# zhang-tao-whu/DVIS_Plus

Hardware: AMD Instinct MI355X
Metric: frames/sec DVIS++ R50 offline, 720p T=30 synthetic (higher is better)
Workload: dtype f32 (storage, accumulation, results; the segmenter's dense layers - R50 convolutions from 128 channels on, pixel-decoder projections and FPN output convolution, the deformable encoder's projections and FFN, the decoder's key / value projections - multiply each fp32 operand as two f16 terms on the f1

## Files before the change

### dvis_plus_amd/csrc/conv1x1_x3.hip

```cpp
#include "dvis_common.h"
#include "x3_common.h"

DVIS_EXPORT int64_t dvis_conv_x3_image_bytes(int64_t N, int C, int H, int W);

namespace {

constexpr unsigned kOOB = 0x80000000u;

struct CxArgs {
  const float *x, *bias, *res;
  const void *wp;
  float *y;
  int N, C, K, relu, npass;
  int stride, W_in, OW, H_in;
  int taps;
  long long HW, HW_in, pixels;
  long long tiles;
  float xscale, inv;
  int *flag;
  int tag;
  const float *x2;
  int C2, stride2, W2_in;
  long long HW2_in;
  void *img;
  int XG;
  float oscale;
  int OH;
  const void *ximg;
  int XG_in;
};

__device__ __forceinline__ bool cx_item(const CxArgs &a, long long w, long long *tile, int *pass) {
  const int xcd = blockIdx.x & 7, i = blockIdx.x >> 3, per = gridDim.x >> 3;
  const long long m = i + (long long)per * w;
  const long long u = m / a.npass;
  *pass = (int)(m - u * a.npass);
  *tile = xcd + 8 * u;
  return *tile < a.tiles;
}

struct CxGeom {
  unsigned base;
  int iy, ix;
  int row0;
};
__device__ __forceinline__ CxGeom cx_geom(const CxArgs &a, long long p) {
  CxGeom gm = {kOOB, 0, 0, 0};
  if (p >= a.pixels) return gm;
  const long long n = p / a.HW;
  const int pix = (int)(p - n * a.HW);
  const int oy = pix / a.OW, ox = pix - oy * a.OW, pad = a.taps == 9 ? 1 : 0;
  gm.base = (unsigned)(n * a.C * a.HW_in * 4);
  gm.iy = oy * a.stride - pad, gm.ix = ox * a.stride - pad;
  gm.row0 = (int)(n * a.H_in);
  return gm;
}
__device__ __forceinline__ unsigned cx_tap_offset(const CxArgs &a, const CxGeom &gm, int tap) {
  const int dy = a.taps == 9 ? tap / 3 : 0, dx = a.taps == 9 ? tap - 3 * dy : 0;
  const int iy = gm.iy + dy, ix = gm.ix + dx;
  const bool ok = gm.base != kOOB && iy >= 0 && iy < a.H_in && ix >= 0 && ix < a.W_in;
  return ok ? gm.base + (unsigned)((iy * a.W_in + ix) * 4) : kOOB;
}

__device__ __forceinline__ unsigned cx_tap_offset_img(const CxArgs &a, const CxGeom &gm, int tap, int g) {
  const int dy = a.taps == 9 ? tap / 3 : 0, dx = a.taps == 9 ? tap - 3 * dy : 0;
  const int iy = gm.iy + dy, ix = gm.ix + dx;
  const bool ok = gm.base != kOOB && iy >= 0 && iy < a.H_in && ix >= 0 && ix < a.W_in;
  return ok ? (unsigned)(((gm.row0 + iy) * a.XG_in + (ix >> 5)) * ((a.C / 64) * 8192) + g * 512 + (ix & 31) * 16) : kOOB;
}

__device__ __forceinline__ unsigned cx_geom2(const CxArgs &a, long long p) {
  if (a.C2 == 0 || p >= a.pixels) return kOOB;
  const long long n = p / a.HW;
  const int pix = (int)(p - n * a.HW);
  const int oy = pix / a.OW, ox = pix - oy * a.OW;
  return (unsigned)(n * a.C2 * a.HW2_in * 4) + (unsigned)((oy * a.stride2 * a.W2_in + ox * a.stride2) * 4);
}

template <int NB, int IK, bool IMGIN = false, bool IMGOUT = false>
__global__ __launch_bounds__(512) void conv1x1_x3_kernel(const CxArgs a) {
  constexpr int NW = 8, kTile = NW * 32, PW = 2 * IK * NB / NW, STAGES = IK == 4 ? 2 : 3, IPC = 4 / IK;
  static_assert(2 * IK * NB % NW == 0, "the item's pieces must divide among the waves");
  extern __shared__ __attribute__((aligned(1024))) char lds[];
  const int wave = threadIdx.x >> 6, lane = threadIdx.x & 63, j = lane & 31, g = lane >> 5;
  const int NCC = a.C / 64, NC1 = a.taps * NCC, NC = NC1 + a.C2 / 64, NI = IPC * NC;
  long long wcount = 0;
  {
    long long t;
    int q;
    while (cx_item(a, wcount, &t, &q)) ++wcount;
  }
  if (wcount == 0) return;
  const __amdgpu_buffer_rsrc_t rx = dvis_make_rsrc_uniform(a.x, (unsigned)((long long)a.N * a.C * a.HW_in * 4));
  const __amdgpu_buffer_rsrc_t ry = dvis_make_rsrc_uniform(a.y, (unsigned)((long long)a.N * a.K * a.HW * 4));
  const __amdgpu_buffer_rsrc_t rr = dvis_make_rsrc_uniform(a.res ? a.res : a.y, (unsigned)((long long)a.N * a.K * a.HW * 4));
  const unsigned chan = (unsigned)(a.HW_in * 4);
  const __amdgpu_buffer_rsrc_t rx2 = dvis_make_rsrc_uniform(a.C2 ? a.x2 : a.x, a.C2 ? (unsigned)((long long)a.N * a.C2 * a.HW2_in * 4) : 0u);
  const unsigned chan2 = (unsigned)(a.HW2_in * 4);

  typedef Ring<PW, IMGIN ? 8 : 32, NW, STAGES> RingT;
  RingT ring;
  long long iw = 0;
  int ic = 0, ipass;
  {
    long long t;
    cx_item(a, 0, &t, &ipass);
  }
  auto next_offset = [&]() -> size_t {
    const size_t o = ((size_t)ipass * NI + ic) * RingT::kItemBytes;
    if (++ic == NI) {
      ic = 0;
      long long t;
      if (!cx_item(a, ++iw, &t, &ipass)) ipass = 0;
    }
    return o;
  };
  ring.init(a.wp, lds, 1, (int)(wcount * NI), wave, lane);
#pragma unroll
  for (int i = 0; i < RingT::kAhead; ++i)
    if (ring.total > i) ring.issue_at(next_offset());

  float raw[32];
  auto load_raw = [&](unsigned pixoff, int cc, bool second = false) {
    const __amdgpu_buffer_rsrc_t r = second ? rx2 : rx;
    const unsigned ch = second ? chan2 : chan;
    const unsigned vo = pixoff + (unsigned)(8 * g) * ch;
    const unsigned so = (unsigned)(64 * cc) * ch;
#pragma unroll
    for (int s = 0; s < 4; ++s)
#pragma unroll
      for (int e = 0; e < 8; ++e)
        raw[8 * s + e] = __builtin_bit_cast(float, __builtin_amdgcn_raw_buffer_load_b32(r, vo, so + (unsigned)(16 * s + e) * ch, 0));
  };
  const __amdgpu_buffer_rsrc_t rxi = dvis_make_rsrc_uniform(IMGIN ? a.ximg : (const void *)a.x,
                                                            IMGIN ? (unsigned)((long long)a.N * a.H_in * a.XG_in * (a.C / 64) * 8192) : 0u);
  h8 nh[4], nl[4];
  auto load_img = [&](unsigned off, int cc) {
#pragma unroll
    for (int s = 0; s < 4; ++s) {
      nh[s] = __builtin_bit_cast(h8, __builtin_amdgcn_raw_buffer_load_b128(rxi, off, (unsigned)(8192 * cc + 2048 * s), 0));
      nl[s] = __builtin_bit_cast(h8, __builtin_amdgcn_raw_buffer_load_b128(rxi, off, (unsigned)(8192 * cc + 2048 * s + 1024), 0));
    }
  };
  long long tile;
  int pass;
  cx_item(a, 0, &tile, &pass);
  CxGeom gm = cx_geom(a, tile * kTile + wave * 32 + j);
  unsigned gm2 = cx_geom2(a, tile * kTile + wave * 32 + j);
  if constexpr (IMGIN)
    load_img(cx_tap_offset_img(a, gm, 0, g), 0);
  else
    load_raw(cx_tap_offset(a, gm, 0), 0);
  for (long long w = 0; w < wcount; ++w) {
    const long long p = tile * kTile + wave * 32 + j;
    long long ntile = tile;
    int npass_ = pass;
    const bool more = cx_item(a, w + 1, &ntile, &npass_);
    const CxGeom ngm = more ? cx_geom(a, ntile * kTile + wave * 32 + j) : CxGeom{kOOB, 0, 0, 0};
    const unsigned ngm2 = more ? cx_geom2(a, ntile * kTile + wave * 32 + j) : kOOB;
    int tap = 0, cc = 0;
    f16v acc[NB];
#pragma unroll
    for (int nb = 0; nb < NB; ++nb)
#pragma unroll
      for (int i = 0; i < 16; ++i) acc[nb][i] = 0.f;
    const long long n = p / a.HW;
    const unsigned obase = p < a.pixels ? (unsigned)((n * a.K * a.HW + (p - n * a.HW)) * 4) : kOOB;
    const unsigned ochan = (unsigned)(a.HW * 4);
    const int co0 = pass * 32 * NB;
    for (int kc = 0; kc < NC; ++kc) {
      h8 xh[4], xl[4];
      if constexpr (IMGIN) {
#pragma unroll
        for (int s = 0; s < 4; ++s) {
          asm volatile("" : "+v"(nh[s]), "+v"(nl[s]));
          xh[s] = nh[s], xl[s] = nl[s];
        }
        if (++cc == NCC) cc = 0, ++tap;
        const bool first = kc + 1 < NC1;
        load_img(first ? cx_tap_offset_img(a, gm, tap, g) : cx_tap_offset_img(a, ngm, 0, g), first ? cc : 0);
      } else {
#pragma unroll
        for (int i = 0; i < 32; ++i) asm volatile("" : "+v"(raw[i]));
#pragma unroll
        for (int s = 0; s < 4; ++s) {
          const f4 lo4 = {raw[8 * s], raw[8 * s + 1], raw[8 * s + 2], raw[8 * s + 3]};
          const f4 hi4 = {raw[8 * s + 4], raw[8 * s + 5], raw[8 * s + 6], raw[8 * s + 7]};
          split8(lo4, hi4, a.xscale, xh[s], xl[s]);
        }
        if (++cc == NCC) cc = 0, ++tap;
        const bool first = kc + 1 < NC1, sec = !first && kc + 1 < NC;
        const unsigned po = first ? cx_tap_offset(a, gm, tap) : (sec ? gm2 : cx_tap_offset(a, ngm, 0));
        load_raw(po, first ? cc : (sec ? kc + 1 - NC1 : 0), sec);
      }
#pragma unroll
      for (int part = 0; part < IPC; ++part) {
        const char *stage = ring.wait(false);
        ring.begin(ring.more() ? next_offset() : 0);
        mma_item<IK, NB, PW>(stage, lane, acc, xh + IK * part, xl + IK * part, [&](int i) { ring.piece(i); });
      }
    }
    float chk = 0.f;
    if constexpr (NB == 2 || IMGOUT) {
      if (a.img != nullptr) {
        const unsigned gs = (unsigned)(a.K / 64) * 8192u;
        const __amdgpu_buffer_rsrc_t ri = dvis_make_rsrc_uniform(a.img, (unsigned)((long long)a.N * a.OH * a.XG * gs));
        const __amdgpu_buffer_rsrc_t rb = dvis_make_rsrc_uniform(a.bias ? (const void *)a.bias : (const void *)a.img, a.bias ? (unsigned)a.K * 4u : 0u);
        unsigned ibase = kOOB;
        if (p < a.pixels) {
          const int pix = (int)(p - n * a.HW), oy = pix / a.OW, ox = pix - oy * a.OW;
          ibase = (unsigned)(((n * a.OH + oy) * a.XG + (ox >> 5)) * gs + (co0 / 64) * 8192 + g * 512 + (ox & 31) * 16);
        }
#pragma unroll
        for (int nb = 0; nb < NB; ++nb) {
          float v[16];
#pragma unroll
          for (int q = 0; q < 4; ++q) {
            const f4 b = __builtin_bit_cast(f4, __builtin_amdgcn_raw_buffer_load_b128(rb, (unsigned)(co0 + 32 * nb + 8 * q + 4 * g) * 4u, 0, 0));
#pragma unroll
            for (int i = 0; i < 4; ++i) {
              const float t = acc[nb][4 * q + i] * a.inv + b[i];
              chk = __builtin_fmaf(t, 0.f, chk);
              v[4 * q + i] = a.relu ? x3_relu(t) : t;
            }
          }
          h8 hi[2], lo[2];
#pragma unroll
          for (int u = 0; u < 2; ++u) {
            const f4 p0 = {v[8 * u], v[8 * u + 1], v[8 * u + 2], v[8 * u + 3]}, p1 = {v[8 * u + 4], v[8 * u + 5], v[8 * u + 6], v[8 * u + 7]};
            split8(p0, p1, a.oscale, hi[u], lo[u]);
          }
          const h8 ls = lo[0] + lo[1];
          chk = __builtin_fmaf((float)((ls[0] + ls[1]) + (ls[2] + ls[3]) + (ls[4] + ls[5]) + (ls[6] + ls[7])), 0.f, chk);
          store_fragments4(ri, ibase, hi[0], 4096 * nb, lo[0], 4096 * nb + 1024, hi[1], 4096 * nb + 2048, lo[1], 4096 * nb + 3072);
        }
        if (a.flag != nullptr && chk != chk && p < a.pixels) atomicCAS(a.flag, 0, a.tag);
        tile = ntile, pass = npass_, gm = ngm, gm2 = ngm2;
        continue;
      }
    }
#pragma unroll
    for (int nb = 0; nb < NB; ++nb) {
      float rv[16];
#pragma unroll
      for (int r = 0; r < 16; ++r)
        rv[r] = a.res ? __builtin_bit_cast(float, __builtin_amdgcn_raw_buffer_load_b32(
                                                      rr, obase + (unsigned)(co0 + 32 * nb + 8 * (r >> 2) + 4 * g + (r & 3)) * ochan, 0, 0))
                      : 0.f;
#pragma unroll
      for (int q = 0; q < 4; ++q) {
        const int co = co0 + 32 * nb + 8 * q + 4 * g;
        f4 b = {0.f, 0.f, 0.f, 0.f};
        if (a.bias) b = *(const f4 *)(a.bias + co);
#pragma unroll
        for (int i = 0; i < 4; ++i) {
          const unsigned o = obase + (unsigned)(co + i) * ochan;
          float v = acc[nb][4 * q + i] * a.inv + b[i] + rv[4 * q + i];
          chk = __builtin_fmaf(v, 0.f, chk);
          if (a.relu) v = x3_relu(v);
          __builtin_amdgcn_raw_buffer_store_b32(__builtin_bit_cast(unsigned, v), ry, o, 0, 0);
        }
      }
    }
    if (a.flag != nullptr && chk != chk && p < a.pixels) atomicCAS(a.flag, 0, a.tag);
    tile = ntile, pass = npass_, gm = ngm, gm2 = ngm2;
  }
}

__global__ __launch_bounds__(256) void upsample_add_image_kernel(const float *__restrict__ lateral, const float *__restrict__ top,
                                                                 void *__restrict__ img, int N, int C, int H, int W, int h, int w,
                                                                 const float *__restrict__ lat_scale, const float *__restrict__ lat_shift,
                                                                 float oscale) {
  const int NCC = C / 64, XG = (W + 31) / 32;
  const int cc = blockIdx.x, xg = blockIdx.y;
  const int x = threadIdx.x & 31, g = (threadIdx.x >> 5) & 1, S = threadIdx.x >> 6;
  const int px = 32 * xg + x;
  const float sy = (float)h / (float)H, sx = (float)w / (float)W;
  const int pxc = px < W ? px : W - 1;
  float fx = sx * ((float)pxc + 0.5f) - 0.5f;
  fx = fx < 0.f ? 0.f : fx;
  const int x0 = min((int)fx, w - 1), x1 = x0 + (x0 < w - 1 ? 1 : 0);
  const float lx1 = fx - (float)x0, lx0 = 1.f - lx1;
  const __amdgpu_buffer_rsrc_t ri = dvis_make_rsrc_uniform(img, (unsigned)((long long)N * H * XG * NCC * 8192));
  const unsigned rows = (unsigned)N * (unsigned)H;
  for (unsigned row = blockIdx.z * 16u; row < blockIdx.z * 16u + 16u && row < rows; ++row) {
    const unsigned n = row / (unsigned)H;
    const int y = (int)(row - n * (unsigned)H);
    float fy = sy * ((float)y + 0.5f) - 0.5f;
    fy = fy < 0.f ? 0.f : fy;
    const int y0 = min((int)fy, h - 1), y1 = y0 + (y0 < h - 1 ? 1 : 0);
    const float ly1 = fy - (float)y0, ly0 = 1.f - ly1;
    float v[8];
#pragma unroll
    for (int e = 0; e < 8; ++e) {
      const int c = 64 * cc + 32 * (S >> 1) + 16 * (S & 1) + 8 * (e >> 2) + 4 * g + (e & 3);
      const unsigned pl = n * (unsigned)C + (unsigned)c;
      const float *t0 = top + ((size_t)pl * h + y0) * (size_t)w, *t1 = top + ((size_t)pl * h + y1) * (size_t)w;
      float lat = lateral[((size_t)pl * H + y) * (size_t)W + pxc];
      if (lat_scale) lat = lat * lat_scale[pl] + lat_shift[pl];
      v[e] = lat + (ly0 * (lx0 * t0[x0] + lx1 * t0[x1]) + ly1 * (lx0 * t1[x0] + lx1 * t1[x1]));
    }
    const f4 p0 = {v[0], v[1], v[2], v[3]}, p1 = {v[4], v[5], v[6], v[7]};
    h8 hi, lo;
    split8(p0, p1, oscale, hi, lo);
    const unsigned G = row * (unsigned)XG + (unsigned)xg;
    const unsigned off = (G * (unsigned)NCC + (unsigned)cc) * 8192u + (unsigned)(S * 2048 + g * 512 + x * 16);
    store_fragments2(ri, off, hi, 0, lo, 1024);
  }
}

}

DVIS_EXPORT int dvis_upsample_add_image(const float *lateral, const float *lat_scale, const float *lat_shift, const float *top, void *image,
                                        int N, int C, int H, int W, int h, int w, int oexp, void *stream) {
  DVIS_REQUIRE(lateral && top && image, "dvis_upsample_add_image: null pointer");
  DVIS_REQUIRE((lat_scale == nullptr) == (lat_shift == nullptr), "dvis_upsample_add_image: scale and shift together");
  DVIS_REQUIRE(N > 0 && C > 0 && C % 64 == 0 && H > 0 && W > 0 && h > 0 && w > 0, "dvis_upsample_add_image: bad sizes");
  DVIS_REQUIRE((uintptr_t)image % 16 == 0 && dvis_conv_x3_image_bytes(N, C, H, W) < ((int64_t)1 << 31), "dvis_upsample_add_image: a 16-byte "
               "aligned image below 2 GiB");
  const int per = 16 * 65535 / H;
  DVIS_REQUIRE(per >= 1 && (W + 31) / 32 <= 65535, "dvis_upsample_add_image: map too large (%d x %d)", H, W);
  for (int i = 0; i < N; i += per) {
    const int n = N - i < per ? N - i : per;
    hipLaunchKernelGGL(upsample_add_image_kernel, dim3(C / 64, (W + 31) / 32, (n * H + 15) / 16), dim3(256), 0, (hipStream_t)stream,
                       lateral + (size_t)i * C * H * W, top + (size_t)i * C * h * w,
                       (char *)image + (size_t)i * H * ((W + 31) / 32) * (C / 64) * 8192, n, C, H, W, h, w,
                       lat_scale ? lat_scale + (size_t)i * C : nullptr, lat_shift ? lat_shift + (size_t)i * C : nullptr, ldexpf(1.f, oexp));
  }
  return dvis_check_launch("dvis_upsample_add_image");
}

DVIS_EXPORT int dvis_conv1x1_x3_supported(int C, int K, int64_t N, int64_t HW_in, int64_t HW_out) {
  if (C < 64 || C % 64 != 0 || C > 4096) return 0;
  if (!(K == 64 || K == 128 || (K > 0 && K % 256 == 0 && K <= 8192))) return 0;
  if (N <= 0 || HW_out <= 0 || HW_in < HW_out) return 0;
  if (N * C * HW_in * 4 >= ((int64_t)1 << 31) || N * K * HW_out * 4 >= ((int64_t)1 << 31)) return 0;
  return 1;
}

DVIS_EXPORT int64_t dvis_conv1x1_x3_packed_bytes(int C, int K) {
  if (!dvis_conv1x1_x3_supported(C, K, 1, 1, 1)) return -1;
  return (int64_t)(C / 16) * (K / 32) * 2 * kPiece;
}

DVIS_EXPORT int dvis_conv1x1_x3_pack(const float *w, int K, int C, int wexp, void *packed, void *stream) {
  DVIS_REQUIRE(w && packed, "dvis_conv1x1_x3_pack: null operand");
  DVIS_REQUIRE(dvis_conv1x1_x3_supported(C, K, 1, 1, 1), "dvis_conv1x1_x3_pack: (C, K) = (%d, %d) is not served", C, K);
  DVIS_REQUIRE(wexp >= -60 && wexp <= 60, "dvis_conv1x1_x3_pack: wexp = %d", wexp);
  const int NB = K == 64 ? 2 : K == 128 ? 4 : 8;
  const int64_t fragments = (int64_t)(C / 16) * (K / 32) * 64;
  hipLaunchKernelGGL(x3_pack_kernel, dim3((unsigned)((fragments + 255) / 256)), dim3(256), 0, (hipStream_t)stream, w, (int64_t)C, K, C,
                     NB, 0, ldexpf(1.f, wexp), (_Float16 *)packed, fragments);
  return dvis_check_launch("dvis_conv1x1_x3_pack");
}

static int cx_launch(const float *x, const void *packed, const float *bias, const float *res, float *y, int N, int C, int K, int H, int W,
                     int stride, int taps, int xexp, int wexp, int relu, void *stream, const float *x2 = nullptr, int C2 = 0, int H2 = 0,
                     int W2 = 0, int stride2 = 1, void *image = nullptr, int oexp = 0, const void *ximg = nullptr);

DVIS_EXPORT int dvis_conv1x1_x3_dual(const float *x, const float *x2, const void *packed, const float *bias, const float *res, float *y,
                                     int N, int C, int C2, int K, int H, int W, int H2, int W2, int stride2, int xexp, int wexp, int relu,
                                     void *stream) {
  DVIS_REQUIRE(x2 != nullptr && C2 >= 64 && C2 % 64 == 0 && C2 <= 4096, "dvis_conv1x1_x3_dual: C2 %% 64 == 0 (got %d)", C2);
  DVIS_REQUIRE((stride2 == 1 || stride2 == 2) && (H2 + stride2 - 1) / stride2 == H && (W2 + stride2 - 1) / stride2 == W,
               "dvis_conv1x1_x3_dual: x2 (%d x %d, stride %d) must down-sample onto x's %d x %d map", H2, W2, stride2, H, W);
  DVIS_REQUIRE((long long)N * C2 * H2 * W2 * 4 < ((long long)1 << 31) && (uintptr_t)x2 % 16 == 0, "dvis_conv1x1_x3_dual: x2 below 2 GiB, 16-byte aligned");
  return cx_launch(x, packed, bias, res, y, N, C, K, H, W, 1, 1, xexp, wexp, relu, stream, x2, C2, H2, W2, stride2);
}

DVIS_EXPORT int dvis_conv1x1_x3(const float *x, const void *packed, const float *bias, const float *res, float *y, int N, int C, int K,
                                int H, int W, int stride, int xexp, int wexp, int relu, void *stream) {
  return cx_launch(x, packed, bias, res, y, N, C, K, H, W, stride, 1, xexp, wexp, relu, stream);
}

DVIS_EXPORT int dvis_conv1x1_x3_image(const float *x, const void *packed, const float *bias, void *image, int N, int C, int H, int W, int xexp,
                                      int wexp, int oexp, int relu, void *stream) {
  DVIS_REQUIRE(image != nullptr && (uintptr_t)image % 16 == 0, "dvis_conv1x1_x3_image: null / unaligned image");
  DVIS_REQUIRE((long long)N * H * ((W + 31) / 32) * 8192 < ((long long)1 << 31), "dvis_conv1x1_x3_image: the image must stay below 2 GiB");
  return cx_launch(x, packed, bias, nullptr, nullptr, N, C, 64, H, W, 1, 1, xexp, wexp, relu, stream, nullptr, 0, 0, 0, 1, image, oexp);
}

DVIS_EXPORT int64_t dvis_conv_x3_image_bytes(int64_t N, int C, int H, int W) {
  if (N < 0 || C <= 0 || C % 64 != 0 || H <= 0 || W <= 0) return -1;
  return N * H * ((W + 31) / 32) * (int64_t)(C / 64) * 8192;
}

DVIS_EXPORT int dvis_conv_x3_pack_image(const float *w, int K, int C, int taps, int wexp, void *packed, void *stream) {
  DVIS_REQUIRE(w && packed, "dvis_conv_x3_pack_image: null operand");
  DVIS_REQUIRE(taps == 1 || taps == 9, "dvis_conv_x3_pack_image: taps = %d", taps);
  DVIS_REQUIRE(dvis_conv1x1_x3_supported(C, K, 1, 1, 1) && K >= 128, "dvis_conv_x3_pack_image: (C, K) = (%d, %d) is not served", C, K);
  DVIS_REQUIRE(wexp >= -60 && wexp <= 60, "dvis_conv_x3_pack_image: wexp = %d", wexp);
  const int NB = K == 128 ? 4 : 8;
  const int64_t fragments = (int64_t)(taps * C / 16) * (K / 32) * 64;
  hipLaunchKernelGGL(x3_pack_kernel, dim3((unsigned)((fragments + 255) / 256)), dim3(256), 0, (hipStream_t)stream, w, (int64_t)taps * C, K,
                     taps * C, NB, 1, ldexpf(1.f, wexp), (_Float16 *)packed, fragments, taps);
  return dvis_check_launch("dvis_conv_x3_pack_image");
}

DVIS_EXPORT int dvis_conv_x3_image(const void *ximg, const float *x, const void *packed, const float *bias, const float *res, float *y,
                                   void *image, int N, int C, int K, int H, int W, int stride, int taps, int xexp, int wexp, int oexp, int relu,
                                   void *stream) {
  DVIS_REQUIRE(ximg != nullptr || image != nullptr, "dvis_conv_x3_image: neither side is an operand image (use dvis_conv1x1_x3 / dvis_conv3x3_x3)");
  DVIS_REQUIRE((ximg != nullptr) != (x != nullptr), "dvis_conv_x3_image: exactly one of ximg and x");
  DVIS_REQUIRE((image != nullptr) != (y != nullptr), "dvis_conv_x3_image: exactly one of image and y");
  DVIS_REQUIRE(K == 128 || K % 256 == 0, "dvis_conv_x3_image: K = %d (128 or a multiple of 256)", K);
  DVIS_REQUIRE(taps == 1 || taps == 9, "dvis_conv_x3_image: taps = %d", taps);
  DVIS_REQUIRE(image == nullptr || res == nullptr, "dvis_conv_x3_image: an image output takes no residual");
  DVIS_REQUIRE(((uintptr_t)ximg | (uintptr_t)image) % 16 == 0, "dvis_conv_x3_image: images must be 16-byte aligned");
  const int OH = (H + stride - 1) / stride, OW = (W + stride - 1) / stride;
  DVIS_REQUIRE(dvis_conv_x3_image_bytes(N, C, H, W) < ((int64_t)1 << 31) && dvis_conv_x3_image_bytes(N, K, OH, OW) < ((int64_t)1 << 31),
               "dvis_conv_x3_image: images must stay below 2 GiB");
  return cx_launch(x, packed, bias, res, y, N, C, K, H, W, stride, taps, xexp, wexp, relu, stream, nullptr, 0, 0, 0, 1, image, oexp, ximg);
}

DVIS_EXPORT int64_t dvis_conv3x3_x3_packed_bytes(int C, int K) {
  const int64_t b = dvis_conv1x1_x3_packed_bytes(C, K);
  return b < 0 ? b : 9 * b;
}

DVIS_EXPORT int dvis_conv3x3_x3_pack(const float *w, int K, int C, int wexp, void *packed, void *stream) {
  DVIS_REQUIRE(w && packed, "dvis_conv3x3_x3_pack: null operand");
  DVIS_REQUIRE(dvis_conv1x1_x3_supported(C, K, 1, 1, 1), "dvis_conv3x3_x3_pack: (C, K) = (%d, %d) is not served", C, K);
  DVIS_REQUIRE(wexp >= -60 && wexp <= 60, "dvis_conv3x3_x3_pack: wexp = %d", wexp);
  const int NB = K == 64 ? 2 : K == 128 ? 4 : 8;
  const int64_t fragments = (int64_t)(9 * C / 16) * (K / 32) * 64;
  hipLaunchKernelGGL(x3_pack_kernel, dim3((unsigned)((fragments + 255) / 256)), dim3(256), 0, (hipStream_t)stream, w, (int64_t)9 * C, K, 9 * C,
                     NB, 0, ldexpf(1.f, wexp), (_Float16 *)packed, fragments, 9);
  return dvis_check_launch("dvis_conv3x3_x3_pack");
}

DVIS_EXPORT int dvis_conv3x3_x3(const float *x, const void *packed, const float *bias, const float *res, float *y, int N, int C, int K,
                                int H, int W, int stride, int xexp, int wexp, int relu, void *stream) {
  return cx_launch(x, packed, bias, res, y, N, C, K, H, W, stride, 9, xexp, wexp, relu, stream);
}

static int cx_launch(const float *x, const void *packed, const float *bias, const float *res, float *y, int N, int C, int K, int H, int W,
                     int stride, int taps, int xexp, int wexp, int relu, void *stream, const float *x2, int C2, int H2, int W2, int stride2,
                     void *image, int oexp, const void *ximg) {
  DVIS_REQUIRE((x || ximg) && packed && (y || image), "dvis_conv1x1_x3: null operand");
  DVIS_REQUIRE(stride == 1 || stride == 2, "dvis_conv1x1_x3: stride %d", stride);
  const int OH = (H + stride - 1) / stride, OW = (W + stride - 1) / stride;
  DVIS_REQUIRE(dvis_conv1x1_x3_supported(C, K, N, (int64_t)H * W, (int64_t)OH * OW), "dvis_conv1x1_x3: shape (N %d, C %d, K %d, %d x %d, "
               "stride %d) is not served (C %% 64 == 0, K = 64 / 128 or K %% 256 == 0, tensors below 2 GiB)", N, C, K, H, W, stride);
  DVIS_REQUIRE((uintptr_t)x % 16 == 0 && (uintptr_t)y % 16 == 0 && (uintptr_t)packed % 16 == 0 && (bias == nullptr || (uintptr_t)bias % 16 == 0),
               "dvis_conv1x1_x3: operands must be 16-byte aligned");
  CxArgs a = {};
  a.x = x, a.bias = bias, a.res = res, a.wp = packed, a.y = y, a.N = N, a.C = C, a.K = K, a.relu = relu;
  a.stride = stride, a.W_in = W, a.H_in = H, a.taps = taps, a.OW = OW, a.HW = (long long)OH * OW, a.HW_in = (long long)H * W;
  a.pixels = a.HW * N;
  a.xscale = ldexpf(1.f, xexp), a.inv = ldexpf(1.f, -(xexp + wexp));
  const X3Guard gd = dvis_x3_guard();
  a.flag = gd.flag, a.tag = gd.tag;
  a.x2 = x2, a.C2 = x2 ? C2 : 0, a.stride2 = stride2, a.W2_in = W2, a.HW2_in = (long long)H2 * W2;
  a.img = image, a.XG = (OW + 31) / 32, a.oscale = ldexpf(1.f, oexp), a.OH = OH;
  a.ximg = ximg, a.XG_in = (W + 31) / 32;
  const int grid = dvis_x3_persistent_cus();
  hipStream_t st = (hipStream_t)stream;
  a.npass = K <= 128 ? 1 : K / 256;
#define DVIS_CX_LAUNCH(NBV, IKV)                                                                              \
  {                                                                                                           \
    static DvisLdsOptIn opted;                                                                                \
    typedef Ring<2 * IKV * NBV / 8, 32, 8, (IKV == 4 ? 2 : 3)> R;                                             \
    a.tiles = (a.pixels + 255) / 256;                                                                         \
    const size_t lds = (IKV == 4 ? 2 : 3) * R::kItemBytes;                                                    \
    const int rc = dvis_lds_opt_in((const void *)conv1x1_x3_kernel<NBV, IKV>, lds, &opted, "dvis_conv1x1_x3"); \
    if (rc != DVIS_OK) return rc;                                                                             \
    hipLaunchKernelGGL((conv1x1_x3_kernel<NBV, IKV>), dim3(grid), dim3(512), lds, st, a);                     \
  }
#define DVIS_CX_LAUNCH_IMG(NBV, IKV, INV, OUTV)                                                                                    \
  {                                                                                                                                \
    static DvisLdsOptIn opted;                                                                                                     \
    typedef Ring<2 * IKV * NBV / 8, 8, 8, (IKV == 4 ? 2 : 3)> R;                                                                   \
    a.tiles = (a.pixels + 255) / 256;                                                                                              \
    const size_t lds = (IKV == 4 ? 2 : 3) * R::kItemBytes;                                                                         \
    const int rc = dvis_lds_opt_in((const void *)conv1x1_x3_kernel<NBV, IKV, INV, OUTV>, lds, &opted, "dvis_conv_x3_image");    \
    if (rc != DVIS_OK) return rc;                                                                                                  \
    hipLaunchKernelGGL((conv1x1_x3_kernel<NBV, IKV, INV, OUTV>), dim3(grid), dim3(512), lds, st, a);                            \
    return dvis_check_launch("dvis_conv_x3_image");                                                                                \
  }
  if (ximg != nullptr || (image != nullptr && K != 64)) {
    DVIS_REQUIRE(x2 == nullptr, "dvis_conv_x3_image: no second source");
    if (K == 128) {
      if (ximg && image) DVIS_CX_LAUNCH_IMG(4, 2, true, true)
      if (ximg) DVIS_CX_LAUNCH_IMG(4, 2, true, false)
      DVIS_CX_LAUNCH_IMG(4, 2, false, true)
    }
    if (ximg && image) DVIS_CX_LAUNCH_IMG(8, 4, true, true)
    if (ximg) DVIS_CX_LAUNCH_IMG(8, 4, true, false)
    DVIS_CX_LAUNCH_IMG(8, 4, false, true)
  }
#undef DVIS_CX_LAUNCH_IMG
  if (K == 64) DVIS_CX_LAUNCH(2, 2)
  else if (K == 128) DVIS_CX_LAUNCH(4, 2)
  else DVIS_CX_LAUNCH(8, 4)
#undef DVIS_CX_LAUNCH
  return dvis_check_launch("dvis_conv1x1_x3");
}
```

### dvis_plus_amd/csrc/fused_elementwise.hip

```cpp
#include <math.h>

#include "dvis_common.h"

namespace {

template <int V>
__global__ __launch_bounds__(256) void add_layernorm_kernel(const float *__restrict__ x, const float *__restrict__ res,
                                                            int64_t res_row_stride, const float *__restrict__ gamma,
                                                            const float *__restrict__ beta, float *__restrict__ out,
                                                            size_t rows, int C, float eps,
                                                            const float *__restrict__ pos, size_t pos_rows,
                                                            float *__restrict__ out_pos) {
  const int lane = threadIdx.x & 63;
  const size_t row = (size_t)blockIdx.x * 4 + (threadIdx.x >> 6);
  if (row >= rows) return;
  const float4 *xr = reinterpret_cast<const float4 *>(x + row * C);
  const float4 *rr = res ? reinterpret_cast<const float4 *>(res + row * res_row_stride) : nullptr;
  float4 v[V];
  float sum = 0.f;
#pragma unroll
  for (int i = 0; i < V; ++i) {
    const int c4 = lane + 64 * i;
    if (c4 * 4 < C) {
      v[i] = xr[c4];
// ... 372 lines not shown
  float *ob = out + b * batch_stride + c4;
#pragma unroll
  for (int o = 0; o < 4; ++o) {
    if (x0 + o >= w) break;
    float4 v = acc[o];
    if (gelu) {
      v.x = 0.5f * v.x * (1.f + erff(v.x * 0.70710678118654752440f)), v.y = 0.5f * v.y * (1.f + erff(v.y * 0.70710678118654752440f));
      v.z = 0.5f * v.z * (1.f + erff(v.z * 0.70710678118654752440f)), v.w = 0.5f * v.w * (1.f + erff(v.w * 0.70710678118654752440f));
    }
    *reinterpret_cast<float4 *>(ob + ((int64_t)y * w + x0 + o) * C) = v;
  }
}

}

DVIS_EXPORT int dvis_normalize_pad(const void *in, int is_u8, float *out, int64_t planes, int C, int H, int W, int Hp, int Wp,
                                   const float *mean, const float *stdv, void *stream) {
  DVIS_REQUIRE(planes >= 0 && C > 0 && H > 0 && W > 0 && Hp >= H && Wp >= W, "normalize_pad: bad sizes");
  if (planes == 0) return DVIS_OK;
  DVIS_REQUIRE(in && out && mean && stdv, "normalize_pad: null pointer");
  DVIS_REQUIRE(planes <= 65535 && (Hp + 3) / 4 <= 65535, "normalize_pad: grid too large");
  const dim3 grid((unsigned)(((Wp + 3) / 4 + 63) / 64), (unsigned)((Hp + 3) / 4), (unsigned)planes);
  if (is_u8)
    hipLaunchKernelGGL(normalize_pad_kernel<unsigned char>, grid, dim3(256), 0, (hipStream_t)stream, (const unsigned char *)in, out, C,
                       H, W, Hp, Wp, mean, stdv);
  else
    hipLaunchKernelGGL(normalize_pad_kernel<float>, grid, dim3(256), 0, (hipStream_t)stream, (const float *)in, out, C, H, W, Hp, Wp,
                       mean, stdv);
  return dvis_check_launch("normalize_pad_kernel");
}

DVIS_EXPORT int dvis_tokens_to_nchw(const float *tok, float *out, int64_t N, int C, int64_t HW, int64_t S, int64_t row0, void *stream) {
  DVIS_REQUIRE(N >= 0 && C > 0 && HW > 0 && S >= HW && row0 >= 0 && row0 + HW <= S, "tokens_to_nchw: bad sizes");
  if (N == 0) return DVIS_OK;
  DVIS_REQUIRE(tok && out, "tokens_to_nchw: null pointer");
  DVIS_REQUIRE(N <= 65535 && (C + 63) / 64 <= 65535 && HW < (1ll << 31), "tokens_to_nchw: grid too large");
  hipLaunchKernelGGL(tokens_to_nchw_kernel, dim3((unsigned)((HW + 63) / 64), (unsigned)((C + 63) / 64), (unsigned)N), dim3(256), 0,
                     (hipStream_t)stream, tok, out, C, (int)HW, S, row0);
  return dvis_check_launch("tokens_to_nchw_kernel");
}

static int nchw_to_tokens_launch(const float *x, float *out, int64_t N, int C, int64_t HW, int64_t S, int64_t row0,
                                 const float *scale, const float *shift, const float *pos, float *out_pos, void *stream) {
  DVIS_REQUIRE(N >= 0 && C > 0 && HW > 0 && S >= HW && row0 >= 0 && row0 + HW <= S, "nchw_to_tokens: bad sizes");
  if (N == 0) return DVIS_OK;
  DVIS_REQUIRE(x && out, "nchw_to_tokens: null pointer");
  DVIS_REQUIRE((scale == nullptr) == (shift == nullptr) && (pos == nullptr) == (out_pos == nullptr),
               "nchw_to_tokens: scale/shift and pos/out_pos come in pairs");
  DVIS_REQUIRE(N <= 65535 && (C + 63) / 64 <= 65535 && HW < (1ll << 31), "nchw_to_tokens: grid too large");
  hipLaunchKernelGGL(nchw_to_tokens_kernel, dim3((unsigned)((HW + 63) / 64), (unsigned)((C + 63) / 64), (unsigned)N), dim3(256),
                     0, (hipStream_t)stream, x, out, C, (int)HW, S, row0, scale, shift, pos, out_pos);
  return dvis_check_launch("nchw_to_tokens_kernel");
}

DVIS_EXPORT int dvis_nchw_to_tokens(const float *x, float *out, int64_t N, int C, int64_t HW, int64_t S, int64_t row0,
                                    void *stream) {
  return nchw_to_tokens_launch(x, out, N, C, HW, S, row0, nullptr, nullptr, nullptr, nullptr, stream);
}

DVIS_EXPORT int dvis_nchw_to_tokens_affine(const float *x, const float *scale, const float *shift, const float *pos,
                                           float *out, float *out_pos, int64_t N, int C, int64_t HW, int64_t S,
                                           int64_t row0, void *stream) {
  return nchw_to_tokens_launch(x, out, N, C, HW, S, row0, scale, shift, pos, out_pos, stream);
}

DVIS_EXPORT int dvis_bias_act(float *x, const float *bias, const float *res, int64_t planes, int C, int64_t HW, int relu,
                              void *stream) {
  DVIS_REQUIRE(planes >= 0 && C > 0 && HW > 0, "bias_act: bad sizes");
  if (planes == 0) return DVIS_OK;
  DVIS_REQUIRE(x, "bias_act: null pointer");
  if (HW % 4 != 0 || (((uintptr_t)x | (uintptr_t)res) & 15) != 0) {
    const long long total = (long long)planes * HW;
    const long long blocks = (total + 255) / 256;
    hipLaunchKernelGGL(bias_act_scalar_kernel, dim3((unsigned)(blocks > 65535 * 16 ? 65535 * 16 : blocks)), dim3(256), 0,
                       (hipStream_t)stream, x, bias, res, C, (long long)HW, total, relu);
    return dvis_check_launch("bias_act_scalar_kernel");
  }
  const int HW4 = (int)(HW / 4);
  int chunks = (HW4 + 1023) / 1024;
  if (chunks < 1) chunks = 1;
  DVIS_REQUIRE(planes * chunks < (1ll << 31), "bias_act: too many planes");
  hipLaunchKernelGGL(bias_act_kernel, dim3((unsigned)(planes * chunks)), dim3(256), 0, (hipStream_t)stream, x, bias, res, C,
                     HW4, chunks, relu);
  return dvis_check_launch("bias_act_kernel");
}

static int add_layernorm_launch(const float *x, const float *res, int64_t res_row_stride, const float *gamma,
                                const float *beta, float *out, int64_t rows, int C, float eps, const float *pos,
                                int64_t pos_rows, float *out_pos, void *stream) {
  DVIS_REQUIRE(rows >= 0 && C > 0, "add_layernorm: bad sizes");
  if (rows == 0) return DVIS_OK;
  DVIS_REQUIRE(x && gamma && beta && out, "add_layernorm: null pointer");
  DVIS_REQUIRE(C % 4 == 0 && C <= 1024, "add_layernorm: C must be a multiple of 4 and <= 1024 (got %d)", C);
  DVIS_REQUIRE(res == nullptr || res_row_stride % 4 == 0, "add_layernorm: residual row stride must be a multiple of 4");
  DVIS_REQUIRE(pos == nullptr || (pos_rows > 0 && out_pos != nullptr), "add_layernorm: pos needs pos_rows > 0 and out_pos");
  const uintptr_t al = (uintptr_t)x | (uintptr_t)res | (uintptr_t)gamma | (uintptr_t)beta | (uintptr_t)out |
                       (uintptr_t)pos | (uintptr_t)out_pos;
  DVIS_REQUIRE((al & 15) == 0, "add_layernorm: pointers must be 16-byte aligned");
  const dim3 grid((unsigned)((rows + 3) / 4)), block(256);
  hipStream_t st = (hipStream_t)stream;
  const size_t pr = pos ? (size_t)pos_rows : 1;
  if (C <= 256)
    hipLaunchKernelGGL((add_layernorm_kernel<1>), grid, block, 0, st, x, res, res_row_stride, gamma, beta, out, (size_t)rows, C, eps, pos, pr, out_pos);
  else if (C <= 512)
    hipLaunchKernelGGL((add_layernorm_kernel<2>), grid, block, 0, st, x, res, res_row_stride, gamma, beta, out, (size_t)rows, C, eps, pos, pr, out_pos);
  else
    hipLaunchKernelGGL((add_layernorm_kernel<4>), grid, block, 0, st, x, res, res_row_stride, gamma, beta, out, (size_t)rows, C, eps, pos, pr, out_pos);
  return dvis_check_launch("add_layernorm_kernel");
}

DVIS_EXPORT int dvis_add_layernorm(const float *x, const float *res, int64_t res_row_stride, const float *gamma,
                                   const float *beta, float *out, int64_t rows, int C, float eps, void *stream) {
  return add_layernorm_launch(x, res, res_row_stride, gamma, beta, out, rows, C, eps, nullptr, 0, nullptr, stream);
}

DVIS_EXPORT int dvis_add_layernorm_pos(const float *x, const float *res, int64_t res_row_stride, const float *gamma,
                                       const float *beta, float *out, const float *pos, int64_t pos_rows, float *out_pos,
                                       int64_t rows, int C, float eps, void *stream) {
  DVIS_REQUIRE(pos && out_pos, "add_layernorm_pos: null pos / out_pos");
  return add_layernorm_launch(x, res, res_row_stride, gamma, beta, out, rows, C, eps, pos, pos_rows, out_pos, stream);
}

static int upsample_add_launch(const float *lateral, const float *top, float *out, int64_t planes, int H, int W, int h,
                               int w, const float *lat_scale, const float *lat_shift, void *stream) {
  DVIS_REQUIRE(planes >= 0 && H > 0 && W > 0 && h > 0 && w > 0, "upsample_add: bad sizes");
  if (planes == 0) return DVIS_OK;
  DVIS_REQUIRE(lateral && top && out, "upsample_add: null pointer");
  DVIS_REQUIRE((lat_scale == nullptr) == (lat_shift == nullptr), "upsample_add: scale and shift come together");
  DVIS_REQUIRE(planes < (1ll << 31), "upsample_add: too many planes");
  if (W % 4 != 0 || (((uintptr_t)lateral | (uintptr_t)out) & 15) != 0) {
    const long long tot = (long long)planes * H * W;
    long long nb = (tot + 255) / 256;
    if (nb > 256 * 32) nb = 256 * 32;
    hipLaunchKernelGGL(upsample_add_scalar_kernel, dim3((unsigned)nb), dim3(256), 0, (hipStream_t)stream, lateral, top, out, tot, H, W,
                       h, w, lat_scale, lat_shift);
    return dvis_check_launch("upsample_add_scalar_kernel");
  }
  const size_t total = (size_t)planes * H * (W / 4);
  size_t blocks = (total + 255) / 256;
  if (blocks > 256 * 32) blocks = 256 * 32;
  DVIS_REQUIRE(total < (1ull << 32), "upsample_add: more than 2^32 output quads");
  const bool x2 = H == 2 * h && W == 2 * w && (w & 1) == 0 && ((uintptr_t)top & 7) == 0;
  if (x2)
    hipLaunchKernelGGL(upsample_add_kernel<true>, dim3((unsigned)blocks), dim3(256), 0, (hipStream_t)stream, lateral, top,
                       out, (int)planes, H, W, h, w, lat_scale, lat_shift);
  else
    hipLaunchKernelGGL(upsample_add_kernel<false>, dim3((unsigned)blocks), dim3(256), 0, (hipStream_t)stream, lateral, top,
                       out, (int)planes, H, W, h, w, lat_scale, lat_shift);
  return dvis_check_launch("upsample_add_kernel");
}

DVIS_EXPORT int dvis_dwconv3x3_tokens(const float *x, float *out, int64_t batch_stride, int B, int h, int w, int C, const float *weight,
                                      const float *bias, int gelu, void *stream) {
  DVIS_REQUIRE(x && out && weight, "dwconv3x3_tokens: null pointer");
  DVIS_REQUIRE(B >= 0 && h > 0 && w > 0 && C > 0 && C % 4 == 0 && batch_stride % 4 == 0 && batch_stride >= (int64_t)h * w * C,
               "dwconv3x3_tokens: C %% 4 == 0 and a batch stride that is a multiple of 4 floats >= h * w * C are required");
  DVIS_REQUIRE(((uintptr_t)x | (uintptr_t)out | (uintptr_t)(bias ? bias : weight)) % 16 == 0, "dwconv3x3_tokens: 16-byte alignment");
  DVIS_REQUIRE(x != out, "dwconv3x3_tokens: in place is not possible (neighbouring tokens are read)");
  if (B == 0) return DVIS_OK;
  const int64_t strips = (int64_t)h * ((w + 3) / 4);
  DVIS_REQUIRE(strips * B < ((int64_t)1 << 32), "dwconv3x3_tokens: too many tokens");
  hipLaunchKernelGGL(dwconv3x3_tokens_kernel, dim3((unsigned)((strips * B + 3) / 4), (C / 4 + 63) / 64), dim3(256), 0, (hipStream_t)stream, x,
                     out, batch_stride, B, h, w, C, weight, bias, gelu);
  return dvis_check_launch("dwconv3x3_tokens_kernel");
}

DVIS_EXPORT int dvis_adapter_res2(const float *g, const float *c1, const float *x1, const float *scale, const float *shift, float *out,
                                  int B, int C, int h8, int w8, void *stream) {
  DVIS_REQUIRE(g && c1 && scale && shift && out, "adapter_res2: null pointer");
  DVIS_REQUIRE(((uintptr_t)g | (uintptr_t)c1 | (uintptr_t)out) % 16 == 0, "adapter_res2: g / c1 / out must be 16-byte aligned");
  DVIS_REQUIRE(B >= 0 && C > 0 && C % 64 == 0 && h8 > 0 && w8 > 0 && h8 % 2 == 0 && w8 % 2 == 0,
               "adapter_res2: C %% 64 == 0 and an even stride-8 grid are required (C %d, grid %d x %d)", C, h8, w8);
  DVIS_REQUIRE((int64_t)B * h8 <= 65535 && C / 64 <= 65535, "adapter_res2: grid too large (B * rows %lld)", (long long)B * h8);
  if (B == 0) return DVIS_OK;
  hipLaunchKernelGGL(adapter_res2_kernel, dim3((w8 + 31) / 32, C / 64, B * h8), dim3(256), 0, (hipStream_t)stream, g, c1, x1, scale, shift,
                     out, C, h8, w8);
  return dvis_check_launch("adapter_res2_kernel");
}

DVIS_EXPORT int dvis_upsample_add(const float *lateral, const float *top, float *out, int64_t planes, int H, int W, int h,
                                  int w, void *stream) {
  return upsample_add_launch(lateral, top, out, planes, H, W, h, w, nullptr, nullptr, stream);
}

DVIS_EXPORT int dvis_upsample_add_affine(const float *lateral, const float *lat_scale, const float *lat_shift,
                                         const float *top, float *out, int64_t planes, int H, int W, int h, int w,
                                         void *stream) {
  DVIS_REQUIRE(lat_scale && lat_shift, "upsample_add_affine: null scale / shift");
  return upsample_add_launch(lateral, top, out, planes, H, W, h, w, lat_scale, lat_shift, stream);
}

DVIS_EXPORT int dvis_bias_relu_maxpool(const float *x, const float *bias, float *out, int64_t planes, int C, int H, int W,
                                       void *stream) {
  DVIS_REQUIRE(planes >= 0 && C > 0 && H > 0 && W > 0, "bias_relu_maxpool: bad sizes");
  if (planes == 0) return DVIS_OK;
  DVIS_REQUIRE(x && out, "bias_relu_maxpool: null pointer");
  DVIS_REQUIRE(H % 2 == 0 && W % 8 == 0 && (((uintptr_t)x | (uintptr_t)out) & 15) == 0,
               "bias_relu_maxpool: needs even H, W %% 8 == 0 and 16-byte aligned x / out (H=%d W=%d)", H, W);
  const size_t total = (size_t)planes * (H / 2) * (W / 8);
  DVIS_REQUIRE(planes < (1ll << 31) && total < (1ull << 32), "bias_relu_maxpool: too many planes / outputs");
  size_t blocks = (total + 255) / 256;
  if (blocks > 256 * 32) blocks = 256 * 32;
  hipLaunchKernelGGL(bias_relu_maxpool_kernel, dim3((unsigned)blocks), dim3(256), 0, (hipStream_t)stream, x, bias, out,
                     (int)planes, C, H, W);
  return dvis_check_launch("bias_relu_maxpool_kernel");
}

namespace {

__global__ __launch_bounds__(1024) void group_norm_affine_kernel(const float *__restrict__ x, const float *__restrict__ gamma,
                                                                 const float *__restrict__ beta, float *__restrict__ scale,
                                                                 float *__restrict__ shift, int C, int G, long long HW,
                                                                 float eps, int vec) {
  __shared__ double s_sum[16], s_sq[16];
  const int Cg = C / G;
  const int n = blockIdx.x / G, g = blockIdx.x - n * G;
  const long long count = (long long)Cg * HW, count4 = count / 4;
  const float4 *xp = reinterpret_cast<const float4 *>(x + ((size_t)n * C + (size_t)g * Cg) * HW);
  double sum = 0.0, sq = 0.0;
  if (vec) {
    for (long long i = threadIdx.x; i < count4; i += 1024) {
      const float4 v = xp[i];
      sum += ((double)v.x + (double)v.y) + ((double)v.z + (double)v.w);
      sq += ((double)v.x * v.x + (double)v.y * v.y) + ((double)v.z * v.z + (double)v.w * v.w);
    }
  } else {
    const float *xs = reinterpret_cast<const float *>(xp);
    for (long long i = threadIdx.x; i < count; i += 1024) {
      const double v = (double)xs[i];
      sum += v;
      sq += v * v;
    }
  }
#pragma unroll
  for (int o = 32; o > 0; o >>= 1) {
    sum += __shfl_down(sum, o);
    sq += __shfl_down(sq, o);
  }
  const int wv = threadIdx.x >> 6;
  if ((threadIdx.x & 63) == 0) {
    s_sum[wv] = sum;
    s_sq[wv] = sq;
  }
  __syncthreads();
  if (threadIdx.x < Cg) {
    double ts = 0.0, tq = 0.0;
#pragma unroll
    for (int i = 0; i < 16; ++i) {
      ts += s_sum[i];
      tq += s_sq[i];
    }
    const double mean = ts / (double)count;
    double var = tq / (double)count - mean * mean;
    var = var < 0.0 ? 0.0 : var;
    const float rstd = (float)(1.0 / sqrt(var + (double)eps));
    const int c = g * Cg + threadIdx.x;
    const float a = rstd * (gamma ? gamma[c] : 1.f);
    scale[(size_t)n * C + c] = a;
    shift[(size_t)n * C + c] = (beta ? beta[c] : 0.f) - (float)mean * a;
  }
}

__global__ __launch_bounds__(256) void scale_shift_act_kernel(float *__restrict__ x, const float *__restrict__ scale,
                                                              const float *__restrict__ shift, int HW4, int chunks, int relu) {
  const unsigned plane = blockIdx.x / chunks;
  const int chunk = blockIdx.x - plane * chunks;
  const float a = scale[plane], b = shift[plane];
  float4 *xp = reinterpret_cast<float4 *>(x) + (size_t)plane * HW4;
  for (int i = chunk * 256 + threadIdx.x; i < HW4; i += chunks * 256) {
    float4 v = xp[i];
    v.x = v.x * a + b; v.y = v.y * a + b; v.z = v.z * a + b; v.w = v.w * a + b;
    if (relu) {
      v.x = fmaxf(v.x, 0.f); v.y = fmaxf(v.y, 0.f); v.z = fmaxf(v.z, 0.f); v.w = fmaxf(v.w, 0.f);
    }
    xp[i] = v;
  }
}

__global__ __launch_bounds__(256) void scale_shift_act_scalar_kernel(float *__restrict__ x, const float *__restrict__ scale,
                                                                     const float *__restrict__ shift, long long HW, long long total,
                                                                     int relu) {
  for (long long i = (long long)blockIdx.x * 256 + threadIdx.x; i < total; i += (long long)gridDim.x * 256) {
    const long long plane = i / HW;
    const float v = x[i] * scale[plane] + shift[plane];
    x[i] = relu ? fmaxf(v, 0.f) : v;
  }
}

}

DVIS_EXPORT int dvis_group_norm_affine(const float *x, const float *gamma, const float *beta, float *scale, float *shift,
                                       int64_t N, int C, int G, int64_t HW, float eps, void *stream) {
  DVIS_REQUIRE(N >= 0 && C > 0 && G > 0 && HW > 0 && C % G == 0, "group_norm_affine: bad sizes (C=%d G=%d)", C, G);
  if (N == 0) return DVIS_OK;
  DVIS_REQUIRE(x && scale && shift, "group_norm_affine: null pointer");
  DVIS_REQUIRE(C / G <= 1024, "group_norm_affine: at most 1024 channels per group");
  const int vec = ((int64_t)(C / G) * HW) % 4 == 0 && ((uintptr_t)x & 15) == 0;
  DVIS_REQUIRE(N * G < (1ll << 31), "group_norm_affine: too many groups");
  hipLaunchKernelGGL(group_norm_affine_kernel, dim3((unsigned)(N * G)), dim3(1024), 0, (hipStream_t)stream, x, gamma, beta,
                     scale, shift, C, G, (long long)HW, eps, vec);
  return dvis_check_launch("group_norm_affine_kernel");
}

DVIS_EXPORT int dvis_scale_shift_act(float *x, const float *scale, const float *shift, int64_t planes, int64_t HW, int relu,
                                     void *stream) {
  DVIS_REQUIRE(planes >= 0 && HW > 0, "scale_shift_act: bad sizes");
  if (planes == 0) return DVIS_OK;
  DVIS_REQUIRE(x && scale && shift, "scale_shift_act: null pointer");
  if (HW % 4 != 0 || ((uintptr_t)x & 15) != 0) {
    const long long total = (long long)planes * HW;
    const long long blocks = (total + 255) / 256;
    hipLaunchKernelGGL(scale_shift_act_scalar_kernel, dim3((unsigned)(blocks > 65535 * 16 ? 65535 * 16 : blocks)), dim3(256), 0,
                       (hipStream_t)stream, x, scale, shift, (long long)HW, total, relu);
    return dvis_check_launch("scale_shift_act_scalar_kernel");
  }
  const int HW4 = (int)(HW / 4);
  int chunks = (HW4 + 1023) / 1024;
  if (chunks < 1) chunks = 1;
  DVIS_REQUIRE(planes * chunks < (1ll << 31), "scale_shift_act: too many planes");
  hipLaunchKernelGGL(scale_shift_act_kernel, dim3((unsigned)(planes * chunks)), dim3(256), 0, (hipStream_t)stream, x, scale,
                     shift, HW4, chunks, relu);
  return dvis_check_launch("scale_shift_act_kernel");
}
```

### dvis_plus_amd/functions.py

```python
import collections
import ctypes
import math
import os
import threading

import torch
from torch.autograd import Function
from torch.autograd.function import once_differentiable

from . import cpu_ops, derived, native
from .cpu_ops import ms_deform_attn_core_pytorch


def _torch_path(op, x, why):
    if os.environ.get("DVIS_STRICT", "1") != "0" and x.is_cuda and not torch.is_grad_enabled():
        raise RuntimeError(f"DVIS_STRICT: {op} would run its torch formulation on a GPU tensor ({why}; shape "
                           f"{tuple(x.shape)}, dtype {x.dtype}, contiguous {x.is_contiguous()})")


class no_autocast:

    def __enter__(self):
        import contextlib
        self._stack = contextlib.ExitStack()
# ... 1263 lines not shown
    buf, wexp = x3_tile_pack(weight, img.order)
    bptr = None if bias is None else native.dev_ptr(bias.detach(), "bias")
    lib = native.lib()
    with torch.cuda.device(img.device):
        if act == "gelu":
            if residual is not None:
                raise RuntimeError("x3_tile_linear: the GELU form of a row image writes a row image (no residual)")
            out = _rows_image_buffer(M, N, img.device)
            native.check(lib.dvis_x3_tile_linear_image(ctypes.c_void_p(img.data.data_ptr()), M, K, ctypes.c_void_p(buf.data_ptr()), N, img.exp, wexp,
                                                       bptr, 2, None, 0, None, 0, ctypes.c_void_p(out.data_ptr()), X3_XEXP,
                                                       native.stream_ptr(img.device)), "dvis_x3_tile_linear_image")
            return RowImage(out, (*img.shape[:-1], N), X3_XEXP, 1)
        out = torch.empty((*img.shape[:-1], N), dtype=torch.float32, device=img.device)
        rptr, ldr = None, 0
        if residual is not None:
            if residual.shape != out.shape or residual.dtype != torch.float32 or not residual.is_cuda:
                raise RuntimeError("x3_tile_linear: residual must be a float32 GPU tensor of the output's shape")
            r2, ldr = _rows2d(residual, N)
            rptr = ctypes.c_void_p(r2.data_ptr())
        native.check(lib.dvis_x3_tile_linear_image(ctypes.c_void_p(img.data.data_ptr()), M, K, ctypes.c_void_p(buf.data_ptr()), N, img.exp, wexp,
                                                   bptr, {None: 0, "relu": 1}[act], rptr, ldr, ctypes.c_void_p(out.data_ptr()), N, None, 0,
                                                   native.stream_ptr(img.device)), "dvis_x3_tile_linear_image")
    return out


X3_QKV_FUSED = os.environ.get("DVIS_X3_QKV_FUSED", "1") != "0"


def x3_qkv_attention_ok(x, weight, heads):
    if isinstance(x, RowImage):
        if len(x.shape) != 3 or not (X3_QKV_FUSED and weight.dim() == 2 and weight._base is None):
            return False
        B, L, C = x.shape
        return (C == heads * 64 and weight.shape == (3 * C, C) and L >= 1024 and C >= X3_TILE_MIN_K
                and bool(native.lib().dvis_x3_tile_supported(3 * C, C)))
    if not (X3_QKV_FUSED and x.dim() == 3 and x.is_cuda and x.dtype == torch.float32 and not torch.is_grad_enabled()
            and not torch.is_autocast_enabled() and x3_on() and weight.dim() == 2 and weight._base is None):
        return False
    B, L, C = x.shape
    return (C == heads * 64 and weight.shape == (3 * C, C) and L >= 1024 and x.is_contiguous() and x.data_ptr() % 16 == 0
            and x3_tile_ok(x, 3 * C, C))


def x3_qkv_attention(x, weight, bias, heads, out_image=False):
    B, L, C = x.shape
    image_in = isinstance(x, RowImage)
    buf, wexp = x3_tile_pack(weight, x.order if image_in else 0)
    lib = native.lib()
    nbytes = lib.dvis_attention_ws_bytes_k(B * heads, L, L, 64, 2)
    ws = torch.empty((nbytes + 3) // 4, dtype=torch.float32, device=x.device)
    qscale = (1.0 / 8.0) * 1.4426950408889634 * 16.0
    bptr = None if bias is None else native.dev_ptr(bias.detach(), "bias")
    with torch.cuda.device(x.device):
        if image_in:
            native.check(lib.dvis_x3_tile_linear_qkv_image(
                ctypes.c_void_p(x.data.data_ptr()), B * L, C, ctypes.c_void_p(buf.data_ptr()), 3 * C, x.exp, wexp, bptr, heads, L, qscale,
                ctypes.c_void_p(ws.data_ptr()), native.stream_ptr(x.device)), "dvis_x3_tile_linear_qkv_image")
        else:
            native.check(lib.dvis_x3_tile_linear_qkv(
                ctypes.c_void_p(x.data_ptr()), C, B * L, C, ctypes.c_void_p(buf.data_ptr()), 3 * C, X3_XEXP, wexp, bptr, heads, L, qscale,
                ctypes.c_void_p(ws.data_ptr()), native.stream_ptr(x.device)), "dvis_x3_tile_linear_qkv")
        if out_image:
            out = _rows_image_buffer(B * L, C, x.device)
            native.check(lib.dvis_attention_x3_packed_image(ctypes.c_void_p(ws.data_ptr()), ctypes.c_void_p(out.data_ptr()), B, heads, L, X3_XEXP,
                                                            native.stream_ptr(x.device)), "dvis_attention_x3_packed_image")
            return RowImage(out, (B, L, C), X3_XEXP, 2)
        out = torch.empty((B, L, C), dtype=torch.float32, device=x.device)
        strides = (ctypes.c_int64 * 3)(L * C, 64, C)
        native.check(lib.dvis_attention_x3_packed(ctypes.c_void_p(ws.data_ptr()), ctypes.c_void_p(out.data_ptr()), strides, B, heads, L,
                                                  native.stream_ptr(x.device)), "dvis_attention_x3_packed")
    return out


def x3_ok(x, N, K, ln=False, add=False):
    return (x.is_cuda and x.dtype == torch.float32 and not torch.is_grad_enabled() and x.shape[-1] == K
            and (not add or K == 256) and bool(native.lib().dvis_x3_linear_supported(N, K, int(ln))))


def _x3_rows(x, name):
    K = x.shape[-1]
    x2, ld = _rows2d(x, K)
    if x2.data_ptr() % 16 or ld % 4:
        raise RuntimeError(f"x3: {name} must be 16-byte aligned with a row stride % 4 == 0")
    return x2, ld


def x3_linear(x, weight, bias, relu=False, xexp=None, xadd=None, act=None, residual=None):
    N, K = weight.shape
    x2, ldx = _x3_rows(x, "x")
    buf, wexp = x3_pack(weight)
    out = torch.empty((*x.shape[:-1], N), dtype=torch.float32, device=x.device)
    if act is not None or residual is not None:
        if xadd is not None:
            raise RuntimeError("x3_linear: xadd and act / residual are served by different entry points")
        code = {None: int(bool(relu)), "relu": 1, "gelu": 2}[act]
        rptr, ldr = None, 0
        if residual is not None:
            if residual.shape != out.shape or residual.dtype != torch.float32 or not residual.is_cuda:
                raise RuntimeError("x3_linear: residual must be a float32 GPU tensor of the output's shape")
            r2, ldr = _x3_rows(residual, "residual")
            rptr = ctypes.c_void_p(r2.data_ptr())
        with torch.cuda.device(x.device):
            native.check(native.lib().dvis_x3_linear_res(
                ctypes.c_void_p(x2.data_ptr()), ldx, x2.shape[0], K, ctypes.c_void_p(buf.data_ptr()), N,
                X3_XEXP if xexp is None else xexp, wexp, None if bias is None else native.dev_ptr(bias.detach(), "bias"), code,
                rptr, ldr, ctypes.c_void_p(out.data_ptr()), N, native.stream_ptr(x.device)), "dvis_x3_linear_res")
        return out
    if xadd is not None:
        if x.dim() != 3 or xadd.numel() != x.shape[1] * K or xadd.dtype != torch.float32 or not xadd.is_cuda:
            raise RuntimeError("x3_linear: xadd must be a float32 GPU (S, K) embedding for x of shape (B, S, K)")
        xadd = xadd.contiguous()
        with torch.cuda.device(x.device):
            native.check(native.lib().dvis_x3_linear_add(
                ctypes.c_void_p(x2.data_ptr()), ldx, x2.shape[0], K, ctypes.c_void_p(buf.data_ptr()), N,
                X3_XEXP if xexp is None else xexp, wexp, ctypes.c_void_p(xadd.data_ptr()), x.shape[1],
                None if bias is None else native.dev_ptr(bias.detach(), "bias"), int(relu), ctypes.c_void_p(out.data_ptr()), N,
                native.stream_ptr(x.device)), "dvis_x3_linear_add")
        return out
    with torch.cuda.device(x.device):
        native.check(native.lib().dvis_x3_linear(
            ctypes.c_void_p(x2.data_ptr()), ldx, x2.shape[0], K, ctypes.c_void_p(buf.data_ptr()), N,
            X3_XEXP if xexp is None else xexp, wexp, None if bias is None else native.dev_ptr(bias.detach(), "bias"), int(relu),
            ctypes.c_void_p(out.data_ptr()), N, native.stream_ptr(x.device)), "dvis_x3_linear")
    return out


def _x3_pos(pos, x, N):
    if pos is None:
        return None, 0, None
    if x.dim() != 3 or pos.numel() != x.shape[1] * N or pos.dtype != torch.float32 or not pos.is_cuda:
        raise RuntimeError("x3: pos must be a float32 GPU (S, C) embedding for x of shape (N, S, C)")
    return pos.contiguous(), x.shape[1], torch.empty((*x.shape[:-1], N), dtype=torch.float32, device=x.device)


def x3_linear_ln(x, weight, bias, res, norm, pos=None, xexp=None):
    N, K = weight.shape
    x2, ldx = _x3_rows(x, "x")
    r2, ldr = _x3_rows(res, "res")
    buf, wexp = x3_pack(weight)
    out = torch.empty((*x.shape[:-1], N), dtype=torch.float32, device=x.device)
    pos, pos_rows, out2 = _x3_pos(pos, x, N)
    with torch.cuda.device(x.device):
        native.check(native.lib().dvis_x3_linear_ln(
            ctypes.c_void_p(x2.data_ptr()), ldx, x2.shape[0], K, ctypes.c_void_p(buf.data_ptr()), N,
            X3_XEXP if xexp is None else xexp, wexp, native.dev_ptr(bias.detach(), "bias"), ctypes.c_void_p(r2.data_ptr()), ldr,
            native.dev_ptr(norm.weight.detach(), "gamma"), native.dev_ptr(norm.bias.detach(), "beta"), float(norm.eps),
            None if pos is None else ctypes.c_void_p(pos.data_ptr()), pos_rows, ctypes.c_void_p(out.data_ptr()),
            None if out2 is None else ctypes.c_void_p(out2.data_ptr()), N, native.stream_ptr(x.device)), "dvis_x3_linear_ln")
    return out if out2 is None else (out, out2)


def x3_ffn_ok(x, lin1, lin2):
    K, H, N = lin1.weight.shape[1], lin1.weight.shape[0], lin2.weight.shape[0]
    return (x.is_cuda and x.dtype == torch.float32 and not torch.is_grad_enabled() and x.shape[-1] == K
            and lin2.weight.shape[1] == H and lin1.bias is not None and lin2.bias is not None
            and native.lib().dvis_x3_ffn_packed_bytes(K, H, N) > 0)


def x3_ffn_ln(x, lin1, lin2, norm, pos=None, xexp=None, hexp=None):
    w1, w2 = lin1.weight, lin2.weight
    H, K = w1.shape
    N = w2.shape[0]
    x2, ldx = _x3_rows(x, "x")

    def make():
        a, b = w1.detach().contiguous(), w2.detach().contiguous()
        e1, e2 = _x3_wexp(a), _x3_wexp(b)
        buf = torch.empty(native.lib().dvis_x3_ffn_packed_bytes(K, H, N), dtype=torch.uint8, device=a.device)
        with torch.cuda.device(a.device):
            native.check(native.lib().dvis_x3_ffn_pack(ctypes.c_void_p(a.data_ptr()), K, ctypes.c_void_p(b.data_ptr()), H, K, H,
                                                       N, e1, e2, ctypes.c_void_p(buf.data_ptr()),
                                                       native.stream_ptr(a.device)), "dvis_x3_ffn_pack")
        return buf, e1, e2
    buf, e1, e2 = _x3_cache(w1, [w1, w2], make, kind="ffn")
    out = torch.empty((*x.shape[:-1], N), dtype=torch.float32, device=x.device)
    pos, pos_rows, out2 = _x3_pos(pos, x, N)
    with torch.cuda.device(x.device):
        native.check(native.lib().dvis_x3_ffn_ln(
            ctypes.c_void_p(x2.data_ptr()), ldx, x2.shape[0], K, H, N, ctypes.c_void_p(buf.data_ptr()),
            X3_XEXP if xexp is None else xexp, e1, X3_XEXP if hexp is None else hexp, e2,
            native.dev_ptr(lin1.bias.detach(), "b1"), native.dev_ptr(lin2.bias.detach(), "b2"),
            native.dev_ptr(norm.weight.detach(), "gamma"), native.dev_ptr(norm.bias.detach(), "beta"), float(norm.eps),
            None if pos is None else ctypes.c_void_p(pos.data_ptr()), pos_rows, ctypes.c_void_p(out.data_ptr()),
            None if out2 is None else ctypes.c_void_p(out2.data_ptr()), N, native.stream_ptr(x.device)), "dvis_x3_ffn_ln")
    return out if out2 is None else (out, out2)


def maps_to_tokens(maps, affines=None, pos=None):
    affines = affines or [None] * len(maps)
    N, C = maps[0].shape[:2]
    if not all(m.is_cuda and m.dtype == torch.float32 and m.is_contiguous() for m in maps) or torch.is_grad_enabled():
        _torch_path("maps_to_tokens", maps[0], "needs contiguous fp32 NCHW maps")
        maps = [m if a is None else m * a[0].view(N, C, 1, 1) + a[1].view(N, C, 1, 1) for m, a in zip(maps, affines)]
        out = torch.cat([m.flatten(2).transpose(1, 2) for m in maps], 1)
        return out if pos is None else (out, out + pos.reshape(1, -1, C))
    S = sum(m.shape[2] * m.shape[3] for m in maps)
    out = torch.empty((N, S, C), dtype=torch.float32, device=maps[0].device)
    out_pos = pp = None
    if pos is not None:
        if pos.numel() != S * C or pos.dtype != torch.float32 or not pos.is_cuda:
            raise RuntimeError("maps_to_tokens: pos must be a float32 GPU (S, C) embedding")
        pos = pos.contiguous()
        out_pos = torch.empty_like(out)
        pp = native.dev_ptr(pos, "pos")
    row0 = 0
    with torch.cuda.device(out.device):
        for m, a in zip(maps, affines):
            HW = m.shape[2] * m.shape[3]
            rc = native.lib().dvis_nchw_to_tokens_affine(
                ctypes.c_void_p(m.data_ptr()), None if a is None else native.dev_ptr(a[0], "scale"),
                None if a is None else native.dev_ptr(a[1], "shift"), pp, ctypes.c_void_p(out.data_ptr()),
                None if out_pos is None else ctypes.c_void_p(out_pos.data_ptr()), N, C, HW, S, row0,
                native.stream_ptr(out.device))
            native.check(rc, "dvis_nchw_to_tokens_affine")
            row0 += HW
    return out if pos is None else (out, out_pos)


def normalize_pad_ok(x, mean):
    return bool(x.is_cuda and x.dim() == 4 and x.dtype in (torch.uint8, torch.float32) and x.is_contiguous()
                and mean.numel() == x.shape[1] and mean.dtype == torch.float32 and not torch.is_grad_enabled())


def normalize_pad(x, mean, std, Hp, Wp):
    N, C, H, W = x.shape
    out = torch.empty((N, C, Hp, Wp), dtype=torch.float32, device=x.device)
    with torch.cuda.device(x.device):
        native.check(native.lib().dvis_normalize_pad(
            native.dev_ptr(x, "frames"), int(x.dtype == torch.uint8), native.dev_ptr(out, "out"), N * C, C, H, W, Hp, Wp,
            native.dev_ptr(mean.detach().reshape(-1), "pixel_mean"), native.dev_ptr(std.detach().reshape(-1), "pixel_std"),
            native.stream_ptr(x.device)), "dvis_normalize_pad")
    return out


def tokens_to_map(tokens, row0, h, w):
    N, S, C = tokens.shape
    if not (tokens.is_cuda and tokens.dtype == torch.float32 and tokens.is_contiguous() and not torch.is_grad_enabled()):
        return tokens[:, row0:row0 + h * w].transpose(1, 2).reshape(N, C, h, w)
    out = torch.empty((N, C, h, w), dtype=torch.float32, device=tokens.device)
    with torch.cuda.device(tokens.device):
        native.check(native.lib().dvis_tokens_to_nchw(ctypes.c_void_p(tokens.data_ptr()), ctypes.c_void_p(out.data_ptr()), N, C, h * w,
                                                      S, row0, native.stream_ptr(tokens.device)), "dvis_tokens_to_nchw")
    return out


def conv1x1(x, weight, bias=None):
    Co, Ci = weight.shape[:2]
    if conv1x1_x3_ok(x, weight):
        return conv1x1_x3(x, weight, bias)
    if bias is not None and CONV1X1_MFMA and x.is_cuda and x.dim() == 4 and x.is_contiguous() and x.dtype == torch.float32 \
            and weight.dtype == torch.float32 and not torch.is_grad_enabled() \
            and native.lib().dvis_conv1x1_mfma_supported(Ci, Co, x.shape[2] * x.shape[3]):
        return conv1x1_mfma(x, weight, bias)
    if x.is_cuda and Ci >= Co and x.is_contiguous() and x.dim() == 4 and x.dtype == weight.dtype \
            and not torch.is_grad_enabled():
        N, _, H, W = x.shape
        y = torch.bmm(weight.detach().view(1, Co, Ci).expand(N, Co, Ci), x.view(N, Ci, H * W)).view(N, Co, H, W)
        return y if bias is None else bias_act_(y, bias.detach(), None, relu=False)
    return torch.nn.functional.conv2d(x, weight, bias)


def conv1x1_bias_act(x, weight, bias=None, res=None, relu=False):
    Co, Ci = weight.shape[:2]
    if x.is_cuda and x.dim() == 4 and x.dtype == torch.float32 and weight.dtype == torch.float32 and x.is_contiguous() \
            and not torch.is_grad_enabled() and (res is None or (res.is_contiguous() and res.dtype == torch.float32)):
        N, _, H, W = x.shape
        if Ci >= X3_CONV1X1_MIN_CI and conv1x1_x3_ok(x, weight, 1, res):
            return conv1x1_x3(x, weight, bias, res, relu)
        if native.lib().dvis_conv1x1_supported(Ci, Co, H * W) and (res is None or res.shape == (N, Co, H, W)):
            w2 = weight.detach().reshape(Co, Ci)
            if not w2.is_contiguous():
                w2 = w2.contiguous()
            out = torch.empty((N, Co, H, W), dtype=torch.float32, device=x.device)
            with torch.cuda.device(x.device):
                rc = native.lib().dvis_conv1x1_bias_act(
                    native.dev_ptr(x, "x"), native.dev_ptr(w2, "weight"),
                    None if bias is None else native.dev_ptr(bias.detach(), "bias"),
                    None if res is None else native.dev_ptr(res, "res"), native.dev_ptr(out, "out"), N, Ci, Co, H * W,
                    1 if relu else 0, native.stream_ptr(x.device))
            native.check(rc, "dvis_conv1x1_bias_act")
            return out
        if CONV1X1_MFMA and native.lib().dvis_conv1x1_mfma_supported(Ci, Co, H * W) and (res is None or res.shape == (N, Co, H, W)):
            return conv1x1_mfma(x, weight, bias, res, relu)
    return bias_act_(conv1x1(x, weight), None if bias is None else bias.detach(), res, relu)


def conv1x1_x3_ok(x, weight, stride=1, res=None):
    if not (x3_on() and x.is_cuda and x.dim() == 4 and x.dtype == torch.float32 and weight.dtype == torch.float32 and x.is_contiguous()
            and not torch.is_grad_enabled()):
        return False
    N, Ci, H, W = x.shape
    Co = weight.shape[0]
    OH, OW = (H + stride - 1) // stride, (W + stride - 1) // stride
    if res is not None and not (res.is_contiguous() and res.dtype == torch.float32 and tuple(res.shape) == (N, Co, OH, OW)):
        return False
    return N == 0 or bool(native.lib().dvis_conv1x1_x3_supported(Ci, Co, 1, H * W, OH * OW))


def _conv_x3_chunks(N, Ci, Co, HW_in, HW_out):
    per = max(Ci * HW_in, Co * HW_out) * 4
    return max(1, min(N, (2 ** 31 - 1) // per))


def conv1x1_x3(x, weight, bias=None, res=None, relu=False, stride=1, xexp=None):
    N, Ci, H, W = x.shape
    Co = weight.shape[0]

    def make():
        return _x3_pack_conv1x1(weight.detach().reshape(Co, Ci).contiguous())
    buf, wexp = _x3_cache(weight, [weight], make, kind="conv1x1")
    OH, OW = (H + stride - 1) // stride, (W + stride - 1) // stride
    out = torch.empty((N, Co, OH, OW), dtype=torch.float32, device=x.device)
    step = _conv_x3_chunks(N, Ci, Co, H * W, OH * OW)
    with torch.cuda.device(x.device):
        for i in range(0, N, step):
            n = min(step, N - i)
            native.check(native.lib().dvis_conv1x1_x3(
                native.dev_ptr(x[i:i + n], "x"), ctypes.c_void_p(buf.data_ptr()),
                None if bias is None else native.dev_ptr(bias.detach(), "bias"),
                None if res is None else native.dev_ptr(res[i:i + n], "res"), native.dev_ptr(out[i:i + n], "out"), n, Ci, Co, H, W,
                stride, X3_CONV_XEXP if xexp is None else xexp, wexp, 1 if relu else 0, native.stream_ptr(x.device)),
                "dvis_conv1x1_x3")
    return out


X3_DUAL = os.environ.get("DVIS_X3_DUAL", "1") != "0"


def conv1x1_x3_dual_ok(a, w3, x, ws, stride2):
    if not (X3_DUAL and conv1x1_x3_ok(a, w3) and x.is_cuda and x.dim() == 4 and x.dtype == torch.float32 and x.is_contiguous()
            and ws.dtype == torch.float32 and ws.shape[0] == w3.shape[0] and stride2 in (1, 2)):
        return False
    N, C, H, W = a.shape
    N2, C2, H2, W2 = x.shape
    Co = w3.shape[0]
    return (N2 == N and C2 % 64 == 0 and 64 <= C2 <= 4096 and (H2 + stride2 - 1) // stride2 == H and (W2 + stride2 - 1) // stride2 == W
            and (C + C2) <= 4096 and bool(native.lib().dvis_conv1x1_x3_supported(C + C2, Co, 1, H * W, H * W))
            and C2 * H2 * W2 * 4 < 2 ** 31)


def conv1x1_x3_dual(a, w3, b3, x, ws, bs, relu=True, stride2=1, xexp=None):
    N, C, H, W = a.shape
    _, C2, H2, W2 = x.shape
    Co = w3.shape[0]

    def make():
        wcat = torch.cat([w3.detach().reshape(Co, C), ws.detach().reshape(Co, C2)], 1).contiguous()
        buf, e = _x3_pack_conv1x1(wcat)
        bias = None
        if b3 is not None or bs is not None:
            bias = (0 if b3 is None else b3.detach()) + (0 if bs is None else bs.detach())
        return buf, e, bias
    buf, wexp, bias = _x3_cache(w3, [w3, ws, b3, bs], make, kind="conv1x1 + shortcut")
    out = torch.empty((N, Co, H, W), dtype=torch.float32, device=a.device)
    step = min(_conv_x3_chunks(N, C, Co, H * W, H * W), _conv_x3_chunks(N, C2, Co, H2 * W2, H * W))
    with torch.cuda.device(a.device):
        for i in range(0, N, step):
            n = min(step, N - i)
            native.check(native.lib().dvis_conv1x1_x3_dual(
                native.dev_ptr(a[i:i + n], "a"), native.dev_ptr(x[i:i + n], "x"), ctypes.c_void_p(buf.data_ptr()),
                None if bias is None else native.dev_ptr(bias, "bias"), None, native.dev_ptr(out[i:i + n], "out"), n, C, C2, Co, H, W,
                H2, W2, stride2, X3_CONV_XEXP if xexp is None else xexp, wexp, 1 if relu else 0, native.stream_ptr(a.device)),
                "dvis_conv1x1_x3_dual")
    return out


def conv3x3_x3_ok(x, weight, stride=1, res=None):
    return weight.dim() == 4 and tuple(weight.shape[2:]) == (3, 3) and conv1x1_x3_ok(x, weight, stride, res)


def conv3x3_x3(x, weight, bias=None, res=None, relu=False, stride=1, xexp=None):
    N, Ci, H, W = x.shape
    Co = weight.shape[0]

    def make():
        return _x3_pack_conv3x3(weight.detach().contiguous())
    buf, wexp = _x3_cache(weight, [weight], make, kind="conv3x3")
    OH, OW = (H + stride - 1) // stride, (W + stride - 1) // stride
    out = torch.empty((N, Co, OH, OW), dtype=torch.float32, device=x.device)
    step = _conv_x3_chunks(N, Ci, Co, H * W, OH * OW)
    with torch.cuda.device(x.device):
        for i in range(0, N, step):
            n = min(step, N - i)
            native.check(native.lib().dvis_conv3x3_x3(
                native.dev_ptr(x[i:i + n], "x"), ctypes.c_void_p(buf.data_ptr()),
                None if bias is None else native.dev_ptr(bias.detach(), "bias"),
                None if res is None else native.dev_ptr(res[i:i + n], "res"), native.dev_ptr(out[i:i + n], "out"), n, Ci, Co, H, W,
                stride, X3_CONV_XEXP if xexp is None else xexp, wexp, 1 if relu else 0, native.stream_ptr(x.device)),
                "dvis_conv3x3_x3")
    return out


X3_IMAGES = os.environ.get("DVIS_X3_IMAGES", "1") != "0"


class OperandImage:

    def __init__(self, data, N, C, H, W, exp):
        self.data, self.N, self.C, self.H, self.W, self.exp = data, N, C, H, W, exp

    @property
    def device(self):
        return self.data.device

    def images(self, i, n):
        per = self.data.numel() // self.N
        return self.data[i * per:(i + n) * per]


def x3_images_ok(N, C, K, H, W, device, taps=1, stride=1):
    if not (X3_IMAGES and x3_on() and device.type == "cuda" and not torch.is_grad_enabled()):
        return False
    if taps not in (1, 9) or C % 64 != 0 or not (K == 128 or K % 256 == 0) or N <= 0:
        return False
    OH, OW = (H + stride - 1) // stride, (W + stride - 1) // stride
    return bool(native.lib().dvis_conv1x1_x3_supported(C, K, 1, H * W, OH * OW))


def _image_chunks(N, C, K, H, W, OH, OW):
    per = max(C * H * ((W + 31) // 32 * 32), K * OH * ((OW + 31) // 32 * 32)) * 4
    return max(1, min(N, (2 ** 31 - 1) // per))


def upsample_add_image(lateral, top, lat_affine=None, oexp=None):
    N, C, H, W = lateral.shape
    lib = native.lib()
    oe = X3_CONV_XEXP if oexp is None else oexp
    top = top.contiguous()
    data = torch.empty(lib.dvis_conv_x3_image_bytes(N, C, H, W), dtype=torch.uint8, device=lateral.device)
    img = OperandImage(data, N, C, H, W, oe)
    step = _image_chunks(N, C, C, H, W, H, W)
    with torch.cuda.device(lateral.device):
        for i in range(0, N, step):
            n = min(step, N - i)
            sc = None if lat_affine is None else native.dev_ptr(lat_affine[0].reshape(N, C)[i:i + n], "scale")
            sh = None if lat_affine is None else native.dev_ptr(lat_affine[1].reshape(N, C)[i:i + n], "shift")
            native.check(lib.dvis_upsample_add_image(native.dev_ptr(lateral[i:i + n], "lateral"), sc, sh, native.dev_ptr(top[i:i + n], "top"),
                                                     ctypes.c_void_p(img.images(i, n).data_ptr()), n, C, H, W, top.shape[-2], top.shape[-1], oe,
                                                     native.stream_ptr(lateral.device)), "dvis_upsample_add_image")
    return img


def conv_x3_image(src, weight, bias=None, res=None, relu=False, stride=1, out_image=False, oexp=None, xexp=None):
    lib = native.lib()
    from_img = isinstance(src, OperandImage)
    if not (from_img or out_image):
        raise ValueError("conv_x3_image: neither side is an operand image")
    N, C, H, W = (src.N, src.C, src.H, src.W) if from_img else src.shape
    K, taps = weight.shape[0], weight.shape[2] * weight.shape[3]
    dev = weight.device

    def make():
        w2 = weight.detach().contiguous()
        if from_img:
            return _x3_packed(w2, lib.dvis_conv1x1_x3_packed_bytes(C, K) * taps, lambda e, buf, st: lib.dvis_conv_x3_pack_image(
                native.dev_ptr(w2, "weight"), K, C, taps, e, buf, st), "dvis_conv_x3_pack_image")
        return _x3_pack_conv1x1(w2.reshape(K, C)) if taps == 1 else _x3_pack_conv3x3(w2)
    kind = ("conv%dx%d" % ((1, 1) if taps == 1 else (3, 3))) + (" image-in" if from_img else "")
    buf, wexp = _x3_cache(weight, [weight], make, kind=kind)
    OH, OW = (H + stride - 1) // stride, (W + stride - 1) // stride
    xe = src.exp if from_img else (X3_CONV_XEXP if xexp is None else xexp)
    oe = X3_CONV_XEXP if oexp is None else oexp
    if out_image:
        out = OperandImage(torch.empty(lib.dvis_conv_x3_image_bytes(N, K, OH, OW), dtype=torch.uint8, device=dev), N, K, OH, OW, oe)
    else:
        out = torch.empty((N, K, OH, OW), dtype=torch.float32, device=dev)
    step = _image_chunks(N, C, K, H, W, OH, OW)
    with torch.cuda.device(dev):
        for i in range(0, N, step):
            n = min(step, N - i)
            native.check(lib.dvis_conv_x3_image(
                ctypes.c_void_p(src.images(i, n).data_ptr()) if from_img else None, None if from_img else native.dev_ptr(src[i:i + n], "x"),
                ctypes.c_void_p(buf.data_ptr()), None if bias is None else native.dev_ptr(bias.detach(), "bias"),
                None if res is None else native.dev_ptr(res[i:i + n], "res"), None if out_image else native.dev_ptr(out[i:i + n], "out"),
                ctypes.c_void_p(out.images(i, n).data_ptr()) if out_image else None, n, C, K, H, W, stride, taps, xe, wexp, oe, 1 if relu else 0,
                native.stream_ptr(dev)), "dvis_conv_x3_image")
    return out


X3_BNECK = os.environ.get("DVIS_X3_BNECK", "1") != "0"


def bneck_stage_x3_ok(x, blocks):
    if not (X3_BNECK and x3_on() and x.is_cuda and x.dim() == 4 and x.dtype == torch.float32 and x.is_contiguous()
            and not torch.is_grad_enabled() and len(blocks) >= 2 and x.shape[1] == 64 and x.shape[0] > 0):
        return False
    for i, b in enumerate(blocks):
        cin = 64 if i == 0 else 256
        if tuple(b["w1"].shape) != (64, cin, 1, 1) or tuple(b["w2"].shape) != (64, 64, 3, 3) or tuple(b["w3"].shape) != (256, 64, 1, 1):
            return False
        if (b["ws"] is not None) != (i == 0) or (i == 0 and tuple(b["ws"].shape) != (256, 64, 1, 1)):
            return False
        if any(b[k] is not None and (b[k].dtype != torch.float32 or b[k].device != x.device) for k in b):
            return False
    return bool(native.lib().dvis_bneck_x3_supported(1, x.shape[2], x.shape[3]))


def bneck_stage_x3(x, blocks, xexp=None):
    N, _, H, W = x.shape
    lib = native.lib()
    xe = X3_CONV_XEXP if xexp is None else xexp
    dev = x.device

    def packed_conv1():
        w = blocks[0]["w1"]

        return _x3_cache(w, [w], lambda: _x3_pack_conv1x1(w.detach().reshape(64, 64).contiguous()), kind="conv1x1")

    def packed_block(i):
        b, nxt = blocks[i], (blocks[i + 1] if i + 1 < len(blocks) else None)
        ws, w1n = b["ws"], (None if nxt is None else nxt["w1"])

        def make():
            w2 = b["w2"].detach().contiguous()
            w3 = b["w3"].detach().reshape(256, 64).contiguous()
            wsd = None if ws is None else ws.detach().reshape(256, 64).contiguous()
            w1d = None if w1n is None else w1n.detach().reshape(64, 256).contiguous()
            e2, e1 = _x3_wexp(w2), (0 if w1d is None else _x3_wexp(w1d))
            e3 = _x3_wexp(w3 if wsd is None else torch.cat([w3, wsd], 1))
            buf = torch.empty(lib.dvis_bneck_x3_packed_bytes(0 if w1d is None else 1, 0 if wsd is None else 1), dtype=torch.uint8, device=dev)
            with torch.cuda.device(dev):
                native.check(lib.dvis_bneck_x3_pack(native.dev_ptr(w2, "w2"), native.dev_ptr(w3, "w3"),
                                                    None if wsd is None else native.dev_ptr(wsd, "ws"),
                                                    None if w1d is None else native.dev_ptr(w1d, "w1"), e2, e3, e1,
                                                    ctypes.c_void_p(buf.data_ptr()), native.stream_ptr(dev)), "dvis_bneck_x3_pack")
            b3 = b["b3"]
            if b["bs"] is not None:
                b3 = b["bs"].detach() if b3 is None else b3.detach() + b["bs"].detach()
            return buf, e2, e3, e1, (None if b3 is None else b3.detach().clone())
        return _x3_cache(b["w2"], [b["w2"], b["w3"], ws, w1n, b["b3"], b["bs"]], make, kind="bottleneck chain")

    img_bytes = lib.dvis_bneck_x3_image_bytes(N, H, W)
    imgs = [torch.empty(img_bytes, dtype=torch.uint8, device=dev) for _ in range(2)]
    ys = [torch.empty((N, 256, H, W), dtype=torch.float32, device=dev) for _ in range(min(2, len(blocks)))]
    step = max(1, min(N, (2 ** 31 - 1) // (256 * H * W * 4)))
    per_img = img_bytes // N

    def ptr(t):
        return None if t is None else native.dev_ptr(t.detach(), "shift")

    with torch.cuda.device(dev):
        for i0 in range(0, N, step):
            n = min(step, N - i0)
            isl = slice(i0 * per_img, (i0 + n) * per_img)
            buf1, e1 = packed_conv1()
            native.check(lib.dvis_conv1x1_x3_image(native.dev_ptr(x[i0:i0 + n], "x"), ctypes.c_void_p(buf1.data_ptr()), ptr(blocks[0]["b1"]),
                                                   ctypes.c_void_p(imgs[0][isl].data_ptr()), n, 64, H, W, xe, e1, xe, 1, native.stream_ptr(dev)),
                         "dvis_conv1x1_x3_image")
            for i, b in enumerate(blocks):
                buf, e2, e3, e1n, b3 = packed_block(i)
                last = i + 1 == len(blocks)
                y, yprev = ys[i % 2], ys[(i + 1) % 2]
                native.check(lib.dvis_bneck_x3(
                    ctypes.c_void_p(imgs[i % 2][isl].data_ptr()), None if i == 0 else native.dev_ptr(yprev[i0:i0 + n], "res"),
                    native.dev_ptr(x[i0:i0 + n], "x") if i == 0 else None, ctypes.c_void_p(buf.data_ptr()), ptr(b["b2"]), ptr(b3),
                    None if last else ptr(blocks[i + 1]["b1"]), native.dev_ptr(y[i0:i0 + n], "y"),
                    None if last else ctypes.c_void_p(imgs[(i + 1) % 2][isl].data_ptr()), n, H, W, xe, e2, e3, e1n, native.stream_ptr(dev)),
                    "dvis_bneck_x3")
    return ys[(len(blocks) - 1) % 2]


def _fp32_pack(weight, kind, numel, pack, name):
    def make():
        w = weight.detach().contiguous()
        uf = torch.empty(numel, dtype=torch.float32, device=w.device)
        with torch.cuda.device(w.device):
            native.check(pack(native.dev_ptr(w, "weight"), native.dev_ptr(uf, "uf"), native.stream_ptr(w.device)), name)
        return uf
    return derived.TABLE.get(weight, kind, [weight], make)


CONV1X1_MFMA = os.environ.get("DVIS_CONV1X1_MFMA", "1") != "0"


def conv1x1s2_supported(x, weight):
    N, Ci, H, W = x.shape
    return CONV1X1_MFMA and x.is_cuda and x.dtype == torch.float32 and x.is_contiguous() and not torch.is_grad_enabled() \
        and bool(native.lib().dvis_conv1x1_mfma_supported(Ci, weight.shape[0], ((H + 1) // 2) * ((W + 1) // 2))) \
        and 2 * Ci * H * W * 4 < 2 ** 31


def conv1x1_mfma(x, weight, bias=None, res=None, relu=False, stride=1):
    N, Ci, H, W = x.shape
    Co = weight.shape[0]
    uf = _fp32_pack(weight, "conv1x1 mfma", Co * Ci, lambda w, uf, st: native.lib().dvis_conv1x1_mfma_pack(w, uf, Co, Ci, st),
                    "dvis_conv1x1_mfma_pack")
    if stride == 2:
        out = torch.empty((N, Co, (H + 1) // 2, (W + 1) // 2), dtype=torch.float32, device=x.device)
        with torch.cuda.device(x.device):
            rc = native.lib().dvis_conv1x1s2_mfma(
                native.dev_ptr(x, "x"), native.dev_ptr(uf, "uf"), None if bias is None else native.dev_ptr(bias.detach(), "bias"),
                None if res is None else native.dev_ptr(res, "res"), native.dev_ptr(out, "out"), N, Ci, Co, H, W, 1 if relu else 0,
                native.stream_ptr(x.device))
        native.check(rc, "dvis_conv1x1s2_mfma")
        return out
    out = torch.empty((N, Co, H, W), dtype=torch.float32, device=x.device)
    with torch.cuda.device(x.device):
        rc = native.lib().dvis_conv1x1_mfma(
            native.dev_ptr(x, "x"), native.dev_ptr(uf, "uf"), None if bias is None else native.dev_ptr(bias.detach(), "bias"),
            None if res is None else native.dev_ptr(res, "res"), native.dev_ptr(out, "out"), N, Ci, Co, H * W, 1 if relu else 0,
            native.stream_ptr(x.device))
    native.check(rc, "dvis_conv1x1_mfma")
    return out


WINOGRAD_DEFAULT = os.environ.get("DVIS_WINOGRAD", "1") != "0"


def _winograd_weights(weight):
    K, C = weight.shape[:2]
    return _fp32_pack(weight, "winograd", 16 * K * C, lambda w, uf, st: native.lib().dvis_conv3x3_winograd_pack(w, uf, K, C, st),
                      "dvis_conv3x3_winograd_pack")


S2_DEFAULT = os.environ.get("DVIS_CONV3X3S2", "1") != "0"


def _s2_weights(weight):
    K, C = weight.shape[:2]
    return _fp32_pack(weight, "conv3x3s2", 12 * K * C, lambda w, uf, st: native.lib().dvis_conv3x3s2_pack(w, uf, K, C, st),
                      "dvis_conv3x3s2_pack")


def conv3x3s2_bias_act(x, weight, bias=None, relu=False, own=None):
    N, C, H, W = x.shape
    K = weight.shape[0]
    if own is None and conv3x3_x3_ok(x, weight, 2):
        return conv3x3_x3(x, weight, bias, None, relu, 2)
    ok = x.is_cuda and x.dtype == torch.float32 and weight.dtype == torch.float32 and tuple(weight.shape[1:]) == (C, 3, 3) \
        and not (torch.is_grad_enabled() and (x.requires_grad or weight.requires_grad)) \
        and bool(native.lib().dvis_conv3x3s2_supported(C, K, H, W))
    if own and not ok:
        raise RuntimeError(f"conv3x3s2_bias_act(own=True): C={C} K={K} H={H} W={W} is not served (dvis_conv3x3s2_supported)")
    if ok and (own or (own is None and WINOGRAD_DEFAULT and S2_DEFAULT)):
        x = x if x.is_contiguous() else x.contiguous()
        uf = _s2_weights(weight)
        out = torch.empty((N, K, (H + 1) // 2, W // 2), dtype=torch.float32, device=x.device)
        with torch.cuda.device(x.device):
            rc = native.lib().dvis_conv3x3s2(
                native.dev_ptr(x, "x"), native.dev_ptr(uf, "uf"), None if bias is None else native.dev_ptr(bias.detach(), "bias"),
                native.dev_ptr(out, "out"), N, C, K, H, W, 1 if relu else 0, native.stream_ptr(x.device))
        native.check(rc, "dvis_conv3x3s2")
        return out
    y = torch.nn.functional.conv2d(x, weight, None, 2, 1)
    if bias is None and not relu:
        return y
    return bias_act_(y, None if bias is None else bias.detach(), None, relu)


def conv7x7s2_stem(x, weight, bias=None, relu=False, own=None):
    N, C, H, W = x.shape
    K = weight.shape[0]
    ok = x.is_cuda and x.dtype == torch.float32 and weight.dtype == torch.float32 and tuple(weight.shape) == (64, 3, 7, 7) \
        and not (torch.is_grad_enabled() and (x.requires_grad or weight.requires_grad)) \
        and bool(native.lib().dvis_conv7x7s2_supported(C, K, H, W))
    if own and not ok:
        raise RuntimeError(f"conv7x7s2_stem(own=True): C={C} K={K} H={H} W={W} is not served (dvis_conv7x7s2_supported)")
    if ok and (own or (own is None and WINOGRAD_DEFAULT and S2_DEFAULT)):
        uf = _fp32_pack(weight, "conv7x7s2", 10240, native.lib().dvis_conv7x7s2_pack, "dvis_conv7x7s2_pack")
        x = x if x.is_contiguous() else x.contiguous()
        out = torch.empty((N, 64, H // 2, W // 2), dtype=torch.float32, device=x.device)
        with torch.cuda.device(x.device):
            rc = native.lib().dvis_conv7x7s2(native.dev_ptr(x, "x"), native.dev_ptr(uf, "uf"),
                                             None if bias is None else native.dev_ptr(bias.detach(), "bias"),
                                             native.dev_ptr(out, "out"), N, H, W, 1 if relu else 0, native.stream_ptr(x.device))
        native.check(rc, "dvis_conv7x7s2")
        return out
    y = torch.nn.functional.conv2d(x, weight, None, 2, 3)
    if bias is None and not relu:
        return y
    return bias_act_(y, None if bias is None else bias.detach(), None, relu)


def conv3x3_bias_act(x, weight, bias=None, relu=False, winograd=None):
    if winograd is None and weight.shape[1] >= 128 and conv3x3_x3_ok(x, weight, 1):
        return conv3x3_x3(x, weight, bias, None, relu, 1)
    use = WINOGRAD_DEFAULT if winograd is None else winograd
    if use and x.is_cuda and x.dim() == 4 and x.dtype == torch.float32 and weight.dtype == torch.float32 \
            and tuple(weight.shape[2:]) == (3, 3) and not (torch.is_grad_enabled() and (x.requires_grad or weight.requires_grad)):
        N, C, H, W = x.shape
        K = weight.shape[0]
        served = weight.shape[1] == C and native.lib().dvis_conv3x3_winograd_supported(C, K, H, W)
        if winograd and not served:
            raise RuntimeError(f"conv3x3_bias_act(winograd=True): shape C={C} K={K} H={H} W={W} is not served "
                               "(dvis_conv3x3_winograd_supported)")
        if served:
            x = x if x.is_contiguous() else x.contiguous()
            uf = _winograd_weights(weight)
            out = torch.empty((N, K, H, W), dtype=torch.float32, device=x.device)
            with torch.cuda.device(x.device):
                rc = native.lib().dvis_conv3x3_winograd(
                    native.dev_ptr(x, "x"), native.dev_ptr(uf, "uf"),
                    None if bias is None else native.dev_ptr(bias.detach(), "bias"), native.dev_ptr(out, "out"), N, C, K, H, W,
                    1 if relu else 0, native.stream_ptr(x.device))
            native.check(rc, "dvis_conv3x3_winograd")
            return out
    y = torch.nn.functional.conv2d(x, weight, None, 1, 1)
    if bias is None and not relu:
        return y
    return bias_act_(y, None if bias is None else bias.detach(), None, relu)


def bias_act_(x, bias=None, res=None, relu=True):
    N, C, H, W = x.shape
    if not (x.is_cuda and x.dtype == torch.float32 and x.is_contiguous()
            and (res is None or (res.is_contiguous() and res.shape == x.shape and res.dtype == torch.float32))
            and not torch.is_grad_enabled()):
        _torch_path("bias_act_", x, "needs contiguous fp32 NCHW (and a matching residual)")
        if bias is not None:
            x = x + bias.view(1, -1, 1, 1)
        if res is not None:
            x = x + res
        return torch.relu_(x) if relu else x
    with torch.cuda.device(x.device):
        rc = native.lib().dvis_bias_act(native.dev_ptr(x, "x"), None if bias is None else native.dev_ptr(bias, "bias"),
                                        None if res is None else native.dev_ptr(res, "res"), N * C, C, H * W,
                                        1 if relu else 0, native.stream_ptr(x.device))
    native.check(rc, "dvis_bias_act")
    return x


def _i32(t, name):
    if t.dtype.is_floating_point or t.dtype == torch.bool or t.is_complex():
        raise RuntimeError(f"{name} must be an integer map, got {t.dtype}")
    return t.to(torch.int32).contiguous()


def _same_device(*ts):
    devs = {t.device for t in ts}
    if len(devs) != 1:
        raise RuntimeError(f"video metrics: tensors on different devices {sorted(map(str, devs))}")
    return ts[0].is_cuda


def pan_pair_hist(gt, pred, gt_table, num_pred, check=True):
    if gt.shape != pred.shape or gt.dim() != 3:
        raise RuntimeError(f"pan_pair_hist: gt {tuple(gt.shape)} and pred {tuple(pred.shape)} must be the same (T, H, W)")
    table = gt_table.reshape(-1)
    if check and table.numel() and bool((table[1:] <= table[:-1]).any() or (table <= 0).any()):
        raise ValueError("pan_pair_hist: gt_table must be strictly increasing positive ids")
    if not _same_device(gt, pred, table):
        counts, bad = cpu_ops.pan_pair_hist(gt, pred, table, int(num_pred))
    else:
        T, H, W = gt.shape
        g, p, tb = _i32(gt, "gt"), _i32(pred, "pred"), _i32(table, "gt_table")
        counts = torch.empty((T, tb.numel() + 2, int(num_pred) + 1), dtype=torch.int64, device=g.device)
        badt = torch.empty((1,), dtype=torch.int64, device=g.device)
        with torch.cuda.device(g.device):
            rc = native.lib().dvis_pan_pair_hist(native.dev_ptr(g, "gt"), native.dev_ptr(p, "pred"),
                                                 native.dev_ptr(tb, "gt_table") if tb.numel() else None, tb.numel(),
                                                 int(num_pred), T, H * W, native.dev_ptr(counts, "out"),
                                                 native.dev_ptr(badt, "bad"), native.stream_ptr(g.device))
        native.check(rc, "dvis_pan_pair_hist")
        bad = int(badt.item()) if check else 0
    if check and bad:
        raise ValueError(f"pan_pair_hist: {bad} predicted pixels outside 0..{num_pred}")
    return counts


def sem_confusion(gt, pred, num_class, check=True):
    if gt.shape != pred.shape:
        raise RuntimeError(f"sem_confusion: gt {tuple(gt.shape)} and pred {tuple(pred.shape)} differ")
    if not _same_device(gt, pred):
        conf, bad = cpu_ops.sem_confusion(gt, pred, int(num_class))
    else:
        g, p = _i32(gt, "gt"), _i32(pred, "pred")
        conf = torch.empty((int(num_class), int(num_class)), dtype=torch.int64, device=g.device)
        badt = torch.empty((1,), dtype=torch.int64, device=g.device)
        with torch.cuda.device(g.device):
            rc = native.lib().dvis_sem_confusion(native.dev_ptr(g, "gt") if g.numel() else None,
                                                 native.dev_ptr(p, "pred") if p.numel() else None, g.numel(), int(num_class),
                                                 native.dev_ptr(conf, "out"), native.dev_ptr(badt, "bad"),
                                                 native.stream_ptr(g.device))
        native.check(rc, "dvis_sem_confusion")
        bad = int(badt.item()) if check else 0
    if check and bad:
        raise ValueError(f"sem_confusion: {bad} pixels fall outside the {num_class} x {num_class} matrix")
    return conf


# ... 467 lines not shown
```

### dvis_plus_amd/native.py

```python
import ctypes
import os

import torch

_HERE = os.path.dirname(os.path.abspath(__file__))
LIB_PATH = os.environ.get("DVIS_HIP_LIB") or os.path.join(_HERE, "lib", "libdvis_hip.so")

F32, F64, F16, BF16 = 0, 1, 2, 3
_DTYPE = {torch.float32: F32, torch.float64: F64, torch.float16: F16, torch.bfloat16: BF16}

_c = ctypes
_i, _i64, _p, _f = _c.c_int, _c.c_int64, _c.c_void_p, _c.c_float

SIGNATURES = {
    "dvis_last_error": (_c.c_char_p, []),
    "dvis_version": (_i, []),
    "dvis_msda_forward": (_i, [_i, _p, _p, _p, _p, _p, _i, _i, _i, _i, _i, _i, _i, _p, _p]),
    "dvis_msda_backward": (_i, [_i, _p, _p, _p, _p, _p, _p, _i, _i, _i, _i, _i, _i, _i, _p, _p, _p, _p]),
    "dvis_msda_backward_det_ws_bytes": (_i64, [_i, _i, _i, _i]),
    "dvis_msda_backward_det": (_i, [_p, _p, _p, _p, _p, _p, _i, _i, _i, _i, _i, _i, _i, _p, _p, _p, _p, _p]),
    "dvis_msda_fused_forward": (_i, [_p, _p, _p, _p, _i, _p, _i64, _p, _i64, _i, _i, _i, _i, _i, _i, _i, _p, _p, _p]),
    "dvis_msda_fused_forward_pos": (_i, [_p, _p, _p, _p, _i, _p, _i64, _p, _i64, _p, _p, _i64, _i, _i, _i, _i, _i, _i, _i,
                                         _p, _p, _p]),
    "dvis_msda_fused_forward_h": (_i, [_i, _p, _p, _p, _p, _i, _p, _i64, _p, _i64, _i, _i, _i, _i, _i, _i, _i, _p, _p, _p]),
    "dvis_msda_fused_forward_slots": (_i, [_p, _p, _p, _p, _i, _p, _i64, _p, _i64, _i, _i, _i, _p, _p, _i64, _i, _i, _i, _i,
                                           _i, _i, _i, _p, _p, _p]),
    "dvis_nchw_to_tokens": (_i, [_p, _p, _i64, _i, _i64, _i64, _i64, _p]),
    "dvis_tokens_to_nchw": (_i, [_p, _p, _i64, _i, _i64, _i64, _i64, _p]),
    "dvis_normalize_pad": (_i, [_p, _i, _p, _i64, _i, _i, _i, _i, _i, _p, _p, _p]),
    "dvis_nchw_to_tokens_affine": (_i, [_p, _p, _p, _p, _p, _p, _i64, _i, _i64, _i64, _i64, _p]),
    "dvis_mask_logits": (_i, [_p, _p, _i, _i, _i, _i64, _p, _p]),
    "dvis_mask_logits_backward_ws_bytes": (_i64, [_i, _i, _i, _i64]),
    "dvis_mask_logits_backward": (_i, [_p, _p, _i, _i, _i, _i64, _p, _p, _p, _p]),
    "dvis_attn_mask": (_i, [_p, _p, _i, _i, _i, _i, _i, _i, _i, _p, _p, _p]),
    "dvis_center_pool3": (_i, [_p, _i64, _i, _i, _p, _p, _p, _p]),
    "dvis_attn_mask_pooled": (_i, [_p, _p, _i, _i, _i, _i, _i, _p, _p, _p]),
    "dvis_attention_ws_bytes": (_i64, [_i, _i, _i, _i]),
    "dvis_attention_ws_bytes_k": (_i64, [_i, _i, _i, _i, _i]),
    "dvis_attention_plan": (_i, [_i, _i, _i, _i, _i, _i64, _i64, _i, _p]),
    "dvis_attention_forward": (_i, [_p, _p, _p, _p, _p, _p, _p, _p, _p, _p, _i, _i, _i, _i, _i, _f, _p, _p]),
    "dvis_attention_forward_k": (_i, [_p, _p, _p, _p, _p, _p, _p, _p, _p, _p, _i, _i, _i, _i, _i, _f, _p, _p, _i]),
    "dvis_attention_backward": (_i, [_p, _p, _p, _p, _p, _p, _p, _p, _p, _p, _p, _i, _i, _i, _i, _i, _f, _p]),
    "dvis_attention_backward_threads": (_i, [_i]),
    "dvis_add_layernorm": (_i, [_p, _p, _i64, _p, _p, _p, _i64, _i, _f, _p]),
    "dvis_add_layernorm_pos": (_i, [_p, _p, _i64, _p, _p, _p, _p, _i64, _p, _i64, _i, _f, _p]),
    "dvis_bias_act": (_i, [_p, _p, _p, _i64, _i, _i64, _i, _p]),
    "dvis_conv3x3_winograd_supported": (_i, [_i, _i, _i, _i]),
    "dvis_conv3x3_winograd_pack": (_i, [_p, _p, _i, _i, _p]),
    "dvis_conv3x3_winograd": (_i, [_p, _p, _p, _p, _i, _i, _i, _i, _i, _i, _p]),
    "dvis_conv3x3s2_supported": (_i, [_i, _i, _i, _i]),
    "dvis_conv3x3s2_pack": (_i, [_p, _p, _i, _i, _p]),
    "dvis_conv3x3s2": (_i, [_p, _p, _p, _p, _i, _i, _i, _i, _i, _i, _p]),
    "dvis_conv7x7s2_supported": (_i, [_i, _i, _i, _i]),
    "dvis_conv7x7s2_pack": (_i, [_p, _p, _p]),
    "dvis_conv7x7s2": (_i, [_p, _p, _p, _p, _i, _i, _i, _i, _p]),
    "dvis_conv1x1_mfma_supported": (_i, [_i, _i, _i64]),
    "dvis_conv1x1_mfma_pack": (_i, [_p, _p, _i, _i, _p]),
    "dvis_conv1x1_mfma": (_i, [_p, _p, _p, _p, _p, _i, _i, _i, _i64, _i, _p]),
    "dvis_conv1x1s2_mfma": (_i, [_p, _p, _p, _p, _p, _i, _i, _i, _i, _i, _i, _p]),
    "dvis_conv1x1_supported": (_i, [_i, _i, _i64]),
    "dvis_conv1x1_bias_act": (_i, [_p, _p, _p, _p, _p, _i, _i, _i, _i64, _i, _p]),
    "dvis_bias_relu_maxpool": (_i, [_p, _p, _p, _i64, _i, _i, _i, _p]),
    "dvis_group_norm_affine": (_i, [_p, _p, _p, _p, _p, _i64, _i, _i, _i64, _f, _p]),
    "dvis_scale_shift_act": (_i, [_p, _p, _p, _i64, _i64, _i, _p]),
    "dvis_upsample_add_affine": (_i, [_p, _p, _p, _p, _p, _i64, _i, _i, _i, _i, _p]),
    "dvis_upsample_add": (_i, [_p, _p, _p, _i64, _i, _i, _i, _i, _p]),
    "dvis_dwconv3x3_tokens": (_i, [_p, _p, _i64, _i, _i, _i, _i, _p, _p, _i, _p]),
    "dvis_adapter_res2": (_i, [_p, _p, _p, _p, _p, _p, _i, _i, _i, _i, _p]),
    "dvis_vps_argmax": (_i, [_p, _i64, _i64, _p, _i, _i, _i, _i, _i, _i, _i, _i, _i, _i, _p, _p, _p, _p]),
    "dvis_vss_argmax": (_i, [_p, _i64, _i64, _p, _i, _i, _i, _i, _i, _i, _i, _i, _i, _i, _i, _i, _p, _p]),
    "dvis_resize2_gt0": (_i, [_p, _i64, _i64, _i, _i, _i, _i, _i, _i, _i, _i, _i, _i, _p, _p]),
    "dvis_resize2": (_i, [_p, _i64, _i64, _i, _i, _i, _i, _i, _i, _i, _i, _i, _i, _i, _p, _p]),
    "dvis_lsap_solve": (_i, [_p, _i, _i, _p]),
    "dvis_match_chain": (_i, [_p, _i, _i, _p]),
    "dvis_gemm_nt": (_i, [_p, _i64, _i64, _p, _i64, _i64, _p, _p, _i64, _i64, _p, _i64, _i64, _i, _i, _i, _i, _i, _i, _p]),
    "dvis_gemm_nt_hm": (_i, [_p, _i64, _i64, _p, _i64, _i64, _p, _p, _i64, _i64, _p, _i64, _i64, _i, _i, _i, _i, _i, _i, _i,
                             _i64, _p]),
    "dvis_gemm_nt_bb": (_i, [_p, _i64, _i64, _p, _i64, _i64, _p, _i64, _p, _i64, _i64, _p, _i64, _i64, _i, _i, _i, _i, _i, _i,
                             _p]),
    "dvis_gemm_ln": (_i, [_p, _i64, _p, _i64, _p, _p, _f, _p, _p, _f, _p, _i64, _p, _i64, _p, _p, _i64, _p, _i64, _i, _i, _i,
                          _i, _i, _p]),
    "dvis_gemm_ln_supported": (_i, [_i, _i, _i, _i]),
    "dvis_gemm_ln_num_configs": (_i, []),
    "dvis_gemm_ln_pick_config": (_i, [_i, _i, _i]),
    "dvis_x3_packed_bytes": (_i64, [_i, _i]),
    "dvis_x3_set_reserve": (_i, [_i]),
    "dvis_x3_set_range_flag": (_i, [_p]),
    "dvis_x3_set_tag": (_i, [_i]),
    "dvis_x3_pack": (_i, [_p, _i64, _i, _i, _i, _p, _p]),
    "dvis_x3_linear_supported": (_i, [_i, _i, _i]),
    "dvis_x3_linear": (_i, [_p, _i64, _i64, _i, _p, _i, _i, _i, _p, _i, _p, _i64, _p]),
    "dvis_x3_tile_supported": (_i, [_i, _i]),
    "dvis_x3_tile_packed_bytes": (_i64, [_i, _i]),
    "dvis_x3_tile_pack": (_i, [_p, _i64, _i, _i, _i, _p, _p]),
    "dvis_x3_tile_linear_qkv": (_i, [_p, _i64, _i64, _i, _p, _i, _i, _i, _p, _i, _i, _f, _p, _p]),
    "dvis_attention_x3_packed": (_i, [_p, _p, _p, _i, _i, _i, _p]),
    "dvis_x3_rows_image_bytes": (_i64, [_i64, _i]),
    "dvis_x3_rows_image": (_i, [_p, _i64, _i64, _i, _i, _p, _p]),
    "dvis_layernorm_rows_image": (_i, [_p, _p, _p, _i64, _i, _f, _i, _p, _p]),
    "dvis_x3_tile_pack_order": (_i, [_p, _i64, _i, _i, _i, _i, _p, _p]),
    "dvis_x3_tile_linear_image": (_i, [_p, _i64, _i, _p, _i, _i, _i, _p, _i, _p, _i64, _p, _i64, _p, _i, _p]),
    "dvis_x3_tile_linear_qkv_image": (_i, [_p, _i64, _i, _p, _i, _i, _i, _p, _i, _i, _f, _p, _p]),
    "dvis_attention_x3_packed_image": (_i, [_p, _p, _i, _i, _i, _i, _p]),
    "dvis_x3_tile_linear": (_i, [_p, _i64, _i64, _i, _p, _i, _i, _i, _p, _i, _p, _i64, _p, _i64, _p]),
    "dvis_x3_linear_res": (_i, [_p, _i64, _i64, _i, _p, _i, _i, _i, _p, _i, _p, _i64, _p, _i64, _p]),
    "dvis_x3_linear_add": (_i, [_p, _i64, _i64, _i, _p, _i, _i, _i, _p, _i64, _p, _i, _p, _i64, _p]),
    "dvis_x3_linear_ln": (_i, [_p, _i64, _i64, _i, _p, _i, _i, _i, _p, _p, _i64, _p, _p, _f, _p, _i64, _p, _p, _i64, _p]),
    "dvis_x3_ffn_packed_bytes": (_i64, [_i, _i, _i]),
    "dvis_x3_ffn_pack": (_i, [_p, _i64, _p, _i64, _i, _i, _i, _i, _i, _p, _p]),
    "dvis_x3_ffn_ln": (_i, [_p, _i64, _i64, _i, _i, _i, _p, _i, _i, _i, _i, _p, _p, _p, _p, _f, _p, _i64, _p, _p, _i64, _p]),
    "dvis_conv1x1_x3_supported": (_i, [_i, _i, _i64, _i64, _i64]),
    "dvis_conv1x1_x3_packed_bytes": (_i64, [_i, _i]),
    "dvis_conv1x1_x3_pack": (_i, [_p, _i, _i, _i, _p, _p]),
    "dvis_conv1x1_x3": (_i, [_p, _p, _p, _p, _p, _i, _i, _i, _i, _i, _i, _i, _i, _i, _p]),
    "dvis_conv1x1_x3_dual": (_i, [_p, _p, _p, _p, _p, _p, _i, _i, _i, _i, _i, _i, _i, _i, _i, _i, _i, _i, _p]),
    "dvis_conv3x3_x3_packed_bytes": (_i64, [_i, _i]),
    "dvis_conv3x3_x3_pack": (_i, [_p, _i, _i, _i, _p, _p]),
    "dvis_conv3x3_x3": (_i, [_p, _p, _p, _p, _p, _i, _i, _i, _i, _i, _i, _i, _i, _i, _p]),
    "dvis_bneck_x3_supported": (_i, [_i64, _i, _i]),
    "dvis_bneck_x3_image_bytes": (_i64, [_i64, _i, _i]),
    "dvis_bneck_x3_packed_bytes": (_i64, [_i, _i]),
    "dvis_bneck_x3_pack": (_i, [_p, _p, _p, _p, _i, _i, _i, _p, _p]),
    "dvis_bneck_x3": (_i, [_p, _p, _p, _p, _p, _p, _p, _p, _p, _i, _i, _i, _i, _i, _i, _i, _p]),
    "dvis_conv1x1_x3_image": (_i, [_p, _p, _p, _p, _i, _i, _i, _i, _i, _i, _i, _i, _p]),
    "dvis_conv_x3_image_bytes": (_i64, [_i64, _i, _i, _i]),
    "dvis_conv_x3_pack_image": (_i, [_p, _i, _i, _i, _i, _p, _p]),
    "dvis_conv_x3_image": (_i, [_p, _p, _p, _p, _p, _p, _p, _i, _i, _i, _i, _i, _i, _i, _i, _i, _i, _i, _p]),
    "dvis_upsample_add_image": (_i, [_p, _p, _p, _p, _p, _i, _i, _i, _i, _i, _i, _i, _p]),
    "dvis_gemm_num_configs": (_i, []),
    "dvis_gemm_pick_config": (_i, [_i, _i, _i, _i]),
    "dvis_gemm_pick_config_nw": (_i, [_i, _i, _i, _i, _i]),
    "dvis_gemm_config_waves": (_i, [_i]),
    "dvis_pan_pair_hist": (_i, [_p, _p, _p, _i, _i, _i, _i64, _p, _p, _p]),
    "dvis_sem_confusion": (_i, [_p, _p, _i64, _i, _p, _p, _p]),
    "dvis_video_consistency": (_i, [_p, _p, _i, _i64, _p, _i, _p, _p, _p]),
    "dvis_rle_encode": (_i, [_p, _i64, _i, _i, _i, _p, _p, _p, _p, _p, _p, _p]),
    "dvis_rle_strings": (_i, [_p, _p, _i64, _p, _p, _p, _p]),
    "dvis_rle_decode": (_i, [_p, _p, _i64, _i, _i, _p, _p]),
    "dvis_track_intersections": (_i, [_p, _i64, _i, _p, _i64, _i, _i, _i64, _i, _p, _p]),
    "dvis_pan_segment_stats": (_i, [_p, _i, _i, _i, _i, _p, _p, _p]),
    "dvis_pan_paint_rgb": (_i, [_p, _i64, _p, _i, _p, _p]),
    "dvis_sem_paint": (_i, [_p, _i64, _p, _p, _p, _p]),
    "dvis_resize_frames_u8": (_i, [_p, _i, _i, _i, _p, _i, _i, _p, _i, _p, _i, _i, _p]),
    "dvis_match_cost_ws_bytes": (_i64, [_i, _i, _i, _i]),
    "dvis_match_cost": (_i, [_p, _p, _i, _p, _p, _p, _i, _i, _i, _i, _i, _i, _i, _i, _i, _f, _f, _f, _p, _p, _p, _p]),
    "dvis_point_sample_rows": (_i, [_p, _i, _p, _i64, _i, _i, _i, _p, _p]),
    "dvis_point_loss_ws_bytes": (_i64, [_i64]),
    "dvis_point_loss_fwd": (_i, [_p, _p, _i, _p, _i, _i, _i, _i, _i, _i, _p, _p, _p]),
    "dvis_point_loss_bwd": (_i, [_p, _p, _i, _p, _p, _p, _p, _i, _i, _i, _i, _i, _i, _f, _p, _p, _p]),
}

_lib = None


def lib():
    global _lib
    if _lib is None:
        if not os.path.exists(LIB_PATH):
            raise RuntimeError(
                f"{LIB_PATH} not found: build it with `python -m dvis_plus_amd.build` "
                "(__graft_entry__.build()).  dvis_plus_amd has no CPU/eager fallback.")
        l = ctypes.CDLL(LIB_PATH)
        for name, (res, args) in SIGNATURES.items():
            fn = getattr(l, name)
            fn.restype, fn.argtypes = res, args
        _lib = l
    return _lib


def check(rc, what):
    if rc != 0:
        msg = lib().dvis_last_error().decode()
        raise RuntimeError(f"{what} failed (code {rc}): {msg}")


def dtype_code(t):
    try:
        return _DTYPE[t.dtype]
    except KeyError:
        raise RuntimeError(f"unsupported dtype {t.dtype}") from None


def dev_ptr(t, name):
    if not t.is_cuda:
        raise RuntimeError(f"{name} must be a GPU tensor (dvis_plus_amd has no CPU path); got device {t.device}")
    if not t.is_contiguous():
        raise RuntimeError(f"{name} tensor has to be contiguous")
    return ctypes.c_void_p(t.data_ptr())


def stream_ptr(device=None):
    return ctypes.c_void_p(torch.cuda.current_stream(device).cuda_stream)
```

### dvis_plus_amd/pixel_decoder.py

```python
import math
import os
import warnings

import torch
import torch.nn.functional as F
from torch import nn
from torch.nn.init import constant_, normal_, xavier_uniform_

from . import derived, functions as Fn
from .d2 import configurable
from .registry import SEM_SEG_HEADS_REGISTRY, ShapeSpec

_POS_IN_KERNEL = os.environ.get("DVIS_MSDA_POS", "0") == "1"
_MSDA_SLOTS = int(os.environ.get("DVIS_MSDA_SLOTS", "0") or 0)
_MSDA_HM = os.environ.get("DVIS_MSDA_HM", "0") == "1"


def _is_power_of_2(n):
    if (not isinstance(n, int)) or (n < 0):
        raise ValueError("invalid input for _is_power_of_2: {} (type: {})".format(n, type(n)))
    return (n & (n - 1) == 0) and n != 0


class PositionEmbeddingSine(nn.Module):
# ... 31 lines not shown


class MSDeformAttn(nn.Module):
    def __init__(self, d_model=256, n_levels=4, n_heads=8, n_points=4, ratio=1.0):
        super().__init__()
        if d_model % n_heads != 0:
            raise ValueError("d_model must be divisible by n_heads, but got {} and {}".format(d_model, n_heads))
        if not _is_power_of_2(d_model // n_heads):
            warnings.warn("MSDeformAttn: a power-of-2 head dimension (32 / 64) takes the tiled gfx950 kernel; "
                          "other sizes run the generic kernel.")
        self.im2col_step = 128
        self.d_model, self.n_levels, self.n_heads, self.n_points = d_model, n_levels, n_heads, n_points
        self.sampling_offsets = nn.Linear(d_model, n_heads * n_levels * n_points * 2)
        self.attention_weights = nn.Linear(d_model, n_heads * n_levels * n_points)
        self.value_proj = nn.Linear(d_model, d_model)
        self.output_proj = nn.Linear(d_model, d_model)
        self._fused = derived.Derived()
        self._reset_parameters()

    def _reset_parameters(self):
        M, L, P = self.n_heads, self.n_levels, self.n_points
        angle = torch.arange(M, dtype=torch.float32) * (2.0 * math.pi / M)
        direction = torch.stack([angle.cos(), angle.sin()], -1)
        direction = direction / direction.abs().max(-1, keepdim=True)[0]
        steps = torch.arange(1, P + 1, dtype=torch.float32)
        bias = direction[:, None, None, :] * steps[None, None, :, None]
        with torch.no_grad():
            self.sampling_offsets.bias = nn.Parameter(bias.expand(M, L, P, 2).reshape(-1).clone())
            self.sampling_offsets.weight.zero_()
            self.attention_weights.weight.zero_()
            self.attention_weights.bias.zero_()
            for proj in (self.value_proj, self.output_proj):
                xavier_uniform_(proj.weight)
                proj.bias.zero_()

    def _fused_projection(self):
        so, aw = self.sampling_offsets, self.attention_weights

        def make():
            M, LP = self.n_heads, self.n_levels * self.n_points
            width = -(-(3 * M * LP) // 64) * 64
            slot = width // M if _MSDA_SLOTS and width % M == 0 and (width // M) % 4 == 0 and width // M >= 3 * LP else 0
            if slot:
                C = so.weight.shape[1]
                w = so.weight.new_zeros(M, slot, C)
                b = so.bias.new_zeros(M, slot)
                o0, l0 = (LP, 0) if _MSDA_SLOTS == 2 else (0, 2 * LP)
                w[:, o0:o0 + 2 * LP] = so.weight.detach().view(M, 2 * LP, C)
                w[:, l0:l0 + LP] = aw.weight.detach().view(M, LP, C)
                b[:, o0:o0 + 2 * LP] = so.bias.detach().view(M, 2 * LP)
                b[:, l0:l0 + LP] = aw.bias.detach().view(M, LP)
                w, b = w.view(M * slot, C), b.view(M * slot)
            else:
                w = torch.cat([so.weight.detach(), aw.weight.detach()], 0)
                b = torch.cat([so.bias.detach(), aw.bias.detach()], 0)
                pad = width - w.shape[0]
                if pad:
                    w = torch.cat([w, w.new_zeros(pad, w.shape[1])], 0)
                    b = torch.cat([b, b.new_zeros(pad)], 0)
            w, b = w.contiguous(), b.contiguous()
            rows = w.shape[0] if slot else 3 * M * LP
            return w, b, slot, w[:rows], b[:rows]
        return self._fused.get([so.weight, so.bias, aw.weight, aw.bias], make, (_MSDA_SLOTS,))

    def _fast_path_ok(self, query, reference_points, input_padding_mask):
        d = self.d_model // self.n_heads
        return (not torch.is_grad_enabled() and query.is_cuda and query.dtype in (torch.float32, torch.float16, torch.bfloat16)
                and input_padding_mask is None and reference_points.shape[-1] == 2 and d in (32, 64)
                and (self.n_levels, self.n_points) in ((1, 4), (3, 4), (4, 4)))

    def forward(self, query, reference_points, input_flatten, input_spatial_shapes, input_level_start_index,
                input_padding_mask=None, spatial_shapes_py=None, query_pos=None, post=None):
        if post is not None:
            out = self._forward(query, reference_points, input_flatten, input_spatial_shapes, input_level_start_index,
                                input_padding_mask, spatial_shapes_py, query_pos, post)
            if isinstance(out, tuple):
                return out[0]
            return out + post[0] if post[1] is None else Fn.add_layer_norm(out, post[0], post[1])
        return self._forward(query, reference_points, input_flatten, input_spatial_shapes, input_level_start_index,
                             input_padding_mask, spatial_shapes_py, query_pos, None)

    def _forward(self, query, reference_points, input_flatten, input_spatial_shapes, input_level_start_index,
                 input_padding_mask, spatial_shapes_py, query_pos, post):
        N, Len_q, _ = query.shape
        N, Len_in, _ = input_flatten.shape
        M, L, P = self.n_heads, self.n_levels, self.n_points
        fast = self._fast_path_ok(query, reference_points, input_padding_mask)
        lowp = query.dtype != torch.float32 or torch.is_autocast_enabled()
        hm = fast and _MSDA_HM and input_flatten.is_contiguous() and not lowp
        x3 = fast and Fn.x3_on() and not lowp and not hm and not _MSDA_SLOTS and Fn.x3_ok(input_flatten, self.d_model, self.d_model) \
            and Fn.x3_ok(query, 3 * M * L * P, self.d_model)
        if x3:
            value = Fn.linear(input_flatten, self.value_proj.weight, self.value_proj.bias, tall=True).view(N, Len_in, M, -1)
        elif hm:
            value = Fn.gemm_nt(input_flatten.view(N * Len_in, self.d_model), self.value_proj.weight.detach(),
                               self.value_proj.bias.detach(), head_major=self.d_model // M).view(M, N, Len_in, -1)
        else:
            value = Fn.linear(input_flatten, self.value_proj.weight, self.value_proj.bias, tall=True)
            if input_padding_mask is not None:
                value = value.masked_fill(input_padding_mask[..., None], float(0))
            value = value.view(N, Len_in, M, self.d_model // M)
        if fast:
            w, b, slot, w_rows, b_rows = self._fused_projection()
            o_off, l_off = ((L * P, 0) if _MSDA_SLOTS == 2 else (0, 2 * L * P)) if slot else (0, M * L * P * 2)
            po = pl = None
            if lowp and slot:
                raise RuntimeError("DVIS_MSDA_SLOTS is an fp32-only layout experiment")
            if query_pos is not None and query_pos.shape[0] == 1 and _POS_IN_KERNEL and not lowp:
                pp = Fn.linear(query_pos[0], w)
                po, pl = pp[:, o_off:], pp[:, l_off:]
            elif query_pos is not None and not (x3 and query_pos.shape[0] == 1 and query.dim() == 3 and self.d_model == 256):
                query = query + query_pos
                query_pos = None
            if x3 and query_pos is not None and po is None:
                proj = Fn.x3_linear(query, w_rows, b_rows, xadd=query_pos).view(N * Len_q, -1)
            elif x3:
                proj = Fn.x3_linear(query.reshape(N * Len_q, self.d_model), w_rows, b_rows)
            else:
                proj = Fn.linear(query.reshape(N * Len_q, self.d_model), w, b, tall=True)
            ref = reference_points if reference_points.is_contiguous() else reference_points.contiguous()
            output = Fn.msda_fused_forward(value, input_spatial_shapes, input_level_start_index, ref,
                                           proj[:, o_off:], proj[:, l_off:], L, P, shapes_host=spatial_shapes_py,
                                           pos_offsets=po, pos_logits=pl, head_stride=slot, value_head_major=hm)
            if x3 and post is not None and post[1] is None and post[0].shape[:-1] == output.shape[:-1] and post[0].dtype == torch.float32:
                return (Fn.linear(output, self.output_proj.weight, self.output_proj.bias, tall=True, residual=post[0]),)
            if x3 and post is not None and post[1] is not None and Fn.x3_ok(output, self.d_model, self.d_model, ln=True) \
                    and post[0].shape == output.shape and post[0].dtype == torch.float32 and post[1].weight is not None:
                return (Fn.x3_linear_ln(output, self.output_proj.weight, self.output_proj.bias, post[0], post[1]),)
            if x3:
                return Fn.linear(output, self.output_proj.weight, self.output_proj.bias, tall=True)
            return Fn.linear(output, self.output_proj.weight, self.output_proj.bias, tall=True)
        if query_pos is not None:
            query = query + query_pos
        sampling_offsets = self.sampling_offsets(query).view(N, Len_q, M, L, P, 2)
        attention_weights = self.attention_weights(query).view(N, Len_q, M, L * P)
        attention_weights = F.softmax(attention_weights, -1).view(N, Len_q, M, L, P)
        if reference_points.shape[-1] == 2:
            offset_normalizer = torch.stack([input_spatial_shapes[..., 1], input_spatial_shapes[..., 0]], -1)
            sampling_locations = reference_points[:, :, None, :, None, :] \
                + sampling_offsets / offset_normalizer[None, None, None, :, None, :]
        elif reference_points.shape[-1] == 4:
            sampling_locations = reference_points[:, :, None, :, None, :2] \
                + sampling_offsets / P * reference_points[:, :, None, :, None, 2:] * 0.5
        else:
            raise ValueError("Last dim of reference_points must be 2 or 4, but get {} instead.".format(
                reference_points.shape[-1]))
        if value.device.type == "cpu":
            output = Fn.ms_deform_attn_core_pytorch(value, input_spatial_shapes, sampling_locations, attention_weights)
        else:
            output = Fn.MSDeformAttnFunction.apply(value.contiguous(), input_spatial_shapes, input_level_start_index,
                                                   sampling_locations.contiguous(), attention_weights.contiguous(),
                                                   self.im2col_step)
        return self.output_proj(output)


class MSDeformAttnTransformerEncoderLayer(nn.Module):
    def __init__(self, d_model=256, d_ffn=1024, dropout=0.1, activation="relu", n_levels=4, n_heads=8, n_points=4):
        super().__init__()
        if activation != "relu":
            raise NotImplementedError("only relu is used by the DVIS++ configs")
        self.self_attn = MSDeformAttn(d_model, n_levels, n_heads, n_points)
        self.norm1 = nn.LayerNorm(d_model)
        self.linear1 = nn.Linear(d_model, d_ffn)
        self.linear2 = nn.Linear(d_ffn, d_model)
        self.norm2 = nn.LayerNorm(d_model)
        self.dropout_p = dropout

    def pos_in_projection(self, src, pos):
        a = self.self_attn
        return bool(Fn.x3_on() and pos is not None and pos.dim() == 3 and pos.shape[0] == 1 and src.dim() == 3 and src.is_cuda
                    and src.dtype == torch.float32 and not torch.is_grad_enabled() and not torch.is_autocast_enabled()
                    and not _POS_IN_KERNEL and not _MSDA_SLOTS and not _MSDA_HM and a.d_model == 256
                    and 3 * a.n_heads * a.n_levels * a.n_points in (128, 192, 256, 288) and a.d_model // a.n_heads in (32, 64)
                    and (a.n_levels, a.n_points) in ((1, 4), (3, 4), (4, 4)))

    def forward(self, src, pos, reference_points, spatial_shapes, level_start_index, padding_mask=None,
                shapes_py=None, query=None, emit_next_query=False):
        pos_in_proj = self.pos_in_projection(src, pos)
        if query is not None and not pos_in_proj:
            src = self.self_attn(query, reference_points, src, spatial_shapes, level_start_index, padding_mask,
                                 spatial_shapes_py=shapes_py, post=(src, self.norm1))
        else:
            src = self.self_attn(src, reference_points, src, spatial_shapes, level_start_index, padding_mask,
                                 spatial_shapes_py=shapes_py, query_pos=pos, post=(src, self.norm1))
        if Fn.x3_on() and Fn.x3_ffn_ok(src, self.linear1, self.linear2) and self.norm2.weight is not None:
            with_pos = emit_next_query and pos is not None and pos.shape[0] == 1 and src.dim() == 3 and not pos_in_proj
            r = Fn.x3_ffn_ln(src, self.linear1, self.linear2, self.norm2, pos=pos if with_pos else None)
            return r if with_pos or not emit_next_query else (r, None)
        src2 = Fn.linear(Fn.linear_relu(src, self.linear1, tall=True), self.linear2.weight, self.linear2.bias, tall=True)
        if emit_next_query and pos is not None and pos.shape[0] == 1:
            return Fn.add_layer_norm(src2, src, self.norm2, pos=pos)
        out = Fn.add_layer_norm(src2, src, self.norm2)
        return (out, None) if emit_next_query else out


class MSDeformAttnTransformerEncoder(nn.Module):
    def __init__(self, encoder_layer_factory, num_layers):
        super().__init__()
        self.layers = nn.ModuleList([encoder_layer_factory() for _ in range(num_layers)])
        self.num_layers = num_layers
        self._ref_cache = {}

    @staticmethod
    def get_reference_points(spatial_shapes, valid_ratios, device):
        pts = []
        for lvl, (H_, W_) in enumerate(spatial_shapes):
            H_, W_ = int(H_), int(W_)
            ref_y, ref_x = torch.meshgrid(torch.linspace(0.5, H_ - 0.5, H_, dtype=torch.float32, device=device),
                                          torch.linspace(0.5, W_ - 0.5, W_, dtype=torch.float32, device=device),
                                          indexing="ij")
            ref_y = ref_y.reshape(-1)[None] / (valid_ratios[:, None, lvl, 1] * H_)
            ref_x = ref_x.reshape(-1)[None] / (valid_ratios[:, None, lvl, 0] * W_)
            pts.append(torch.stack((ref_x, ref_y), -1))
        reference_points = torch.cat(pts, 1)
        return reference_points[:, :, None] * valid_ratios[:, None]

    def reference_points_unpadded(self, shapes_py, device):
        key = (tuple(shapes_py), str(device))
        if key not in self._ref_cache:
            vr = torch.ones(1, len(shapes_py), 2, device=device)
            self._ref_cache[key] = self.get_reference_points(shapes_py, vr, device).contiguous()
        return self._ref_cache[key]

    def forward(self, src, spatial_shapes, level_start_index, valid_ratios=None, pos=None, padding_mask=None,
                shapes_py=None, query0=None):
        if valid_ratios is None:
            reference_points = self.reference_points_unpadded(shapes_py, src.device)
        else:
            reference_points = self.get_reference_points(spatial_shapes.tolist(), valid_ratios, src.device)
        output, query = src, query0
        for i, layer in enumerate(self.layers):
            last = i + 1 == len(self.layers)
            r = layer(output, pos, reference_points, spatial_shapes, level_start_index, padding_mask,
                      shapes_py=shapes_py, query=query, emit_next_query=not last)
            output, query = (r, None) if last else r
        return output


class MSDeformAttnTransformerEncoderOnly(nn.Module):
    def __init__(self, d_model=256, nhead=8, num_encoder_layers=6, dim_feedforward=1024, dropout=0.1,
                 activation="relu", num_feature_levels=4, enc_n_points=4):
        super().__init__()
        self.d_model, self.nhead = d_model, nhead
        self.encoder = MSDeformAttnTransformerEncoder(
            lambda: MSDeformAttnTransformerEncoderLayer(d_model, dim_feedforward, dropout, activation,
                                                        num_feature_levels, nhead, enc_n_points),
            num_encoder_layers)
        self.level_embed = nn.Parameter(torch.Tensor(num_feature_levels, d_model))
        self._shape_cache = {}
        self._reset_parameters()

    def _reset_parameters(self):
        for p in self.parameters():
            if p.dim() > 1:
                nn.init.xavier_uniform_(p)
        for m in self.modules():
            if isinstance(m, MSDeformAttn):
                m._reset_parameters()
        normal_(self.level_embed)

    def _shape_tensors(self, shapes_py, device):
        key = (tuple(shapes_py), str(device))
        if key not in self._shape_cache:
            s = torch.as_tensor(shapes_py, dtype=torch.long, device=device)
            lsi = torch.cat((s.new_zeros((1,)), s.prod(1).cumsum(0)[:-1]))
            self._shape_cache[key] = (s, lsi)
        return self._shape_cache[key]

    def forward(self, srcs, pos_embeds, affines=None):
        shapes_py = [(int(s.shape[2]), int(s.shape[3])) for s in srcs]
        lvl_pos = torch.cat([p.flatten(2).transpose(1, 2) + self.level_embed[lvl].view(1, 1, -1)
                             for lvl, p in enumerate(pos_embeds)], 1)
        query0 = None
        layer0 = self.encoder.layers[0] if len(self.encoder.layers) else None
        probe = srcs[0].new_empty((1, 1, srcs[0].shape[1]))
        if layer0 is not None and layer0.pos_in_projection(probe, lvl_pos):
            src_flatten = Fn.maps_to_tokens(srcs, affines)
        elif lvl_pos.shape[0] == 1 and srcs[0].is_cuda and not torch.is_grad_enabled():
            src_flatten, query0 = Fn.maps_to_tokens(srcs, affines, pos=lvl_pos)
        else:
            src_flatten = Fn.maps_to_tokens(srcs, affines)
        spatial_shapes, level_start_index = self._shape_tensors(shapes_py, src_flatten.device)
        memory = self.encoder(src_flatten, spatial_shapes, level_start_index, None, lvl_pos, None, shapes_py=shapes_py,
                              query0=query0)
        return memory, spatial_shapes, level_start_index, shapes_py


class ConvNorm(nn.Conv2d):

    def __init__(self, *args, norm=None, activation=None, **kwargs):
        super().__init__(*args, **kwargs)
        self.norm, self.activation = norm, activation

    def conv(self, x):
        if self.kernel_size == (1, 1) and self.stride == (1, 1) and self.groups == 1 and self.padding == (0, 0):
            return Fn.conv1x1(x, self.weight, self.bias)
        if self.kernel_size == (3, 3) and self.stride == (1, 1) and self.padding == (1, 1) and self.dilation == (1, 1) \
                and self.groups == 1 and x.is_cuda and not torch.is_grad_enabled():
            return Fn.conv3x3_bias_act(x, self.weight, self.bias)
        return F.conv2d(x, self.weight, self.bias, self.stride, self.padding, self.dilation, self.groups)

    def conv_and_affine(self, x):
        if isinstance(self.norm, nn.GroupNorm) and self.activation is None:
            y = self.conv(x)
            aff = Fn.group_norm_affine(y, self.norm)
            if aff is not None:
                return y, aff
            return self.norm(y), None
        return self.forward(x), None

    def image_input_ok(self, N, C, H, W, device):
        return self.stride == (1, 1) and self.dilation == (1, 1) and self.groups == 1 and self.weight.dtype == torch.float32 \
            and ((self.kernel_size == (3, 3) and self.padding == (1, 1)) or (self.kernel_size == (1, 1) and self.padding == (0, 0))) \
            and C == self.in_channels and Fn.x3_images_ok(N, C, self.out_channels, H, W, device, taps=self.kernel_size[0] ** 2)

    def forward(self, x):
        if isinstance(x, Fn.OperandImage):
            x = Fn.conv_x3_image(x, self.weight, self.bias)
        else:
            x = self.conv(x)
        if isinstance(self.norm, nn.GroupNorm) and self.activation in (None, F.relu):
            aff = Fn.group_norm_affine(x, self.norm)
            if aff is not None:
                return Fn.scale_shift_act_(x, aff[0], aff[1], relu=self.activation is not None)
        if self.norm is not None:
            x = self.norm(x)
        if self.activation is not None:
            x = self.activation(x)
        return x


def get_norm(norm, out_channels):
    if norm is None or norm == "":
        return None
    if norm != "GN":
        raise NotImplementedError(f"norm {norm!r}: the DVIS++ configs use GN")
    return nn.GroupNorm(32, out_channels)


def c2_xavier_fill(module):
    nn.init.kaiming_uniform_(module.weight, a=1)
    if module.bias is not None:
        nn.init.constant_(module.bias, 0)


@SEM_SEG_HEADS_REGISTRY.register()
class MSDeformAttnPixelDecoder(nn.Module):
    @configurable
    def __init__(self, input_shape, *, transformer_dropout, transformer_nheads, transformer_dim_feedforward,
                 transformer_enc_layers, conv_dim, mask_dim, norm=None, transformer_in_features, common_stride):
        super().__init__()
        transformer_input_shape = {k: v for k, v in input_shape.items() if k in transformer_in_features}
        input_shape = sorted(input_shape.items(), key=lambda x: x[1].stride)
        self.in_features = [k for k, v in input_shape]
        self.feature_strides = [v.stride for k, v in input_shape]
        self.feature_channels = [v.channels for k, v in input_shape]
        transformer_input_shape = sorted(transformer_input_shape.items(), key=lambda x: x[1].stride)
        self.transformer_in_features = [k for k, v in transformer_input_shape]
        transformer_in_channels = [v.channels for k, v in transformer_input_shape]
        self.transformer_feature_strides = [v.stride for k, v in transformer_input_shape]
        self.transformer_num_feature_levels = len(self.transformer_in_features)
        chans = transformer_in_channels[::-1] if self.transformer_num_feature_levels > 1 \
            else [transformer_in_channels[-1]]
        self.input_proj = nn.ModuleList([
            nn.Sequential(nn.Conv2d(c, conv_dim, kernel_size=1), nn.GroupNorm(32, conv_dim)) for c in chans])
        for proj in self.input_proj:
            nn.init.xavier_uniform_(proj[0].weight, gain=1)
            nn.init.constant_(proj[0].bias, 0)
        self.transformer = MSDeformAttnTransformerEncoderOnly(
            d_model=conv_dim, dropout=transformer_dropout, nhead=transformer_nheads,
            dim_feedforward=transformer_dim_feedforward, num_encoder_layers=transformer_enc_layers,
            num_feature_levels=self.transformer_num_feature_levels)
        self.pe_layer = PositionEmbeddingSine(conv_dim // 2, normalize=True)
        self.mask_dim = mask_dim
        self.mask_features = ConvNorm(conv_dim, mask_dim, kernel_size=1, stride=1, padding=0)
        c2_xavier_fill(self.mask_features)
        self.maskformer_num_feature_levels = 3
        self.common_stride = common_stride
        stride = min(self.transformer_feature_strides)
        self.num_fpn_levels = int(math.log2(stride) - math.log2(self.common_stride))
        lateral_convs, output_convs = [], []
        use_bias = norm == ""
        for idx, in_channels in enumerate(self.feature_channels[:self.num_fpn_levels]):
            lateral_conv = ConvNorm(in_channels, conv_dim, kernel_size=1, bias=use_bias, norm=get_norm(norm, conv_dim))
            output_conv = ConvNorm(conv_dim, conv_dim, kernel_size=3, stride=1, padding=1, bias=use_bias,
                                   norm=get_norm(norm, conv_dim), activation=F.relu)
            c2_xavier_fill(lateral_conv)
            c2_xavier_fill(output_conv)
            self.add_module("adapter_{}".format(idx + 1), lateral_conv)
            self.add_module("layer_{}".format(idx + 1), output_conv)
            lateral_convs.append(lateral_conv)
            output_convs.append(output_conv)
        self.lateral_convs = lateral_convs[::-1]
        self.output_convs = output_convs[::-1]

    @classmethod
    def from_config(cls, cfg, input_shape):
        hd = cfg.MODEL.SEM_SEG_HEAD
        return dict(
            input_shape={k: v for k, v in input_shape.items() if k in hd.IN_FEATURES},
            conv_dim=hd.CONVS_DIM, mask_dim=hd.MASK_DIM, norm=hd.NORM,
            transformer_dropout=cfg.MODEL.MASK_FORMER.DROPOUT, transformer_nheads=cfg.MODEL.MASK_FORMER.NHEADS,
            transformer_dim_feedforward=1024, transformer_enc_layers=hd.TRANSFORMER_ENC_LAYERS,
            transformer_in_features=hd.DEFORMABLE_TRANSFORMER_ENCODER_IN_FEATURES, common_stride=hd.COMMON_STRIDE)

    def forward_features(self, features):
        with torch.autocast(device_type="cuda", enabled=False), Fn.x3_stage("pd_proj"):
            srcs, pos, affines = [], [], []
            for idx, f in enumerate(self.transformer_in_features[::-1]):
                x = features[f].float().contiguous()
                conv, gn = self.input_proj[idx][0], self.input_proj[idx][1]
                s_ = Fn.conv1x1(x, conv.weight, conv.bias) if conv.kernel_size == (1, 1) and conv.stride == (1, 1) \
                    and conv.padding == (0, 0) and conv.groups == 1 else conv(x)
                affine = Fn.group_norm_affine(s_, gn)
                srcs.append(s_ if affine is not None else gn(s_))
                affines.append(affine)
                pos.append(self.pe_layer.compute(x.shape[2], x.shape[3], x.device))
            with Fn.x3_stage("encoder"):
                y, _, _, shapes_py = self.transformer(srcs, pos, affines)
            bs = y.shape[0]
            out, tokens, start = [], [], 0
            for li, (h, w) in enumerate(shapes_py):
                tokens.append(y[:, start:start + h * w])
                if li + 1 == len(shapes_py) and self.num_fpn_levels > 0:
                    out.append(Fn.tokens_to_map(y, start, h, w))
                else:
                    out.append(tokens[-1].transpose(1, 2).reshape(bs, -1, h, w))
                start += h * w
            with Fn.x3_stage("mask_path"):
                for idx, f in enumerate(self.in_features[:self.num_fpn_levels][::-1]):
                    x = features[f].float().contiguous()
                    cur_fpn, affine = self.lateral_convs[idx].conv_and_affine(x)
                    oc = self.output_convs[idx]
                    if cur_fpn.is_cuda and cur_fpn.dtype == torch.float32 and cur_fpn.is_contiguous() and out[-1].dtype == torch.float32 \
                            and oc.image_input_ok(*cur_fpn.shape, cur_fpn.device):
                        out.append(oc(Fn.upsample_add_image(cur_fpn, out[-1], affine)))
                    else:
                        out.append(oc(Fn.upsample_add(cur_fpn, out[-1], affine)))
                multi_scale_features = TokenMaps(out[:self.maskformer_num_feature_levels])
                multi_scale_features.tokens = tokens[:self.maskformer_num_feature_levels]
                return self.mask_features(out[-1]), out[0], multi_scale_features


class TokenMaps(list):
    tokens = None


def r50_input_shape():
    return {"res2": ShapeSpec(channels=256, stride=4), "res3": ShapeSpec(channels=512, stride=8),
            "res4": ShapeSpec(channels=1024, stride=16), "res5": ShapeSpec(channels=2048, stride=32)}
```

### include/dvis_hip.h

```cpp
#ifndef DVIS_HIP_H
#define DVIS_HIP_H

#include <stdint.h>

#ifdef __cplusplus
extern "C" {
#endif

enum { DVIS_F32 = 0, DVIS_F64 = 1, DVIS_F16 = 2, DVIS_BF16 = 3 };

enum {
  DVIS_OK = 0,
  DVIS_E_ARG = -1,
  DVIS_E_LAUNCH = -2,
  DVIS_E_UNSUPPORTED = -3
};

const char *dvis_last_error(void);
int dvis_version(void);

int dvis_msda_forward(int dtype, const void *value, const int64_t *shapes, const int64_t *level_start,
                      const void *loc, const void *w, int N, int S, int M, int D, int L, int Lq, int P,
                      void *out, void *stream);

int dvis_msda_backward(int dtype, const void *value, const int64_t *shapes, const int64_t *level_start,
                       const void *loc, const void *w, const void *grad_out,
                       int N, int S, int M, int D, int L, int Lq, int P,
                       void *grad_value, void *grad_loc, void *grad_w, void *stream);

int64_t dvis_msda_backward_det_ws_bytes(int N, int S, int M, int D);
int dvis_msda_backward_det(const float *value, const int64_t *shapes, const int64_t *level_start, const float *loc, const float *w,
                           const float *grad_out, int N, int S, int M, int D, int L, int Lq, int P, float *grad_value, float *grad_loc,
                           float *grad_w, void *ws, void *stream);

int dvis_msda_fused_forward(const float *value, const int64_t *shapes, const int64_t *level_start,
                            const float *ref, int Nref, const float *offsets, int64_t off_stride,
                            const float *logits, int64_t logit_stride,
                            int N, int S, int M, int D, int L, int Lq, int P, float *out,
                            const int64_t *shapes_host, void *stream);

int dvis_msda_fused_forward_pos(const float *value, const int64_t *shapes, const int64_t *level_start,
                                const float *ref, int Nref, const float *offsets, int64_t off_stride,
                                const float *logits, int64_t logit_stride, const float *pos_offsets,
                                const float *pos_logits, int64_t pos_stride, int N, int S, int M, int D, int L, int Lq,
                                int P, float *out, const int64_t *shapes_host, void *stream);

int dvis_msda_fused_forward_h(int dtype, const void *value, const int64_t *shapes, const int64_t *level_start,
                              const float *ref, int Nref, const void *offsets, int64_t off_stride, const void *logits,
                              int64_t logit_stride, int N, int S, int M, int D, int L, int Lq, int P, void *out,
                              const int64_t *shapes_host, void *stream);

int dvis_msda_fused_forward_slots(const float *value, const int64_t *shapes, const int64_t *level_start,
                                  const float *ref, int Nref, const float *offsets, int64_t off_stride,
                                  const float *logits, int64_t logit_stride, int off_head_stride, int logit_head_stride,
                                  int value_head_major, const float *pos_offsets, const float *pos_logits, int64_t pos_stride, int N, int S,
                                  int M, int D, int L, int Lq, int P, float *out, const int64_t *shapes_host,
                                  void *stream);

int dvis_mask_logits(const float *embed, const float *feat, int B, int Q, int C, int64_t HW,
                     float *out, void *stream);

int64_t dvis_mask_logits_backward_ws_bytes(int B, int R, int C, int64_t HW);
int dvis_mask_logits_backward(const float *g, const float *feat, int B, int R, int C, int64_t HW, float *grad_embed,
                              float *row_sum, void *ws, void *stream);

int dvis_attn_mask(const float *embed, const float *feat, int B, int Q, int C, int H, int W, int h, int w,
                   uint8_t *mask, int32_t *allowed_count, void *stream);
int dvis_center_pool3(const float *feat, int64_t planes, int H, int W, float *p2, float *p4, float *p8, void *stream);
int dvis_attn_mask_pooled(const float *embed, const float *pooled, int B, int Q, int C, int h, int w, uint8_t *mask,
                          int32_t *allowed_count, void *stream);

int64_t dvis_attention_ws_bytes(int BH, int Lq, int Lk, int d);
int dvis_attention_forward(const float *q, const int64_t *q_strides, const float *k, const int64_t *k_strides,
                           const float *v, const int64_t *v_strides, float *out, const int64_t *o_strides,
                           const uint8_t *mask, const int32_t *allowed_count, int B, int heads, int Lq, int Lk,
                           int d, float scale, void *ws, void *stream);
int dvis_attention_forward_k(const float *q, const int64_t *q_strides, const float *k, const int64_t *k_strides,
                           const float *v, const int64_t *v_strides, float *out, const int64_t *o_strides,
                           const uint8_t *mask, const int32_t *allowed_count, int B, int heads, int Lq, int Lk,
                           int d, float scale, void *ws, void *stream, int kernel);
int64_t dvis_attention_ws_bytes_k(int BH, int Lq, int Lk, int d, int kernel);
enum {
  DVIS_ATTN_FWD = 0,
  DVIS_ATTN_SHORT = 1,
  DVIS_ATTN_X3 = 2,
  DVIS_ATTN_KEYSPLIT = 3
};
int dvis_attention_plan(int BH, int Lq, int Lk, int d, int has_mask, int64_t k_row, int64_t v_row, int kernel, int32_t *plan);

int dvis_attention_backward(const float *q, const int64_t *q_strides, const float *k, const int64_t *k_strides,
                            const float *v, const int64_t *v_strides, const float *grad_out, const int64_t *g_strides,
                            float *dq, float *dk, float *dv, int B, int heads, int Lq, int Lk, int d, float scale,
                            void *stream);
int dvis_attention_backward_threads(int Lk);

int dvis_add_layernorm(const float *x, const float *res, int64_t res_row_stride, const float *gamma, const float *beta,
                       float *out, int64_t rows, int C, float eps, void *stream);

int dvis_add_layernorm_pos(const float *x, const float *res, int64_t res_row_stride, const float *gamma, const float *beta,
                           float *out, const float *pos, int64_t pos_rows, float *out_pos, int64_t rows, int C, float eps,
                           void *stream);

int dvis_upsample_add(const float *lateral, const float *top, float *out, int64_t planes, int H, int W, int h, int w,
                      void *stream);

int dvis_nchw_to_tokens(const float *x, float *out, int64_t N, int C, int64_t HW, int64_t S, int64_t row0, void *stream);

int dvis_tokens_to_nchw(const float *tok, float *out, int64_t N, int C, int64_t HW, int64_t S, int64_t row0, void *stream);
int dvis_normalize_pad(const void *in, int is_u8, float *out, int64_t planes, int C, int H, int W, int Hp, int Wp, const float *mean,
                       const float *stdv, void *stream);
int dvis_nchw_to_tokens_affine(const float *x, const float *scale, const float *shift, const float *pos, float *out,
                               float *out_pos, int64_t N, int C, int64_t HW, int64_t S, int64_t row0, void *stream);

int dvis_conv1x1_supported(int K, int M, int64_t HW);
int dvis_conv1x1_mfma_supported(int C, int K, int64_t HW);
int dvis_conv1x1_mfma_pack(const float *w, float *uf, int K, int C, void *stream);
int dvis_conv1x1_mfma(const float *x, const float *uf, const float *bias, const float *res, float *y, int N, int C, int K, int64_t HW,
                      int relu, void *stream);
int dvis_conv1x1s2_mfma(const float *x, const float *uf, const float *bias, const float *res, float *y, int N, int C, int K, int H, int W,
                        int relu, void *stream);
int dvis_conv1x1_bias_act(const float *x, const float *w, const float *bias, const float *res, float *out,
                          int N, int K, int M, int64_t HW, int relu, void *stream);

int dvis_conv3x3_winograd_supported(int C, int K, int H, int W);
int dvis_conv3x3s2_supported(int C, int K, int H, int W);
int dvis_conv7x7s2_supported(int C, int K, int H, int W);
int dvis_conv7x7s2_pack(const float *w, float *uf, void *stream);
int dvis_conv7x7s2(const float *x, const float *uf, const float *bias, float *y, int N, int H, int W, int relu, void *stream);
int dvis_conv3x3s2_pack(const float *w, float *uf, int K, int C, void *stream);
int dvis_conv3x3s2(const float *x, const float *uf, const float *bias, float *y, int N, int C, int K, int H, int W, int relu,
                   void *stream);
int dvis_conv3x3_winograd_pack(const float *w, float *uf, int K, int C, void *stream);
int dvis_conv3x3_winograd(const float *x, const float *uf, const float *bias, float *y, int N, int C, int K, int H, int W,
                          int relu, void *stream);

int dvis_bias_act(float *x, const float *bias, const float *res, int64_t planes, int C, int64_t HW, int relu,
                  void *stream);

int dvis_bias_relu_maxpool(const float *x, const float *bias, float *out, int64_t planes, int C, int H, int W,
                           void *stream);

int dvis_group_norm_affine(const float *x, const float *gamma, const float *beta, float *scale, float *shift, int64_t N,
                           int C, int G, int64_t HW, float eps, void *stream);
int dvis_scale_shift_act(float *x, const float *scale, const float *shift, int64_t planes, int64_t HW, int relu,
                         void *stream);
int dvis_upsample_add_affine(const float *lateral, const float *lat_scale, const float *lat_shift, const float *top,
                             float *out, int64_t planes, int H, int W, int h, int w, void *stream);

int dvis_dwconv3x3_tokens(const float *x, float *out, int64_t batch_stride, int B, int h, int w, int C, const float *weight,
                          const float *bias, int gelu, void *stream);

int dvis_adapter_res2(const float *g, const float *c1, const float *x1, const float *scale, const float *shift, float *out, int B, int C,
                      int h8, int w8, void *stream);

int dvis_vps_argmax(const float *logits, int64_t stride_k, int64_t stride_t, const float *scores, int K, int T,
                    int h, int w, int first_h, int first_w, int img_h, int img_w, int out_h, int out_w,
                    int32_t *ids, uint8_t *conf, int32_t *areas, void *stream);

int dvis_resize2_gt0(const float *logits, int64_t stride_k, int64_t stride_t, int K, int T, int h, int w, int first_h,
                     int first_w, int img_h, int img_w, int out_h, int out_w, uint8_t *out, void *stream);

int dvis_resize2(const float *logits, int64_t stride_k, int64_t stride_t, int K, int T, int h, int w, int first_h,
                 int first_w, int img_h, int img_w, int out_h, int out_w, int sigmoid, float *out, void *stream);

int dvis_vss_argmax(const float *logits, int64_t stride_q, int64_t stride_t, const float *cls, int cls_row_stride, int Q,
                    int C, int T, int h, int w, int first_h, int first_w, int img_h, int img_w, int out_h, int out_w,
                    int64_t *out, void *stream);

int dvis_lsap_solve(const double *cost, int nr, int nc, int64_t *col4row);

int dvis_match_chain(const float *cost, int T, int Q, int64_t *indices);

int dvis_gemm_nt(const float *A, int64_t lda, int64_t strideA, const float *W, int64_t ldw, int64_t strideW,
                 const float *bias, const float *res, int64_t ldres, int64_t strideRes, float *C, int64_t ldc,
                 int64_t strideC, int M, int N, int K, int batch, int act, int config, void *stream);
int dvis_gemm_nt_hm(const float *A, int64_t lda, int64_t strideA, const float *W, int64_t ldw, int64_t strideW,
                    const float *bias, const float *res, int64_t ldres, int64_t strideRes, float *C, int64_t ldc,
                    int64_t strideC, int M, int N, int K, int batch, int act, int config, int head_d, int64_t head_stride,
                    void *stream);
int dvis_gemm_nt_bb(const float *A, int64_t lda, int64_t strideA, const float *W, int64_t ldw, int64_t strideW,
                    const float *bias, int64_t strideBias, const float *res, int64_t ldres, int64_t strideRes, float *C,
                    int64_t ldc, int64_t strideC, int M, int N, int K, int batch, int act, int config, void *stream);
int dvis_gemm_num_configs(void);
int dvis_gemm_pick_config(int M, int N, int K, int batch);
int dvis_gemm_pick_config_nw(int M, int N, int K, int batch, int nw);
int dvis_gemm_config_waves(int config);

int dvis_gemm_ln(const float *A, int64_t lda, const float *add, int64_t ldadd, const float *gamma1, const float *beta1,
                 float eps1, const float *gamma2, const float *beta2, float eps2, float *a_out, int64_t ldaout,
                 const float *W, int64_t ldw, const float *bias, const float *res, int64_t ldres, float *C, int64_t ldc,
                 int M, int N, int K, int act, int config, void *stream);
int dvis_gemm_ln_supported(int M, int N, int K, int norms);
int dvis_gemm_ln_num_configs(void);
int dvis_gemm_ln_pick_config(int M, int N, int K);

int64_t dvis_x3_packed_bytes(int N, int K);
int dvis_x3_set_reserve(int cus);
int dvis_x3_set_range_flag(int32_t *device_word);
int dvis_x3_set_tag(int tag);
int dvis_x3_pack(const float *W, int64_t ldw, int N, int K, int wexp, void *packed, void *stream);
int dvis_x3_linear_supported(int N, int K, int ln);
int dvis_x3_linear(const float *x, int64_t ldx, int64_t M, int K, const void *packed, int N, int xexp, int wexp,
                   const float *bias, int relu, float *out, int64_t ldo, void *stream);
int dvis_x3_linear_add(const float *x, int64_t ldx, int64_t M, int K, const void *packed, int N, int xexp, int wexp,
                       const float *xadd, int64_t xadd_rows, const float *bias, int relu, float *out, int64_t ldo, void *stream);
int dvis_x3_linear_res(const float *x, int64_t ldx, int64_t M, int K, const void *wp, int N, int xexp, int wexp, const float *bias, int act,
                       const float *res, int64_t ldres, float *out, int64_t ldo, void *stream);

int dvis_x3_tile_supported(int N, int K);
int64_t dvis_x3_tile_packed_bytes(int N, int K);
int dvis_x3_tile_pack(const float *w, int64_t ldw, int N, int K, int wexp, void *packed, void *stream);
int dvis_x3_tile_linear(const float *x, int64_t ldx, int64_t M, int K, const void *wp, int N, int xexp, int wexp, const float *bias, int act,
                        const float *res, int64_t ldres, float *out, int64_t ldo, void *stream);
int dvis_x3_tile_linear_qkv(const float *x, int64_t ldx, int64_t M, int K, const void *wp, int N, int xexp, int wexp, const float *bias,
                            int heads, int L, float qscale, void *ws, void *stream);
int dvis_attention_x3_packed(const void *ws, float *out, const int64_t *o_strides, int B, int heads, int L, void *stream);
int64_t dvis_x3_rows_image_bytes(int64_t M, int K);
int dvis_x3_rows_image(const float *x, int64_t ldx, int64_t M, int K, int xexp, void *image, void *stream);
int dvis_layernorm_rows_image(const float *x, const float *gamma, const float *beta, int64_t M, int C, float eps, int xexp, void *image,
                              void *stream);
int dvis_x3_tile_pack_order(const float *w, int64_t ldw, int N, int K, int wexp, int order, void *packed, void *stream);
int dvis_x3_tile_linear_image(const void *ximg, int64_t M, int K, const void *wp, int N, int xexp, int wexp, const float *bias, int act,
                              const float *res, int64_t ldres, float *out, int64_t ldo, void *oimg, int oexp, void *stream);
int dvis_x3_tile_linear_qkv_image(const void *ximg, int64_t M, int K, const void *wp, int N, int xexp, int wexp, const float *bias, int heads,
                                  int L, float qscale, void *ws, void *stream);
int dvis_attention_x3_packed_image(const void *ws, void *image, int B, int heads, int L, int xexp, void *stream);
int dvis_x3_linear_ln(const float *x, int64_t ldx, int64_t M, int K, const void *packed, int N, int xexp, int wexp,
                      const float *bias, const float *res, int64_t ldres, const float *gamma, const float *beta, float eps,
                      const float *pos, int64_t pos_rows, float *out, float *out2, int64_t ldo, void *stream);
int64_t dvis_x3_ffn_packed_bytes(int K, int H, int N);
int dvis_conv1x1_x3_supported(int C, int K, int64_t N, int64_t HW_in, int64_t HW_out);
int64_t dvis_conv1x1_x3_packed_bytes(int C, int K);
int dvis_conv1x1_x3_pack(const float *w, int K, int C, int wexp, void *packed, void *stream);
int dvis_conv1x1_x3(const float *x, const void *packed, const float *bias, const float *res, float *y, int N, int C, int K, int H,
                    int W, int stride, int xexp, int wexp, int relu, void *stream);
int dvis_conv1x1_x3_dual(const float *x, const float *x2, const void *packed, const float *bias, const float *res, float *y, int N,
                         int C, int C2, int K, int H, int W, int H2, int W2, int stride2, int xexp, int wexp, int relu, void *stream);
int64_t dvis_conv3x3_x3_packed_bytes(int C, int K);
int dvis_conv3x3_x3_pack(const float *w, int K, int C, int wexp, void *packed, void *stream);
int dvis_conv3x3_x3(const float *x, const void *packed, const float *bias, const float *res, float *y, int N, int C, int K, int H,
                    int W, int stride, int xexp, int wexp, int relu, void *stream);
int dvis_bneck_x3_supported(int64_t N, int H, int W);
int64_t dvis_bneck_x3_image_bytes(int64_t N, int H, int W);
int64_t dvis_bneck_x3_packed_bytes(int tail, int dual);
int dvis_bneck_x3_pack(const float *w2, const float *w3, const float *ws, const float *w1, int e2, int e3, int e1, void *packed,
                       void *stream);
int dvis_bneck_x3(const void *a1, const float *res, const float *x2, const void *packed, const float *b2, const float *b3,
                  const float *b1, float *y, void *out, int N, int H, int W, int xexp, int e2, int e3, int e1, void *stream);
int dvis_conv1x1_x3_image(const float *x, const void *packed, const float *bias, void *image, int N, int C, int H, int W, int xexp,
                          int wexp, int oexp, int relu, void *stream);
int64_t dvis_conv_x3_image_bytes(int64_t N, int C, int H, int W);
int dvis_conv_x3_pack_image(const float *w, int K, int C, int taps, int wexp, void *packed, void *stream);
int dvis_conv_x3_image(const void *ximg, const float *x, const void *packed, const float *bias, const float *res, float *y, void *image,
                       int N, int C, int K, int H, int W, int stride, int taps, int xexp, int wexp, int oexp, int relu, void *stream);
int dvis_upsample_add_image(const float *lateral, const float *lat_scale, const float *lat_shift, const float *top, void *image, int N,
                            int C, int H, int W, int h, int w, int oexp, void *stream);
int dvis_x3_ffn_pack(const float *W1, int64_t ldw1, const float *W2, int64_t ldw2, int K, int H, int N, int w1exp, int w2exp,
                     void *packed, void *stream);
int dvis_x3_ffn_ln(const float *x, int64_t ldx, int64_t M, int K, int H, int N, const void *packed, int xexp, int w1exp,
                   int hexp, int w2exp, const float *b1, const float *b2, const float *gamma, const float *beta, float eps,
                   const float *pos, int64_t pos_rows, float *out, float *out2, int64_t ldo, void *stream);

int dvis_pan_pair_hist(const int32_t *gt, const int32_t *pred, const int32_t *gt_table, int Ng, int Np, int T, int64_t HW,
                       int64_t *out, int64_t *bad, void *stream);
int dvis_sem_confusion(const int32_t *gt, const int32_t *pred, int64_t n, int num_class, int64_t *out, int64_t *bad, void *stream);
int dvis_video_consistency(const int32_t *gt, const int32_t *pred, int T, int64_t HW, const int32_t *ks, int nk, int64_t *gt_const,
                           int64_t *both_const, void *stream);

int dvis_rle_encode(const uint8_t *masks, int64_t N, int H, int W, int phase, int64_t *trans, int64_t *area, const int64_t *toff,
                    const int64_t *moff, int32_t *bnd, uint32_t *runs, void *stream);
int dvis_rle_strings(const uint32_t *runs, const int64_t *run_off, int64_t N, const int64_t *str_off, int64_t *lens, uint8_t *chars,
                     void *stream);
int dvis_rle_decode(const int32_t *ends, const int64_t *run_off, int64_t N, int H, int W, uint8_t *out, void *stream);
int dvis_track_intersections(const uint8_t *pred, int64_t pred_stride, int P, const uint8_t *gt, int64_t gt_stride, int G, int T,
                             int64_t HW, int accumulate, int64_t *out, void *stream);

int dvis_pan_segment_stats(const int32_t *map, int T, int H, int W, int n, int64_t *out, int64_t *bad, void *stream);
int dvis_pan_paint_rgb(const int32_t *map, int64_t npx, const int32_t *lut, int nlut, uint8_t *out, void *stream);
int dvis_sem_paint(const int32_t *map, int64_t npx, const int32_t *lut, uint8_t *out, int64_t *bad, void *stream);

int dvis_resize_frames_u8(const uint8_t *in, int T, int H, int W, uint8_t *out, int h, int w, const int32_t *xtab, int kx,
                          const int32_t *ytab, int ky, int reverse, void *stream);

int64_t dvis_match_cost_ws_bytes(int Q, int G, int T, int K);
int dvis_match_cost(const float *pred, const void *tgt, int tgt_u8, const float *coords, const float *logits,
                    const int64_t *tgt_ids, int Q, int G, int T, int H, int W, int Ht, int Wt, int K, int NC, float w_class,
                    float w_mask, float w_dice, float *C, float *terms, void *ws, void *stream);
int dvis_point_sample_rows(const void *rows, int rows_u8, const float *coords, int64_t R, int P, int H, int W, float *out,
                           void *stream);
int64_t dvis_point_loss_ws_bytes(int64_t R);
int dvis_point_loss_fwd(const float *src, const void *tgt, int tgt_u8, const float *coords, int R, int P, int H, int W, int Ht, int Wt,
                        float *out, void *ws, void *stream);
int dvis_point_loss_bwd(const float *src, const void *tgt, int tgt_u8, const float *coords, const float *sums, const float *g_mask,
                        const float *g_dice, int R, int P, int H, int W, int Ht, int Wt, float num_masks, float *grad_src,
                        void *det_ws, void *stream);

#ifdef __cplusplus
}
#endif
#endif
```

Measured before the change: 420.6.

## Fuse GroupNorm statistics into conv epilogue and defer norm into consumer conv

The x3 conv kernel gains template modes that accumulate per-group sum and sum-of-squares partials in double in its epilogue, and that apply a per-image, per-channel scale/shift (plus optional ReLU) to inputs as they are loaded, using an LDS table. The pixel decoder now finalizes GroupNorm from these partials and carries a DeferredNorm forward, so the next 1x1 conv applies the normalization on input instead of a separate GN pass. The upsample-add kernel also reads the top map through arbitrary strides (avoiding a tokens-to-map copy), processes two rows per step and caches the lateral affine. This removes several full-map memory passes at the cost of extra epilogue shuffles, double arithmetic and thread-local launch state.

Result: no change. 420.5 (-0.0%).

```diff
diff --git a/dvis_plus_amd/csrc/conv1x1_x3.hip b/dvis_plus_amd/csrc/conv1x1_x3.hip
--- a/dvis_plus_amd/csrc/conv1x1_x3.hip
+++ b/dvis_plus_amd/csrc/conv1x1_x3.hip
@@ -28,7 +28,12 @@
   int OH;
   const void *ximg;
   int XG_in;
+  double *part;
+  const float *in_scale, *in_shift;
+  int in_relu;
 };
+
+constexpr int kCxTable = 32 * 1024;
 
 __device__ __forceinline__ bool cx_item(const CxArgs &a, long long w, long long *tile, int *pass) {
   const int xcd = blockIdx.x & 7, i = blockIdx.x >> 3, per = gridDim.x >> 3;
@@ -77,8 +82,10 @@
   return (unsigned)(n * a.C2 * a.HW2_in * 4) + (unsigned)((oy * a.stride2 * a.W2_in + ox * a.stride2) * 4);
 }
 
-template <int NB, int IK, bool IMGIN = false, bool IMGOUT = false>
+template <int NB, int IK, bool IMGIN = false, bool IMGOUT = false, bool STATS = false, bool AFFIN = false>
 __global__ __launch_bounds__(512) void conv1x1_x3_kernel(const CxArgs a) {
+  static_assert(!(STATS || AFFIN) || (NB == 8 && !IMGOUT), "the statistics and input-affine forms: 256 output channels per pass, an fp32 map out");
+  static_assert(!(AFFIN && IMGIN), "the input affine belongs to the fp32 load path");
   constexpr int NW = 8, kTile = NW * 32, PW = 2 * IK * NB / NW, STAGES = IK == 4 ? 2 : 3, IPC = 4 / IK;
   static_assert(2 * IK * NB % NW == 0, "the item's pieces must divide among the waves");
   extern __shared__ __attribute__((aligned(1024))) char lds[];
@@ -165,6 +172,20 @@
 #pragma unroll
       for (int i = 0; i < 16; ++i) acc[nb][i] = 0.f;
     const long long n = p / a.HW;
+    const float2 *tab = nullptr;
+    if constexpr (AFFIN) {
+      float2 *table = reinterpret_cast<float2 *>(lds + STAGES * RingT::kItemBytes);
+      const long long n0 = tile * kTile / a.HW;
+      const long long pl = tile * kTile + kTile - 1 < a.pixels ? tile * kTile + kTile - 1 : a.pixels - 1;
+      const int rows = (int)(pl / a.HW - n0 + 1) * a.C;
+      for (int i = threadIdx.x; i < rows; i += NW * 64) {
+        float2 t;
+        t.x = a.in_scale[n0 * a.C + i], t.y = a.in_shift[n0 * a.C + i];
+        table[i] = t;
+      }
+      __syncthreads();
+      tab = table + (p < a.pixels ? (int)(n - n0) * a.C : 0) + 8 * g;
+    }
     const unsigned obase = p < a.pixels ? (unsigned)((n * a.K * a.HW + (p - n * a.HW)) * 4) : kOOB;
     const unsigned ochan = (unsigned)(a.HW * 4);
     const int co0 = pass * 32 * NB;
@@ -182,6 +203,19 @@
       } else {
 #pragma unroll
         for (int i = 0; i < 32; ++i) asm volatile("" : "+v"(raw[i]));
+        if constexpr (AFFIN) {
+#pragma unroll
+          for (int s = 0; s < 4; ++s)
+#pragma unroll
+            for (int e = 0; e < 8; ++e) {
+              const float2 t = tab[64 * kc + 16 * s + e];
+              float v = raw[8 * s + e] * t.x + t.y;
+              if (a.in_relu) v = fmaxf(v, 0.f);
+              raw[8 * s + e] = v;
+            }
+#pragma unroll
+          for (int i = 0; i < 32; ++i) asm volatile("" : "+v"(raw[i]));
+        }
 #pragma unroll
         for (int s = 0; s < 4; ++s) {
           const f4 lo4 = {raw[8 * s], raw[8 * s + 1], raw[8 * s + 2], raw[8 * s + 3]};
@@ -247,11 +281,13 @@
         rv[r] = a.res ? __builtin_bit_cast(float, __builtin_amdgcn_raw_buffer_load_b32(
                                                       rr, obase + (unsigned)(co0 + 32 * nb + 8 * (r >> 2) + 4 * g + (r & 3)) * ochan, 0, 0))
                       : 0.f;
+      double gs[4], gq[4];
 #pragma unroll
       for (int q = 0; q < 4; ++q) {
         const int co = co0 + 32 * nb + 8 * q + 4 * g;
         f4 b = {0.f, 0.f, 0.f, 0.f};
         if (a.bias) b = *(const f4 *)(a.bias + co);
+        gs[q] = 0.0, gq[q] = 0.0;
 #pragma unroll
         for (int i = 0; i < 4; ++i) {
           const unsigned o = obase + (unsigned)(co + i) * ochan;
@@ -259,6 +295,25 @@
           chk = __builtin_fmaf(v, 0.f, chk);
           if (a.relu) v = x3_relu(v);
           __builtin_amdgcn_raw_buffer_store_b32(__builtin_bit_cast(unsigned, v), ry, o, 0, 0);
+          if constexpr (STATS) gs[q] += (double)v, gq[q] += (double)v * (double)v;
+        }
+      }
+      if constexpr (STATS) {
+        const bool hi5 = g != 0, hi4 = (lane & 16) != 0;
+        double s2[2], q2[2];
+#pragma unroll
+        for (int k = 0; k < 2; ++k) {
+          s2[k] = (hi5 ? gs[2 + k] : gs[k]) + __shfl_xor(hi5 ? gs[k] : gs[2 + k], 32);
+          q2[k] = (hi5 ? gq[2 + k] : gq[k]) + __shfl_xor(hi5 ? gq[k] : gq[2 + k], 32);
+        }
+        double s1 = (hi4 ? s2[1] : s2[0]) + __shfl_xor(hi4 ? s2[0] : s2[1], 16);
+        double q1 = (hi4 ? q2[1] : q2[0]) + __shfl_xor(hi4 ? q2[0] : q2[1], 16);
+#pragma unroll
+        for (int o = 8; o > 0; o >>= 1) s1 += __shfl_xor(s1, o), q1 += __shfl_xor(q1, o);
+        if ((lane & 15) == 0 && p < a.pixels) {
+          double2 t;
+          t.x = s1, t.y = q1;
+          *reinterpret_cast<double2 *>(a.part + ((p >> 5) * 32 + (co0 >> 3) + 4 * nb + 2 * g + (hi4 ? 1 : 0)) * 2) = t;
         }
       }
     }
@@ -267,7 +322,67 @@
   }
 }
 
-__global__ __launch_bounds__(256) void upsample_add_image_kernel(const float *__restrict__ lateral, const float *__restrict__ top,
+struct UaTop {
+  long long tn, tc, tp;
+};
+struct UaRow {
+  float lat[8], t[4][8];
+  float ly0, ly1;
+};
+template <bool TOK>
+__device__ __forceinline__ void ua_load(UaRow &r, const float *__restrict__ lateral, const float *__restrict__ top, const UaTop ts,
+                                        unsigned n, int y, int C, int H, int W, int h, int w, int c0, int pxc, int x0, int x1, float sy) {
+  float fy = sy * ((float)y + 0.5f) - 0.5f;
+  fy = fy < 0.f ? 0.f : fy;
+  const int y0 = min((int)fy, h - 1), y1 = y0 + (y0 < h - 1 ? 1 : 0);
+  r.ly1 = fy - (float)y0, r.ly0 = 1.f - r.ly1;
+  const float *tb = top + (size_t)n * ts.tn;
+  const size_t o00 = ((size_t)y0 * w + x0) * ts.tp, o01 = ((size_t)y0 * w + x1) * ts.tp, o10 = ((size_t)y1 * w + x0) * ts.tp,
+               o11 = ((size_t)y1 * w + x1) * ts.tp;
+  if constexpr (TOK) {
+#pragma unroll
+    for (int u = 0; u < 2; ++u) {
+      const float *tc = tb + c0 + 8 * u;
+      const f4 a = *(const f4 *)(tc + o00), b = *(const f4 *)(tc + o01), c = *(const f4 *)(tc + o10), d = *(const f4 *)(tc + o11);
+#pragma unroll
+      for (int i = 0; i < 4; ++i) r.t[0][4 * u + i] = a[i], r.t[1][4 * u + i] = b[i], r.t[2][4 * u + i] = c[i], r.t[3][4 * u + i] = d[i];
+    }
+  }
+#pragma unroll
+  for (int e = 0; e < 8; ++e) {
+    const int c = c0 + 8 * (e >> 2) + (e & 3);
+    const unsigned pl = n * (unsigned)C + (unsigned)c;
+    if constexpr (!TOK) {
+      const float *tc = tb + (size_t)c * ts.tc;
+      r.t[0][e] = tc[o00], r.t[1][e] = tc[o01], r.t[2][e] = tc[o10], r.t[3][e] = tc[o11];
+    }
+    r.lat[e] = lateral[((size_t)pl * H + y) * (size_t)W + pxc];
+  }
+}
+__device__ __forceinline__ void ua_store(const UaRow &r, bool affine, const float *sc, const float *sh, float lx0, float lx1, float oscale, __amdgpu_buffer_rsrc_t ri,
+                                         unsigned off) {
+  float v[8];
+#pragma unroll
+  for (int e = 0; e < 8; ++e) {
+#pragma clang fp contract(off)
+    const float lat = affine ? __builtin_fmaf(r.lat[e], sc[e], sh[e]) : r.lat[e];
+    const float r1 = __builtin_fmaf(lx0, r.t[2][e], lx1 * r.t[3][e]);
+    if (e < 7) {
+      const float r0 = __builtin_fmaf(lx0, r.t[0][e], lx1 * r.t[1][e]);
+      v[e] = lat + __builtin_fmaf(r.ly0, r0, r.ly1 * r1);
+    } else {
+      const float r0 = __builtin_fmaf(lx1, r.t[1][e], lx0 * r.t[0][e]);
+      v[e] = lat + (r.ly0 * r0 + r.ly1 * r1);
+    }
+  }
+  const f4 p0 = {v[0], v[1], v[2], v[3]}, p1 = {v[4], v[5], v[6], v[7]};
+  h8 hi, lo;
+  split8(p0, p1, oscale, hi, lo);
+  store_fragments2(ri, off, hi, 0, lo, 1024);
+}
+
+template <bool TOK>
+__global__ __launch_bounds__(256) void upsample_add_image_kernel(const float *__restrict__ lateral, const float *__restrict__ top, const UaTop ts,
                                                                  void *__restrict__ img, int N, int C, int H, int W, int h, int w,
                                                                  const float *__restrict__ lat_scale, const float *__restrict__ lat_shift,
                                                                  float oscale) {
@@ -283,51 +398,70 @@
   const float lx1 = fx - (float)x0, lx0 = 1.f - lx1;
   const __amdgpu_buffer_rsrc_t ri = dvis_make_rsrc_uniform(img, (unsigned)((long long)N * H * XG * NCC * 8192));
   const unsigned rows = (unsigned)N * (unsigned)H;
-  for (unsigned row = blockIdx.z * 16u; row < blockIdx.z * 16u + 16u && row < rows; ++row) {
+  const int c0 = 64 * cc + 32 * (S >> 1) + 16 * (S & 1) + 4 * g;
+  const unsigned lane_off = (unsigned)cc * 8192u + (unsigned)(S * 2048 + g * 512 + x * 16);
+  const unsigned end = min(blockIdx.z * 16u + 16u, rows);
+  float sc[8], sh[8];
+  unsigned cur = ~0u;
+  for (unsigned row = blockIdx.z * 16u; row < end;) {
     const unsigned n = row / (unsigned)H;
     const int y = (int)(row - n * (unsigned)H);
-    float fy = sy * ((float)y + 0.5f) - 0.5f;
-    fy = fy < 0.f ? 0.f : fy;
-    const int y0 = min((int)fy, h - 1), y1 = y0 + (y0 < h - 1 ? 1 : 0);
-    const float ly1 = fy - (float)y0, ly0 = 1.f - ly1;
-    float v[8];
-#pragma unroll
-    for (int e = 0; e < 8; ++e) {
-      const int c = 64 * cc + 32 * (S >> 1) + 16 * (S & 1) + 8 * (e >> 2) + 4 * g + (e & 3);
-      const unsigned pl = n * (unsigned)C + (unsigned)c;
-      const float *t0 = top + ((size_t)pl * h + y0) * (size_t)w, *t1 = top + ((size_t)pl * h + y1) * (size_t)w;
-      float lat = lateral[((size_t)pl * H + y) * (size_t)W + pxc];
-      if (lat_scale) lat = lat * lat_scale[pl] + lat_shift[pl];
-      v[e] = lat + (ly0 * (lx0 * t0[x0] + lx1 * t0[x1]) + ly1 * (lx0 * t1[x0] + lx1 * t1[x1]));
-    }
-    const f4 p0 = {v[0], v[1], v[2], v[3]}, p1 = {v[4], v[5], v[6], v[7]};
-    h8 hi, lo;
-    split8(p0, p1, oscale, hi, lo);
-    const unsigned G = row * (unsigned)XG + (unsigned)xg;
-    const unsigned off = (G * (unsigned)NCC + (unsigned)cc) * 8192u + (unsigned)(S * 2048 + g * 512 + x * 16);
-    store_fragments2(ri, off, hi, 0, lo, 1024);
-  }
-}
-
-}
-
-DVIS_EXPORT int dvis_upsample_add_image(const float *lateral, const float *lat_scale, const float *lat_shift, const float *top, void *image,
-                                        int N, int C, int H, int W, int h, int w, int oexp, void *stream) {
+    const bool two = row + 1 < end && y + 1 < H;
+    if (lat_scale != nullptr && n != cur) {
+      cur = n;
+#pragma unroll
+      for (int e = 0; e < 8; ++e) {
+        const unsigned pl = n * (unsigned)C + (unsigned)(c0 + 8 * (e >> 2) + (e & 3));
+        sc[e] = lat_scale[pl], sh[e] = lat_shift[pl];
+      }
+    }
+    UaRow ra, rb;
+    ua_load<TOK>(ra, lateral, top, ts, n, y, C, H, W, h, w, c0, pxc, x0, x1, sy);
+    ua_load<TOK>(rb, lateral, top, ts, n, two ? y + 1 : y, C, H, W, h, w, c0, pxc, x0, x1, sy);
+    ua_store(ra, lat_scale != nullptr, sc, sh, lx0, lx1, oscale, ri, (row * (unsigned)XG + (unsigned)xg) * (unsigned)NCC * 8192u + lane_off);
+    if (two) ua_store(rb, lat_scale != nullptr, sc, sh, lx0, lx1, oscale, ri, ((row + 1) * (unsigned)XG + (unsigned)xg) * (unsigned)NCC * 8192u + lane_off);
+    row += two ? 2 : 1;
+  }
+}
+
+}
+
+static int ua_launch(const float *lateral, const float *lat_scale, const float *lat_shift, const float *top, UaTop ts, void *image, int N, int C,
+                     int H, int W, int h, int w, int oexp, void *stream) {
   DVIS_REQUIRE(lateral && top && image, "dvis_upsample_add_image: null pointer");
   DVIS_REQUIRE((lat_scale == nullptr) == (lat_shift == nullptr), "dvis_upsample_add_image: scale and shift together");
   DVIS_REQUIRE(N > 0 && C > 0 && C % 64 == 0 && H > 0 && W > 0 && h > 0 && w > 0, "dvis_upsample_add_image: bad sizes");
   DVIS_REQUIRE((uintptr_t)image % 16 == 0 && dvis_conv_x3_image_bytes(N, C, H, W) < ((int64_t)1 << 31), "dvis_upsample_add_image: a 16-byte "
                "aligned image below 2 GiB");
+  DVIS_REQUIRE(ts.tn >= 0 && ts.tc > 0 && ts.tp > 0, "dvis_upsample_add_image: top strides (%lld, %lld, %lld)", ts.tn, ts.tc, ts.tp);
+  const bool tok = ts.tc == 1 && ts.tp % 4 == 0 && ts.tn % 4 == 0 && (uintptr_t)top % 16 == 0;
   const int per = 16 * 65535 / H;
   DVIS_REQUIRE(per >= 1 && (W + 31) / 32 <= 65535, "dvis_upsample_add_image: map too large (%d x %d)", H, W);
   for (int i = 0; i < N; i += per) {
     const int n = N - i < per ? N - i : per;
-    hipLaunchKernelGGL(upsample_add_image_kernel, dim3(C / 64, (W + 31) / 32, (n * H + 15) / 16), dim3(256), 0, (hipStream_t)stream,
-                       lateral + (size_t)i * C * H * W, top + (size_t)i * C * h * w,
-                       (char *)image + (size_t)i * H * ((W + 31) / 32) * (C / 64) * 8192, n, C, H, W, h, w,
-                       lat_scale ? lat_scale + (size_t)i * C : nullptr, lat_shift ? lat_shift + (size_t)i * C : nullptr, ldexpf(1.f, oexp));
+    const dim3 grid(C / 64, (W + 31) / 32, (n * H + 15) / 16);
+    void *im = (char *)image + (size_t)i * H * ((W + 31) / 32) * (C / 64) * 8192;
+    const float *sc = lat_scale ? lat_scale + (size_t)i * C : nullptr, *sh = lat_shift ? lat_shift + (size_t)i * C : nullptr;
+    if (tok)
+      hipLaunchKernelGGL(upsample_add_image_kernel<true>, grid, dim3(256), 0, (hipStream_t)stream, lateral + (size_t)i * C * H * W,
+                         top + (size_t)i * ts.tn, ts, im, n, C, H, W, h, w, sc, sh, ldexpf(1.f, oexp));
+    else
+      hipLaunchKernelGGL(upsample_add_image_kernel<false>, grid, dim3(256), 0, (hipStream_t)stream, lateral + (size_t)i * C * H * W,
+                         top + (size_t)i * ts.tn, ts, im, n, C, H, W, h, w, sc, sh, ldexpf(1.f, oexp));
   }
   return dvis_check_launch("dvis_upsample_add_image");
+}
+
+DVIS_EXPORT int dvis_upsample_add_image(const float *lateral, const float *lat_scale, const float *lat_shift, const float *top, void *image,
+                                        int N, int C, int H, int W, int h, int w, int oexp, void *stream) {
+  return ua_launch(lateral, lat_scale, lat_shift, top, UaTop{(long long)C * h * w, (long long)h * w, 1}, image, N, C, H, W, h, w, oexp, stream);
+}
+
+DVIS_EXPORT int dvis_upsample_add_image_strided(const float *lateral, const float *lat_scale, const float *lat_shift, const float *top,
+                                                int64_t top_n, int64_t top_c, int64_t top_p, void *image, int N, int C, int H, int W, int h, int w,
+                                                int oexp, void *stream) {
+  return ua_launch(lateral, lat_scale, lat_shift, top, UaTop{(long long)top_n, (long long)top_c, (long long)top_p}, image, N, C, H, W, h, w, oexp,
+                   stream);
 }
 
 DVIS_EXPORT int dvis_conv1x1_x3_supported(int C, int K, int64_t N, int64_t HW_in, int64_t HW_out) {
@@ -357,6 +491,29 @@
 static int cx_launch(const float *x, const void *packed, const float *bias, const float *res, float *y, int N, int C, int K, int H, int W,
                      int stride, int taps, int xexp, int wexp, int relu, void *stream, const float *x2 = nullptr, int C2 = 0, int H2 = 0,
                      int W2 = 0, int stride2 = 1, void *image = nullptr, int oexp = 0, const void *ximg = nullptr);
+
+struct CxExtras {
+  double *part;
+  const float *in_scale, *in_shift;
+  int in_relu;
+};
+static thread_local CxExtras t_cx_extras = {nullptr, nullptr, nullptr, 0};
+
+DVIS_EXPORT int dvis_conv_x3_set_next(double *partials, const float *in_scale, const float *in_shift, int in_relu) {
+  DVIS_REQUIRE((in_scale == nullptr) == (in_shift == nullptr), "dvis_conv_x3_set_next: scale and shift together");
+  DVIS_REQUIRE(partials == nullptr || in_scale == nullptr, "dvis_conv_x3_set_next: statistics or an input affine, not both");
+  DVIS_REQUIRE((uintptr_t)partials % 16 == 0, "dvis_conv_x3_set_next: partials must be 16-byte aligned");
+  t_cx_extras = CxExtras{partials, in_scale, in_shift, in_relu};
+  return DVIS_OK;
+}
+
+DVIS_EXPORT int dvis_conv_x3_stats_supported(int K, int64_t HW) { return K == 256 && HW > 0 && HW % 32 == 0; }
+
+DVIS_EXPORT int dvis_conv_x3_affine_supported(int C, int K, int64_t N, int64_t HW) {
+  if (!(K > 0 && K % 256 == 0 && C >= 64 && C % 64 == 0 && N > 0 && HW > 0)) return 0;
+  const int64_t span = 255 / HW + 2, nimg = N < span ? N : span;
+  return nimg * C * 8 <= kCxTable;
+}
 
 DVIS_EXPORT int dvis_conv1x1_x3_dual(const float *x, const float *x2, const void *packed, const float *bias, const float *res, float *y,
                                      int N, int C, int C2, int K, int H, int W, int H2, int W2, int stride2, int xexp, int wexp, int relu,
@@ -437,6 +594,8 @@
 static int cx_launch(const float *x, const void *packed, const float *bias, const float *res, float *y, int N, int C, int K, int H, int W,
                      int stride, int taps, int xexp, int wexp, int relu, void *stream, const float *x2, int C2, int H2, int W2, int stride2,
                      void *image, int oexp, const void *ximg) {
+  const CxExtras ex = t_cx_extras;
+  t_cx_extras = CxExtras{nullptr, nullptr, nullptr, 0};
   DVIS_REQUIRE((x || ximg) && packed && (y || image), "dvis_conv1x1_x3: null operand");
   DVIS_REQUIRE(stride == 1 || stride == 2, "dvis_conv1x1_x3: stride %d", stride);
   const int OH = (H + stride - 1) / stride, OW = (W + stride - 1) / stride;
@@ -457,6 +616,31 @@
   const int grid = dvis_x3_persistent_cus();
   hipStream_t st = (hipStream_t)stream;
   a.npass = K <= 128 ? 1 : K / 256;
+  a.part = ex.part, a.in_scale = ex.in_scale, a.in_shift = ex.in_shift, a.in_relu = ex.in_relu;
+#define DVIS_CX_LAUNCH_EX(INV, STATSV, AFFINV, WHAT)                                                                                 \
+  {                                                                                                                                  \
+    static DvisLdsOptIn opted;                                                                                                       \
+    typedef Ring<8, 8, 8, 2> R;                                                                                                      \
+    a.tiles = (a.pixels + 255) / 256;                                                                                                \
+    const size_t lds = 2 * R::kItemBytes + (AFFINV ? kCxTable : 0);                                                                  \
+    const int rc = dvis_lds_opt_in((const void *)conv1x1_x3_kernel<8, 4, INV, false, STATSV, AFFINV>, lds, &opted, WHAT);            \
+    if (rc != DVIS_OK) return rc;                                                                                                    \
+    hipLaunchKernelGGL((conv1x1_x3_kernel<8, 4, INV, false, STATSV, AFFINV>), dim3(grid), dim3(512), lds, st, a);                    \
+    return dvis_check_launch(WHAT);                                                                                                  \
+  }
+  if (ex.part != nullptr) {
+    DVIS_REQUIRE(image == nullptr && x2 == nullptr && dvis_conv_x3_stats_supported(K, a.HW), "dvis_conv_x3_set_next: the statistics form serves "
+                 "K = 256 on maps of a multiple of 32 pixels, an fp32 map out, one source (K %d, %lld pixels)", K, a.HW);
+    if (ximg) DVIS_CX_LAUNCH_EX(true, true, false, "dvis_conv_x3_image (statistics)")
+    DVIS_CX_LAUNCH_EX(false, true, false, "dvis_conv1x1_x3 (statistics)")
+  }
+  if (ex.in_scale != nullptr) {
+    DVIS_REQUIRE(ximg == nullptr && image == nullptr && x2 == nullptr && taps == 1 && stride == 1 && dvis_conv_x3_affine_supported(C, K, N, a.HW),
+                 "dvis_conv_x3_set_next: the input-affine form serves fp32 1x1 convolutions of stride 1 with K %% 256 == 0 (C %d, K %d, taps %d, "
+                 "stride %d, %lld pixels)", C, K, taps, stride, a.HW);
+    DVIS_CX_LAUNCH_EX(false, false, true, "dvis_conv1x1_x3 (input affine)")
+  }
+#undef DVIS_CX_LAUNCH_EX
 #define DVIS_CX_LAUNCH(NBV, IKV)                                                                              \
   {                                                                                                           \
     static DvisLdsOptIn opted;                                                                                \
diff --git a/dvis_plus_amd/csrc/fused_elementwise.hip b/dvis_plus_amd/csrc/fused_elementwise.hip
--- a/dvis_plus_amd/csrc/fused_elementwise.hip
+++ b/dvis_plus_amd/csrc/fused_elementwise.hip
@@ -698,6 +698,58 @@
   return dvis_check_launch("group_norm_affine_kernel");
 }
 
+namespace {
+
+__global__ __launch_bounds__(256) void group_norm_finalize_kernel(const double *__restrict__ part, const float *__restrict__ gamma,
+                                                                  const float *__restrict__ beta, float *__restrict__ scale,
+                                                                  float *__restrict__ shift, int slots, float eps) {
+  __shared__ double s_sum[32][8], s_sq[32][8];
+  constexpr int C = 256, Cg = 8;
+  const int n = blockIdx.x >> 2, g0 = 8 * (blockIdx.x & 3);
+  const int j = threadIdx.x & 7, t = threadIdx.x >> 3;
+  const double2 *pp = reinterpret_cast<const double2 *>(part) + ((size_t)n * slots) * 32 + g0 + j;
+  double sum = 0.0, sq = 0.0;
+  for (int s = t; s < slots; s += 32) {
+    const double2 v = pp[(size_t)s * 32];
+    sum += v.x;
+    sq += v.y;
+  }
+  s_sum[t][j] = sum;
+  s_sq[t][j] = sq;
+  __syncthreads();
+  if (threadIdx.x < 8 * Cg) {
+    const int gj = threadIdx.x >> 3;
+    double ts = 0.0, tq = 0.0;
+#pragma unroll
+    for (int i = 0; i < 32; ++i) {
+      ts += s_sum[i][gj];
+      tq += s_sq[i][gj];
+    }
+    const double count = (double)Cg * 32.0 * (double)slots;
+    const double mean = ts / count;
+    double var = tq / count - mean * mean;
+    var = var < 0.0 ? 0.0 : var;
+    const float rstd = (float)(1.0 / sqrt(var + (double)eps));
+    const int c = (g0 + gj) * Cg + (threadIdx.x & 7);
+    const float a = rstd * (gamma ? gamma[c] : 1.f);
+    scale[(size_t)n * C + c] = a;
+    shift[(size_t)n * C + c] = (beta ? beta[c] : 0.f) - (float)mean * a;
+  }
+}
+
+}
+
+DVIS_EXPORT int dvis_group_norm_finalize(const double *partials, const float *gamma, const float *beta, float *scale, float *shift, int64_t N,
+                                         int64_t HW, float eps, void *stream) {
+  DVIS_REQUIRE(N >= 0 && HW > 0 && HW % 32 == 0 && HW / 32 < (1ll << 31), "group_norm_finalize: a multiple of 32 pixels per image");
+  if (N == 0) return DVIS_OK;
+  DVIS_REQUIRE(partials && scale && shift && (uintptr_t)partials % 16 == 0, "group_norm_finalize: null / unaligned pointer");
+  DVIS_REQUIRE(N * 4 < (1ll << 31), "group_norm_finalize: too many images");
+  hipLaunchKernelGGL(group_norm_finalize_kernel, dim3((unsigned)(N * 4)), dim3(256), 0, (hipStream_t)stream, partials, gamma, beta, scale,
+                     shift, (int)(HW / 32), eps);
+  return dvis_check_launch("group_norm_finalize_kernel");
+}
+
 DVIS_EXPORT int dvis_scale_shift_act(float *x, const float *scale, const float *shift, int64_t planes, int64_t HW, int relu,
                                      void *stream) {
   DVIS_REQUIRE(planes >= 0 && HW > 0, "scale_shift_act: bad sizes");
diff --git a/dvis_plus_amd/functions.py b/dvis_plus_amd/functions.py
--- a/dvis_plus_amd/functions.py
+++ b/dvis_plus_amd/functions.py
@@ -1589,7 +1589,73 @@
     return max(1, min(N, (2 ** 31 - 1) // per))
 
 
-def conv1x1_x3(x, weight, bias=None, res=None, relu=False, stride=1, xexp=None):
+def _conv_next(lib, part, i, n, slots, in_affine, C):
+    if part is None and in_affine is None:
+        return
+    pp = None if part is None else ctypes.c_void_p(part.data_ptr() + i * slots * 64 * 8)
+    sc = sh = None
+    if in_affine is not None:
+        sc = native.dev_ptr(in_affine[0].reshape(-1, C)[i:i + n], "in_scale")
+        sh = native.dev_ptr(in_affine[1].reshape(-1, C)[i:i + n], "in_shift")
+    native.check(lib.dvis_conv_x3_set_next(pp, sc, sh, 1 if in_affine is not None and in_affine[2] else 0), "dvis_conv_x3_set_next")
+
+
+def _conv_launch(lib, rc_call, what):
+    try:
+        native.check(rc_call(), what)
+    except Exception:
+        lib.dvis_conv_x3_set_next(None, None, None, 0)
+        raise
+
+
+def gn_stats_ok(norm, K, H, W):
+    return isinstance(norm, torch.nn.GroupNorm) and norm.num_groups == 32 and norm.num_channels == K \
+        and bool(native.lib().dvis_conv_x3_stats_supported(K, H * W))
+
+
+def conv_in_affine_ok(x, weight):
+    if not (weight.dim() == 4 and tuple(weight.shape[2:]) == (1, 1) and conv1x1_x3_ok(x, weight)):
+        return False
+    N, Ci, H, W = x.shape
+    return N > 0 and bool(native.lib().dvis_conv_x3_affine_supported(Ci, weight.shape[0], N, H * W))
+
+
+def group_norm_finalize(part, norm, N, C, HW):
+    scale = torch.empty(N * C, dtype=torch.float32, device=part.device)
+    shift = torch.empty(N * C, dtype=torch.float32, device=part.device)
+    with torch.cuda.device(part.device):
+        rc = native.lib().dvis_group_norm_finalize(
+            ctypes.c_void_p(part.data_ptr()), None if norm.weight is None else native.dev_ptr(norm.weight.detach(), "gamma"),
+            None if norm.bias is None else native.dev_ptr(norm.bias.detach(), "beta"), native.dev_ptr(scale, "scale"),
+            native.dev_ptr(shift, "shift"), N, HW, float(norm.eps), native.stream_ptr(part.device))
+    native.check(rc, "dvis_group_norm_finalize")
+    return scale, shift
+
+
+def conv1x1_gn(x, weight, bias, norm):
+    N, _, H, W = x.shape
+    K = weight.shape[0]
+    if N > 0 and conv1x1_x3_ok(x, weight) and gn_stats_ok(norm, K, H, W):
+        y, part = conv1x1_x3(x, weight, bias, stats=True)
+        return y, group_norm_finalize(part, norm, N, K, H * W)
+    y = conv1x1(x, weight, bias)
+    return y, group_norm_affine(y, norm)
+
+
+class DeferredNorm:
+
+    def __init__(self, raw, scale, shift, relu):
+        self.raw, self.scale, self.shift, self.relu = raw, scale, shift, relu
+        self._done = None
+
+    def materialize(self):
+        if self._done is None:
+            self._done = scale_shift_act_(self.raw, self.scale, self.shift, relu=self.relu)
+            self.raw = None
+        return self._done
+
+
+def conv1x1_x3(x, weight, bias=None, res=None, relu=False, stride=1, xexp=None, stats=False, in_affine=None):
     N, Ci, H, W = x.shape
     Co = weight.shape[0]
 
@@ -1598,17 +1664,21 @@
     buf, wexp = _x3_cache(weight, [weight], make, kind="conv1x1")
     OH, OW = (H + stride - 1) // stride, (W + stride - 1) // stride
     out = torch.empty((N, Co, OH, OW), dtype=torch.float32, device=x.device)
+    slots = OH * OW // 32
+    part = torch.empty(N * slots * 64, dtype=torch.float64, device=x.device) if stats else None
     step = _conv_x3_chunks(N, Ci, Co, H * W, OH * OW)
+    lib = native.lib()
     with torch.cuda.device(x.device):
         for i in range(0, N, step):
             n = min(step, N - i)
-            native.check(native.lib().dvis_conv1x1_x3(
+            _conv_next(lib, part, i, n, slots, in_affine, Ci)
+            _conv_launch(lib, lambda: lib.dvis_conv1x1_x3(
                 native.dev_ptr(x[i:i + n], "x"), ctypes.c_void_p(buf.data_ptr()),
                 None if bias is None else native.dev_ptr(bias.detach(), "bias"),
                 None if res is None else native.dev_ptr(res[i:i + n], "res"), native.dev_ptr(out[i:i + n], "out"), n, Ci, Co, H, W,
                 stride, X3_CONV_XEXP if xexp is None else xexp, wexp, 1 if relu else 0, native.stream_ptr(x.device)),
                 "dvis_conv1x1_x3")
-    return out
+    return (out, part) if stats else out
 
 
 X3_DUAL = os.environ.get("DVIS_X3_DUAL", "1") != "0"
@@ -1709,11 +1779,18 @@
     return max(1, min(N, (2 ** 31 - 1) // per))
 
 
+def top_strided_ok(top):
+    return top.dim() == 4 and top.is_cuda and top.dtype == torch.float32 and top.stride(2) == top.shape[3] * top.stride(3) \
+        and min(top.stride()) >= 1
+
+
 def upsample_add_image(lateral, top, lat_affine=None, oexp=None):
     N, C, H, W = lateral.shape
     lib = native.lib()
     oe = X3_CONV_XEXP if oexp is None else oexp
-    top = top.contiguous()
+    if not top_strided_ok(top):
+        top = top.contiguous()
+    tn, tc, _, tp = top.stride()
     data = torch.empty(lib.dvis_conv_x3_image_bytes(N, C, H, W), dtype=torch.uint8, device=lateral.device)
     img = OperandImage(data, N, C, H, W, oe)
     step = _image_chunks(N, C, C, H, W, H, W)
@@ -1722,13 +1799,14 @@
             n = min(step, N - i)
             sc = None if lat_affine is None else native.dev_ptr(lat_affine[0].reshape(N, C)[i:i + n], "scale")
             sh = None if lat_affine is None else native.dev_ptr(lat_affine[1].reshape(N, C)[i:i + n], "shift")
-            native.check(lib.dvis_upsample_add_image(native.dev_ptr(lateral[i:i + n], "lateral"), sc, sh, native.dev_ptr(top[i:i + n], "top"),
-                                                     ctypes.c_void_p(img.images(i, n).data_ptr()), n, C, H, W, top.shape[-2], top.shape[-1], oe,
-                                                     native.stream_ptr(lateral.device)), "dvis_upsample_add_image")
+            native.check(lib.dvis_upsample_add_image_strided(
+                native.dev_ptr(lateral[i:i + n], "lateral"), sc, sh, ctypes.c_void_p(top[i:i + n].data_ptr()), tn, tc, tp,
+                ctypes.c_void_p(img.images(i, n).data_ptr()), n, C, H, W, top.shape[-2], top.shape[-1], oe,
+                native.stream_ptr(lateral.device)), "dvis_upsample_add_image")
     return img
 
 
-def conv_x3_image(src, weight, bias=None, res=None, relu=False, stride=1, out_image=False, oexp=None, xexp=None):
+def conv_x3_image(src, weight, bias=None, res=None, relu=False, stride=1, out_image=False, oexp=None, xexp=None, stats=False):
     lib = native.lib()
     from_img = isinstance(src, OperandImage)
     if not (from_img or out_image):
@@ -1753,16 +1831,19 @@
     else:
         out = torch.empty((N, K, OH, OW), dtype=torch.float32, device=dev)
     step = _image_chunks(N, C, K, H, W, OH, OW)
+    slots = OH * OW // 32
+    part = torch.empty(N * slots * 64, dtype=torch.float64, device=dev) if stats else None
     with torch.cuda.device(dev):
         for i in range(0, N, step):
             n = min(step, N - i)
-            native.check(lib.dvis_conv_x3_image(
+            _conv_next(lib, part, i, n, slots, None, C)
+            _conv_launch(lib, lambda: lib.dvis_conv_x3_image(
                 ctypes.c_void_p(src.images(i, n).data_ptr()) if from_img else None, None if from_img else native.dev_ptr(src[i:i + n], "x"),
                 ctypes.c_void_p(buf.data_ptr()), None if bias is None else native.dev_ptr(bias.detach(), "bias"),
                 None if res is None else native.dev_ptr(res[i:i + n], "res"), None if out_image else native.dev_ptr(out[i:i + n], "out"),
                 ctypes.c_void_p(out.images(i, n).data_ptr()) if out_image else None, n, C, K, H, W, stride, taps, xe, wexp, oe, 1 if relu else 0,
                 native.stream_ptr(dev)), "dvis_conv_x3_image")
-    return out
+    return (out, part) if stats else out
 
 
 X3_BNECK = os.environ.get("DVIS_X3_BNECK", "1") != "0"
diff --git a/dvis_plus_amd/native.py b/dvis_plus_amd/native.py
--- a/dvis_plus_amd/native.py
+++ b/dvis_plus_amd/native.py
@@ -127,6 +127,11 @@
     "dvis_conv_x3_pack_image": (_i, [_p, _i, _i, _i, _i, _p, _p]),
     "dvis_conv_x3_image": (_i, [_p, _p, _p, _p, _p, _p, _p, _i, _i, _i, _i, _i, _i, _i, _i, _i, _i, _i, _p]),
     "dvis_upsample_add_image": (_i, [_p, _p, _p, _p, _p, _i, _i, _i, _i, _i, _i, _i, _p]),
+    "dvis_upsample_add_image_strided": (_i, [_p, _p, _p, _p, _i64, _i64, _i64, _p, _i, _i, _i, _i, _i, _i, _i, _p]),
+    "dvis_conv_x3_set_next": (_i, [_p, _p, _p, _i]),
+    "dvis_conv_x3_stats_supported": (_i, [_i, _i64]),
+    "dvis_conv_x3_affine_supported": (_i, [_i, _i, _i64, _i64]),
+    "dvis_group_norm_finalize": (_i, [_p, _p, _p, _p, _p, _i64, _i64, _f, _p]),
     "dvis_gemm_num_configs": (_i, []),
     "dvis_gemm_pick_config": (_i, [_i, _i, _i, _i]),
     "dvis_gemm_pick_config_nw": (_i, [_i, _i, _i, _i, _i]),
diff --git a/dvis_plus_amd/pixel_decoder.py b/dvis_plus_amd/pixel_decoder.py
--- a/dvis_plus_amd/pixel_decoder.py
+++ b/dvis_plus_amd/pixel_decoder.py
@@ -357,19 +357,37 @@
 
     def conv_and_affine(self, x):
         if isinstance(self.norm, nn.GroupNorm) and self.activation is None:
-            y = self.conv(x)
-            aff = Fn.group_norm_affine(y, self.norm)
+            if self._plain_1x1():
+                y, aff = Fn.conv1x1_gn(x, self.weight, self.bias, self.norm)
+            else:
+                y = self.conv(x)
+                aff = Fn.group_norm_affine(y, self.norm)
             if aff is not None:
                 return y, aff
             return self.norm(y), None
         return self.forward(x), None
 
+    def _plain_1x1(self):
+        return self.kernel_size == (1, 1) and self.stride == (1, 1) and self.groups == 1 and self.padding == (0, 0)
+
+    def forward_deferred(self, x):
+        if isinstance(x, Fn.OperandImage) and self.activation in (None, F.relu) \
+                and Fn.gn_stats_ok(self.norm, self.out_channels, x.H, x.W):
+            y, part = Fn.conv_x3_image(x, self.weight, self.bias, stats=True)
+            scale, shift = Fn.group_norm_finalize(part, self.norm, x.N, self.out_channels, x.H * x.W)
+            return Fn.DeferredNorm(y, scale, shift, self.activation is not None)
+        return self.forward(x)
+
     def image_input_ok(self, N, C, H, W, device):
         return self.stride == (1, 1) and self.dilation == (1, 1) and self.groups == 1 and self.weight.dtype == torch.float32 \
             and ((self.kernel_size == (3, 3) and self.padding == (1, 1)) or (self.kernel_size == (1, 1) and self.padding == (0, 0))) \
             and C == self.in_channels and Fn.x3_images_ok(N, C, self.out_channels, H, W, device, taps=self.kernel_size[0] ** 2)
 
     def forward(self, x):
+        if isinstance(x, Fn.DeferredNorm):
+            if self.norm is None and self.activation is None and x.raw is not None and Fn.conv_in_affine_ok(x.raw, self.weight):
+                return Fn.conv1x1_x3(x.raw, self.weight, self.bias, in_affine=(x.scale, x.shift, x.relu))
+            x = x.materialize()
         if isinstance(x, Fn.OperandImage):
             x = Fn.conv_x3_image(x, self.weight, self.bias)
         else:
@@ -465,9 +483,11 @@
             for idx, f in enumerate(self.transformer_in_features[::-1]):
                 x = features[f].float().contiguous()
                 conv, gn = self.input_proj[idx][0], self.input_proj[idx][1]
-                s_ = Fn.conv1x1(x, conv.weight, conv.bias) if conv.kernel_size == (1, 1) and conv.stride == (1, 1) \
-                    and conv.padding == (0, 0) and conv.groups == 1 else conv(x)
-                affine = Fn.group_norm_affine(s_, gn)
+                if conv.kernel_size == (1, 1) and conv.stride == (1, 1) and conv.padding == (0, 0) and conv.groups == 1:
+                    s_, affine = Fn.conv1x1_gn(x, conv.weight, conv.bias, gn)
+                else:
+                    s_ = conv(x)
+                    affine = Fn.group_norm_affine(s_, gn)
                 srcs.append(s_ if affine is not None else gn(s_))
                 affines.append(affine)
                 pos.append(self.pe_layer.compute(x.shape[2], x.shape[3], x.device))
@@ -477,23 +497,28 @@
             out, tokens, start = [], [], 0
             for li, (h, w) in enumerate(shapes_py):
                 tokens.append(y[:, start:start + h * w])
-                if li + 1 == len(shapes_py) and self.num_fpn_levels > 0:
+                view = tokens[-1].transpose(1, 2).reshape(bs, -1, h, w)
+                if li + 1 == len(shapes_py) and self.num_fpn_levels > 0 and not Fn.top_strided_ok(view):
                     out.append(Fn.tokens_to_map(y, start, h, w))
                 else:
-                    out.append(tokens[-1].transpose(1, 2).reshape(bs, -1, h, w))
+                    out.append(view)
                 start += h * w
             with Fn.x3_stage("mask_path"):
                 for idx, f in enumerate(self.in_features[:self.num_fpn_levels][::-1]):
                     x = features[f].float().contiguous()
                     cur_fpn, affine = self.lateral_convs[idx].conv_and_affine(x)
                     oc = self.output_convs[idx]
+                    if isinstance(out[-1], Fn.DeferredNorm):
+                        out[-1] = out[-1].materialize()
                     if cur_fpn.is_cuda and cur_fpn.dtype == torch.float32 and cur_fpn.is_contiguous() and out[-1].dtype == torch.float32 \
                             and oc.image_input_ok(*cur_fpn.shape, cur_fpn.device):
-                        out.append(oc(Fn.upsample_add_image(cur_fpn, out[-1], affine)))
+                        out.append(oc.forward_deferred(Fn.upsample_add_image(cur_fpn, out[-1], affine)))
                     else:
                         out.append(oc(Fn.upsample_add(cur_fpn, out[-1], affine)))
-                multi_scale_features = TokenMaps(out[:self.maskformer_num_feature_levels])
-                multi_scale_features.tokens = tokens[:self.maskformer_num_feature_levels]
+                nl = self.maskformer_num_feature_levels
+                out[:nl] = [o.materialize() if isinstance(o, Fn.DeferredNorm) else o for o in out[:nl]]
+                multi_scale_features = TokenMaps(out[:nl])
+                multi_scale_features.tokens = tokens[:nl]
                 return self.mask_features(out[-1]), out[0], multi_scale_features
 
 
diff --git a/include/dvis_hip.h b/include/dvis_hip.h
--- a/include/dvis_hip.h
+++ b/include/dvis_hip.h
@@ -255,6 +255,13 @@
                        int N, int C, int K, int H, int W, int stride, int taps, int xexp, int wexp, int oexp, int relu, void *stream);
 int dvis_upsample_add_image(const float *lateral, const float *lat_scale, const float *lat_shift, const float *top, void *image, int N,
                             int C, int H, int W, int h, int w, int oexp, void *stream);
+int dvis_upsample_add_image_strided(const float *lateral, const float *lat_scale, const float *lat_shift, const float *top, int64_t top_n,
+                                    int64_t top_c, int64_t top_p, void *image, int N, int C, int H, int W, int h, int w, int oexp, void *stream);
+int dvis_conv_x3_set_next(double *partials, const float *in_scale, const float *in_shift, int in_relu);
+int dvis_conv_x3_stats_supported(int K, int64_t HW);
+int dvis_conv_x3_affine_supported(int C, int K, int64_t N, int64_t HW);
+int dvis_group_norm_finalize(const double *partials, const float *gamma, const float *beta, float *scale, float *shift, int64_t N, int64_t HW,
+                             float eps, void *stream);
 int dvis_x3_ffn_pack(const float *W1, int64_t ldw1, const float *W2, int64_t ldw2, int K, int H, int N, int w1exp, int w2exp,
                      void *packed, void *stream);
 int dvis_x3_ffn_ln(const float *x, int64_t ldx, int64_t M, int K, int H, int N, const void *packed, int xexp, int w1exp,
```
